# TheoCoombes/ClipCap

Hardware: AMD Instinct MI355X
Metric: train samples/sec (512-d prefix, 40-tok caption) (higher is better)
Workload: dtype bf16; 1 GPU; BASELINE configs[1]: TransformerMapper(8L,P=L=10,H=8)+frozen GPT-2-small; per_gpu_batch=256, global_batch=256, encoder_dim=512, train_language_model=False, parallelism=dp1

## Files before the change

clipcap_amd/_lib.py:

```python
from __future__ import annotations

import ctypes as C
import os
import threading

HERE = os.path.dirname(os.path.abspath(__file__))
_SEL = os.environ.get("CLIPCAP_HIP_LIB", "")
LIB_PATH = os.path.join(HERE, "libclipcap_hip.so") if not _SEL else os.path.join(HERE, "libclipcap_hip_lab.so") if _SEL == "lab" else _SEL
IS_LAB = _SEL == "lab"

ERR = {0: "ok", -1: "invalid argument", -2: "unsupported shape / alignment", -3: "kernel launch failed", -4: "invalid state"}


class HipExtensionMissing(RuntimeError):
    pass


class CCError(RuntimeError):
    pass


OP_BF16, OP_FP16, OP_X3 = 0, 1, 2


# ... 44 lines not shown
    "cc_gpt2_embed": (_I, [_GC, _GS, _P, _P, _P, _P, _P]),
    "cc_gpt2_embed_from": (_I, [_GC, _GS, _P, _P, _P, _P]),
    "cc_gpt2_fwd": (_I, [_GC, _GS, _P, _P, _P, _P]),
    "cc_gpt2_logits": (_I, [_GC, _GS, _P, _P, _P, _P, _L, _P]),
    "cc_gpt2_logits_bwd": (_I, [_GC, _GS, _P, _P, _P, _P, _L, _P, _P, _P]),
    "cc_lmhead_ce_fwd": (_I, [_GC, _GS, _P, _P, _P, _P, _P, _P]),
    "cc_lmhead_score": (_I, [_GC, _GS, _P, _P, _P, _P, _I, _P, _P, _P]),
    "cc_lmhead_ce_bwd": (_I, [_GC, _GS, _P, _P, _P, _P, _P, _P, _P]),
    "cc_lmhead_put_x": (_I, [_GC, _GS, _P, _P, _P]),
    "cc_lmhead_get": (_I, [_GC, _GS, _P, _I, _P, _L, _P]),
    "cc_gpt2_bwd": (_I, [_GC, _GS, _P, _P, _P, _P, _P, _P, _P]),
    "cc_decode_ws_bytes": (_L, [_GC, _I, _I]),
    "cc_decode_fwd": (_I, [_GC, _I, _I, _I, _I, _P, _P, _P, _P, _P, _P, _P, _L, _P]),
    "cc_decode_part_floats": (_L, [_GC, _I]),
    "cc_decode_fwd_p": (_I, [_GC, _I, _I, _I, _I, _P, _P, _P, _P, _P, _P, _P, _L, _P, _P]),
    "cc_decode_fwd_g": (_I, [_GC, _I, _I, _I, _I, _P, _P, _P, _P, _P, _I, _P, _P, _L, _P, _P]),
    "cc_beam_step_p": (_I, [_I, _I, _I, _P, _L, _P, _I, _F, _I, _I, _P, _P, _P, _P, _P, _P, _P]),
    "cc_decode_reorder": (_I, [_GC, _I, _I, _I, _I, _P, _P, _P, _P]),
    "cc_beam_step": (_I, [_I, _I, _I, _P, _L, _F, _I, _I, _P, _P, _P, _P, _P, _P, _P]),
    "cc_beam_ws_bytes": (_L, [_I, _I, _I]),
    "cc_logits_constrain": (_I, [_P, _I, _I, _L, _P, _I, _P, _I, _L, _I, _I, _I, _P, _I, _P, _P]),
    "cc_embed_tokens": (_I, [_GC, _I, _P, _P, _P, _P]),
    "cc_embed_tokens_bwd": (_I, [_GC, _I, _P, _P, _P, _P]),
    "cc_embed_tokens_bwd_ws": (_I, [_GC, _I, _P, _P, _P, _P, _P]),
    "cc_embed_tokens_bwd_ws_bytes": (_L, [_GC, _I]),
    "cc_beam_advance": (_I, [_GC, _I, _I, _P, _P, _P, _I, _I, _P, _P, _I, _I, _P, _P, _P, _P]),
    "cc_adamw_step": (_I, [_P, _P, _P, _P, _L, _F, _F, _F, _F, _F, _I, _F, _P, _P, _P]),
    "cc_adamw_step_cast": (_I, [_I, _P, _P, _P, _P, _L, _F, _F, _F, _F, _F, _I, _F, _P, _P, _P, _P]),
    "cc_cast_op16": (_I, [_I, _P, _P, _L, _P]),
    "cc_grad_wire_pack": (_I, [_P, _P, _L, _P]),
    "cc_grad_wire_unpack": (_I, [_P, _P, _L, _P]),
    "cc_grad_nonfinite": (_I, [_P, _L, _P, _P]),
    "cc_loss_scale_update": (_I, [_P, _P, _F, _F, _I, _P]),
    "cc_grad_norm_scratch_floats": (_L, []),
    "cc_grad_sqnorm": (_I, [_P, _L, _P, _P, _P]),
    "cc_grad_clip_coef": (_I, [_P, _F, _F, _P, _P, _P]),
    "cc_adamw_step_clip": (_I, [_I, _P, _P, _P, _P, _L, _F, _F, _F, _F, _F, _I, _F, _P, _P, _P, _P, _P]),
    "cc_dropout_mask": (_I, [C.c_uint64, _I, _I, _F, _L, _P, _P]),
    "cc_sample_step": (_I, [_P, _I, _I, _I, _F, _I, _F, _I, _P, _I, _I, _F, _P, _P, _P, _P]),
    "cc_sample_step_lp": (_I, [_P, _I, _I, _I, _F, _I, _F, _I, _P, _I, _I, _F, _I, _F, _P, _P, _P, _P]),
    "cc_wgrad_scratch_bytes": (_L, []),
    "cc_gemm_wgrad": (_I, [_I, _P, _I, _P, _I, _I, _I, _I, _P, _I, _P, _P]),
    "cc_x3_image_bytes": (_L, [_L, _L]),
    "cc_x3_split_rows": (_I, [_I, _P, _L, _I, _I, _I, _P, _P]),
    "cc_gemm_act": (_I, [_I, _I, _I, _P, _I, _I, _P, _I, _I, _I, _I, _P, _I, _I, _P, _I, _P, _P, _L, _P]),
    "cc_gemm_resid": (_I, [_I, _I, _I, _P, _I, _I, _P, _I, _I, _I, _I, _P, _P, _I, _P, _F, C.c_uint64, _I, _I, _P, _L, _P]),
    "cc_gemm_dact": (_I, [_I, _I, _I, _P, _I, _I, _P, _I, _I, _I, _I, _P, _I, _I, _P, _I, _P, _L, _P]),
    "cc_gemm_f32": (_I, [_I, _I, _I, _P, _I, _I, _P, _I, _I, _I, _I, _P, _I, _P, _I, _F, _I, _P, _L, _P]),
    "cc_gemm_wgrad_split": (_I, [_I, _P, _I, _I, _P, _I, _I, _I, _I, _P, _I, _P, _P, _L, _P]),
    "cc_gemm_tile_mode": (_I, [_I]),
    "cc_gemm_skinny_mode": (_I, [_I]),
    "cc_decode_mode": (_I, [_I]),
    "cc_decode_attention": (_I, [_GC, _I, _I, _I, _I, _P, _P, _P, _I, _I, _P, _P, C.POINTER(_I), _P]),
    "cc_gemm_op16_f32": (_I, [_I, _I, _I, _P, _I, _P, _I, _I, _I, _I, _P, _I, _P, _I, _P]),
    "cc_layernorm_fwd": (_I, [_I, _P, _P, _P, _P, _P, _P, _I, _I, _P]),
    "cc_attention_fwd": (_I, [_I, _P, _I, _I, _I, _I, _I, _P, _P, _P]),
    "cc_attention_bwd": (_I, [_I, _P, _P, _P, _P, _P, _I, _I, _I, _I, _I, _P, _P]),
    "cc_attention_fwd_x": (_I, [_I, _P, _I, _I, _I, _I, _I, _P, _I, _P, _F, C.c_uint64, _I, _P]),
    "cc_attention_bwd_x": (_I, [_I, _P, _P, _P, _P, _P, _I, _I, _I, _I, _I, _P, _I, _F, C.c_uint64, _I, _P]),
    "cc_red_scratch_floats": (_L, []),
    "cc_layernorm_bwd": (_I, [_I, _P, _P, _I, _P, _P, _P, _P, _P, _P, _P, _P, _P, _P, _I, _I, _P, _P]),
    "cc_colsum_bf16": (_I, [_I, _P, _I, _I, _I, _P, _P, _P]),
    "cc_colsum_multi": (_I, [_I, _P, _P, _I, _I, _I, _I, _P, _P]),
    "cc_batch_sum": (_I, [_P, _L, _P, _I, _I, _P, _P]),
    "cc_comm_unique_id": (_I, [_P]),
    "cc_comm_create": (_I, [C.POINTER(_P), _I, _I, _P]),
    "cc_allreduce_bucket": (_I, [_P, _P, _L, _I, _P]),
    "cc_broadcast_bucket": (_I, [_P, _P, _L, _I, _I, _P]),
    "cc_reduce_bucket": (_I, [_P, _P, _L, _I, _I, _P]),
    "cc_comm_destroy": (_I, [_P]),
    "cc_comm_count": (_I, [_P, C.POINTER(_I)]),
    "cc_prof_start": (_I, [_I, _I]),
    "cc_prof_stop": (_I, [C.POINTER(C.c_float), C.POINTER(C.c_double), C.POINTER(_I)]),
}

LAB_SIGNATURES = {
    "cc_decode_ws_check": (_I, [_GC, _I, _I, _P, _P]),
    "cc_decode_image_bytes": (_L, [_GC]),
    "cc_decode_image": (_I, [_GC, _P, _P, _P]),
    "cc_decode_xt_image_bytes": (_L, [_GC]),
    "cc_decode_xt_image": (_I, [_GC, _P, _P, _P]),
    "cc_decode_fwd_x": (_I, [_GC, _I, _I, _I, _I, _P, _P, _P, _P, _P, _P, _P, _I, _P, _P, _L, _P, _P]),
    "cc_decode_last_path": (_I, []),
}

ABI_VERSION = 3

SITES = {"lmhead_fwd": 1, "lmhead_dgrad": 2, "gpt2_fc_fwd": 3, "gpt2_proj2_fwd": 4, "gpt2_fc_dgrad": 5, "mapper_fc1_fwd": 6,
         "mapper_qkv_fwd": 7, "mapper_wgrad_fc2": 8, "all_gemms": 100}

_lib = None
_lock = threading.Lock()


def lib() -> C.CDLL:
    global _lib
    if _lib is not None:
        return _lib
    with _lock:
        if _lib is None:
            if not os.path.exists(LIB_PATH):
                raise HipExtensionMissing(
                    f"{LIB_PATH} not found: build it with `make -C clipcap_amd/csrc` (hipcc, gfx950). "
                    "clipcap_amd has no CPU fallback.")
            try:
                l = C.CDLL(LIB_PATH)
# ... 18 lines not shown
```

clipcap_amd/csrc/abi_dispatch.cpp:

```cpp
#include "../../include/clipcap_hip.h"
#ifdef CC_EXPERIMENTS
#include "../../include/clipcap_hip_lab.h"
#endif

extern "C" {

int64_t cc_mapper_param_count_bf16(const cc_mapper_cfg* cfg);
int64_t cc_mapper_param_count_f16(const cc_mapper_cfg* cfg);
int64_t cc_mapper_param_count_x3(const cc_mapper_cfg* cfg);
int cc_mapper_param_offsets_bf16(const cc_mapper_cfg* cfg, int64_t* offsets);
int cc_mapper_param_offsets_f16(const cc_mapper_cfg* cfg, int64_t* offsets);
int cc_mapper_param_offsets_x3(const cc_mapper_cfg* cfg, int64_t* offsets);
int64_t cc_mapper_ws_bytes_bf16(const cc_mapper_cfg* cfg, int32_t B, int32_t save);
int64_t cc_mapper_ws_bytes_f16(const cc_mapper_cfg* cfg, int32_t B, int32_t save);
int64_t cc_mapper_ws_bytes_x3(const cc_mapper_cfg* cfg, int32_t B, int32_t save);
int cc_mapper_sync_weights_bf16(const cc_mapper_cfg* cfg, const float* w32, uint16_t* w16, void* stream);
int cc_mapper_sync_weights_f16(const cc_mapper_cfg* cfg, const float* w32, uint16_t* w16, void* stream);
int cc_mapper_sync_weights_x3(const cc_mapper_cfg* cfg, const float* w32, uint16_t* w16, void* stream);
int cc_mapper_transpose_weights_bf16(const cc_mapper_cfg* cfg, uint16_t* w16, void* stream);
int cc_mapper_transpose_weights_f16(const cc_mapper_cfg* cfg, uint16_t* w16, void* stream);
int cc_mapper_transpose_weights_x3(const cc_mapper_cfg* cfg, uint16_t* w16, void* stream);
int cc_mapper_fwd_bf16(const cc_mapper_cfg* cfg, int32_t B, const float* w32, const uint16_t* w16, const float* emb, void* ws, float* out, int32_t save, void* stream);
int cc_mapper_fwd_f16(const cc_mapper_cfg* cfg, int32_t B, const float* w32, const uint16_t* w16, const float* emb, void* ws, float* out, int32_t save, void* stream);
int cc_mapper_fwd_x3(const cc_mapper_cfg* cfg, int32_t B, const float* w32, const uint16_t* w16, const float* emb, void* ws, float* out, int32_t save, void* stream);
// ... 81 lines not shown
int cc_embed_tokens_bwd_x3(const cc_gpt2_cfg* cfg, int32_t R, const float* dout, const int32_t* tokens, float* dwte, void* stream);
int cc_embed_tokens_bwd_ws_bf16(const cc_gpt2_cfg* cfg, int32_t R, const float* dout, const int32_t* tokens, float* dwte, void* ws, void* stream);
int cc_embed_tokens_bwd_ws_f16(const cc_gpt2_cfg* cfg, int32_t R, const float* dout, const int32_t* tokens, float* dwte, void* ws, void* stream);
int cc_embed_tokens_bwd_ws_x3(const cc_gpt2_cfg* cfg, int32_t R, const float* dout, const int32_t* tokens, float* dwte, void* ws, void* stream);
int64_t cc_embed_tokens_bwd_ws_bytes_bf16(const cc_gpt2_cfg* cfg, int32_t R);
int64_t cc_embed_tokens_bwd_ws_bytes_f16(const cc_gpt2_cfg* cfg, int32_t R);
int64_t cc_embed_tokens_bwd_ws_bytes_x3(const cc_gpt2_cfg* cfg, int32_t R);
int cc_beam_advance_bf16(const cc_gpt2_cfg* cfg, int32_t R, int32_t beam, const float* w32, const int32_t* next_tokens, const int32_t* src_rows, int32_t pos, int32_t ctx_max, const int32_t* row_map_in, int32_t* row_map_out, int32_t step, int32_t tok_ld, const int32_t* tokens_in, int32_t* tokens_out, float* x_out, void* stream);
int cc_beam_advance_f16(const cc_gpt2_cfg* cfg, int32_t R, int32_t beam, const float* w32, const int32_t* next_tokens, const int32_t* src_rows, int32_t pos, int32_t ctx_max, const int32_t* row_map_in, int32_t* row_map_out, int32_t step, int32_t tok_ld, const int32_t* tokens_in, int32_t* tokens_out, float* x_out, void* stream);
int cc_beam_advance_x3(const cc_gpt2_cfg* cfg, int32_t R, int32_t beam, const float* w32, const int32_t* next_tokens, const int32_t* src_rows, int32_t pos, int32_t ctx_max, const int32_t* row_map_in, int32_t* row_map_out, int32_t step, int32_t tok_ld, const int32_t* tokens_in, int32_t* tokens_out, float* x_out, void* stream);
int cc_adamw_step_bf16(float* p32, const float* g32, float* m, float* v, int64_t n, float lr, float beta1, float beta2, float eps, float weight_decay, int32_t step, float grad_scale, const float* loss_scale, const float* found_inf, void* stream);
int cc_adamw_step_cast_bf16(float* p32, const float* g32, float* m, float* v, int64_t n, float lr, float beta1, float beta2, float eps, float weight_decay, int32_t step, float grad_scale, const float* loss_scale, const float* found_inf, uint16_t* w16, void* stream);
int cc_adamw_step_cast_f16(float* p32, const float* g32, float* m, float* v, int64_t n, float lr, float beta1, float beta2, float eps, float weight_decay, int32_t step, float grad_scale, const float* loss_scale, const float* found_inf, uint16_t* w16, void* stream);
int cc_adamw_step_cast_x3(float* p32, const float* g32, float* m, float* v, int64_t n, float lr, float beta1, float beta2, float eps, float weight_decay, int32_t step, float grad_scale, const float* loss_scale, const float* found_inf, uint16_t* w16, void* stream);
int cc_cast_op16_bf16(const float* src, uint16_t* dst, int64_t n, void* stream);
int cc_cast_op16_f16(const float* src, uint16_t* dst, int64_t n, void* stream);
int cc_cast_op16_x3(const float* src, uint16_t* dst, int64_t n, void* stream);
int cc_grad_wire_pack_bf16(const float* g32, uint16_t* wire, int64_t n, void* stream);
int cc_grad_wire_unpack_bf16(const uint16_t* wire, float* g32, int64_t n, void* stream);
int cc_grad_nonfinite_bf16(const float* g32, int64_t n, float* found_inf, void* stream);
int cc_loss_scale_update_bf16(float* state, float* found_inf, float growth, float backoff, int32_t interval, void* stream);
int64_t cc_grad_norm_scratch_floats_bf16(void);
int cc_grad_sqnorm_bf16(const float* g32, int64_t n, float* scratch, float* sumsq, void* stream);
int cc_grad_clip_coef_bf16(const float* sumsq, float max_norm, float grad_scale, const float* loss_scale, float* clip, void* stream);
int cc_adamw_step_clip_bf16(float* p32, const float* g32, float* m, float* v, int64_t n, float lr, float beta1, float beta2, float eps, float weight_decay, int32_t step, float grad_scale, const float* loss_scale, const float* found_inf, const float* clip, uint16_t* w16, void* stream);
int cc_adamw_step_clip_f16(float* p32, const float* g32, float* m, float* v, int64_t n, float lr, float beta1, float beta2, float eps, float weight_decay, int32_t step, float grad_scale, const float* loss_scale, const float* found_inf, const float* clip, uint16_t* w16, void* stream);
int cc_adamw_step_clip_x3(float* p32, const float* g32, float* m, float* v, int64_t n, float lr, float beta1, float beta2, float eps, float weight_decay, int32_t step, float grad_scale, const float* loss_scale, const float* found_inf, const float* clip, uint16_t* w16, void* stream);
int cc_dropout_mask_bf16(uint64_t seed, int32_t site, int32_t layer, float p, int64_t n, uint8_t* out, void* stream);
int cc_sample_step_bf16(const float* logits, int32_t R, int32_t V, int32_t ld, float temperature, int32_t top_k, float top_p, int32_t mode, const int64_t* history, int32_t hist_len, int32_t hist_ld, float repetition_penalty, const float* u, int32_t* next_token, float* probs_out, void* stream);
int cc_sample_step_lp_bf16(const float* logits, int32_t R, int32_t V, int32_t ld, float temperature, int32_t top_k, float top_p, int32_t mode, const int64_t* history, int32_t hist_len, int32_t hist_ld, float repetition_penalty, int32_t stop_token, float length_penalty, const float* u, int32_t* next_token, float* probs_out, void* stream);
int cc_gemm_op16_f32_bf16(int32_t al, int32_t bl, const uint16_t* A, int32_t lda, const uint16_t* B, int32_t ldb, int32_t M, int32_t N, int32_t K, float* C, int32_t ldc, const float* bias, int32_t ksplit, void* stream);
int cc_gemm_op16_f32_f16(int32_t al, int32_t bl, const uint16_t* A, int32_t lda, const uint16_t* B, int32_t ldb, int32_t M, int32_t N, int32_t K, float* C, int32_t ldc, const float* bias, int32_t ksplit, void* stream);
int cc_gemm_op16_f32_x3(int32_t al, int32_t bl, const uint16_t* A, int32_t lda, const uint16_t* B, int32_t ldb, int32_t M, int32_t N, int32_t K, float* C, int32_t ldc, const float* bias, int32_t ksplit, void* stream);
int64_t cc_wgrad_scratch_bytes_bf16(void);
int cc_gemm_wgrad_bf16(const uint16_t* X, int32_t ldx, const uint16_t* Y, int32_t ldy, int32_t Mw, int32_t Nw, int32_t K, float* dW, int32_t ldw, float* scratch, void* stream);
int cc_gemm_wgrad_f16(const uint16_t* X, int32_t ldx, const uint16_t* Y, int32_t ldy, int32_t Mw, int32_t Nw, int32_t K, float* dW, int32_t ldw, float* scratch, void* stream);
int cc_gemm_wgrad_x3(const uint16_t* X, int32_t ldx, const uint16_t* Y, int32_t ldy, int32_t Mw, int32_t Nw, int32_t K, float* dW, int32_t ldw, float* scratch, void* stream);
int64_t cc_x3_image_bytes_bf16(int64_t rows, int64_t depth);
int cc_x3_split_rows_bf16(const float* src, int64_t ld, int32_t rows, int32_t width, int32_t form, uint16_t* dst, void* stream);
int cc_x3_split_rows_f16(const float* src, int64_t ld, int32_t rows, int32_t width, int32_t form, uint16_t* dst, void* stream);
int cc_x3_split_rows_x3(const float* src, int64_t ld, int32_t rows, int32_t width, int32_t form, uint16_t* dst, void* stream);
int cc_gemm_act_bf16(int32_t al, int32_t bl, const void* A, int32_t a_img, int32_t lda, const uint16_t* B, int32_t ldb, int32_t M, int32_t N, int32_t K, void* C, int32_t c_img, int32_t ldc, const float* bias, int32_t act, void* pre, void* x3, int64_t x3_bytes, void* stream);
int cc_gemm_act_f16(int32_t al, int32_t bl, const void* A, int32_t a_img, int32_t lda, const uint16_t* B, int32_t ldb, int32_t M, int32_t N, int32_t K, void* C, int32_t c_img, int32_t ldc, const float* bias, int32_t act, void* pre, void* x3, int64_t x3_bytes, void* stream);
int cc_gemm_act_x3(int32_t al, int32_t bl, const void* A, int32_t a_img, int32_t lda, const uint16_t* B, int32_t ldb, int32_t M, int32_t N, int32_t K, void* C, int32_t c_img, int32_t ldc, const float* bias, int32_t act, void* pre, void* x3, int64_t x3_bytes, void* stream);
int cc_gemm_resid_bf16(int32_t al, int32_t bl, const void* A, int32_t a_img, int32_t lda, const uint16_t* B, int32_t ldb, int32_t M, int32_t N, int32_t K, float* out, const float* res, int32_t ld, const float* bias, float p, uint64_t seed, int32_t site, int32_t layer, void* x3, int64_t x3_bytes, void* stream);
int cc_gemm_resid_f16(int32_t al, int32_t bl, const void* A, int32_t a_img, int32_t lda, const uint16_t* B, int32_t ldb, int32_t M, int32_t N, int32_t K, float* out, const float* res, int32_t ld, const float* bias, float p, uint64_t seed, int32_t site, int32_t layer, void* x3, int64_t x3_bytes, void* stream);
int cc_gemm_resid_x3(int32_t al, int32_t bl, const void* A, int32_t a_img, int32_t lda, const uint16_t* B, int32_t ldb, int32_t M, int32_t N, int32_t K, float* out, const float* res, int32_t ld, const float* bias, float p, uint64_t seed, int32_t site, int32_t layer, void* x3, int64_t x3_bytes, void* stream);
int cc_gemm_dact_bf16(int32_t al, int32_t bl, const void* A, int32_t a_img, int32_t lda, const uint16_t* B, int32_t ldb, int32_t M, int32_t N, int32_t K, void* C, int32_t c_img, int32_t ldc, const void* aux, int32_t act, void* x3, int64_t x3_bytes, void* stream);
int cc_gemm_dact_f16(int32_t al, int32_t bl, const void* A, int32_t a_img, int32_t lda, const uint16_t* B, int32_t ldb, int32_t M, int32_t N, int32_t K, void* C, int32_t c_img, int32_t ldc, const void* aux, int32_t act, void* x3, int64_t x3_bytes, void* stream);
int cc_gemm_dact_x3(int32_t al, int32_t bl, const void* A, int32_t a_img, int32_t lda, const uint16_t* B, int32_t ldb, int32_t M, int32_t N, int32_t K, void* C, int32_t c_img, int32_t ldc, const void* aux, int32_t act, void* x3, int64_t x3_bytes, void* stream);
int cc_gemm_f32_bf16(int32_t al, int32_t bl, const void* A, int32_t a_img, int32_t lda, const uint16_t* B, int32_t ldb, int32_t M, int32_t N, int32_t K, float* C, int32_t ldc, const float* bias, int32_t mode, float alpha, int32_t ksplit, void* x3, int64_t x3_bytes, void* stream);
int cc_gemm_f32_f16(int32_t al, int32_t bl, const void* A, int32_t a_img, int32_t lda, const uint16_t* B, int32_t ldb, int32_t M, int32_t N, int32_t K, float* C, int32_t ldc, const float* bias, int32_t mode, float alpha, int32_t ksplit, void* x3, int64_t x3_bytes, void* stream);
int cc_gemm_f32_x3(int32_t al, int32_t bl, const void* A, int32_t a_img, int32_t lda, const uint16_t* B, int32_t ldb, int32_t M, int32_t N, int32_t K, float* C, int32_t ldc, const float* bias, int32_t mode, float alpha, int32_t ksplit, void* x3, int64_t x3_bytes, void* stream);
int cc_gemm_wgrad_split_bf16(const void* X, int32_t x_img, int32_t ldx, const float* Y, int32_t ldy, int32_t Mw, int32_t Nw, int32_t K, float* dW, int32_t ldw, float* scratch, void* x3, int64_t x3_bytes, void* stream);
int cc_gemm_wgrad_split_f16(const void* X, int32_t x_img, int32_t ldx, const float* Y, int32_t ldy, int32_t Mw, int32_t Nw, int32_t K, float* dW, int32_t ldw, float* scratch, void* x3, int64_t x3_bytes, void* stream);
int cc_gemm_wgrad_split_x3(const void* X, int32_t x_img, int32_t ldx, const float* Y, int32_t ldy, int32_t Mw, int32_t Nw, int32_t K, float* dW, int32_t ldw, float* scratch, void* x3, int64_t x3_bytes, void* stream);
int cc_decode_attention_bf16(const cc_gpt2_cfg* cfg, int32_t R, int32_t Tnew, int32_t pos0, int32_t ctx_max, const uint16_t* qkv, uint16_t* kv_layer, const int32_t* row_map, int32_t group, int32_t append, void* ws, uint16_t* out, int32_t* path, void* stream);
int cc_decode_attention_f16(const cc_gpt2_cfg* cfg, int32_t R, int32_t Tnew, int32_t pos0, int32_t ctx_max, const uint16_t* qkv, uint16_t* kv_layer, const int32_t* row_map, int32_t group, int32_t append, void* ws, uint16_t* out, int32_t* path, void* stream);
int cc_decode_attention_x3(const cc_gpt2_cfg* cfg, int32_t R, int32_t Tnew, int32_t pos0, int32_t ctx_max, const uint16_t* qkv, uint16_t* kv_layer, const int32_t* row_map, int32_t group, int32_t append, void* ws, uint16_t* out, int32_t* path, void* stream);
int cc_layernorm_fwd_bf16(const float* x, const float* gamma, const float* beta, uint16_t* y, float* mean, float* rstd, int32_t rows, int32_t D, void* stream);
int cc_layernorm_fwd_f16(const float* x, const float* gamma, const float* beta, uint16_t* y, float* mean, float* rstd, int32_t rows, int32_t D, void* stream);
int cc_layernorm_fwd_x3(const float* x, const float* gamma, const float* beta, uint16_t* y, float* mean, float* rstd, int32_t rows, int32_t D, void* stream);
int cc_attention_fwd_bf16(const uint16_t* qkv, int32_t B, int32_t S, int32_t H, int32_t hd, int32_t causal, uint16_t* out, float* lse, void* stream);
int cc_attention_fwd_f16(const uint16_t* qkv, int32_t B, int32_t S, int32_t H, int32_t hd, int32_t causal, uint16_t* out, float* lse, void* stream);
int cc_attention_fwd_x3(const uint16_t* qkv, int32_t B, int32_t S, int32_t H, int32_t hd, int32_t causal, uint16_t* out, float* lse, void* stream);
int cc_attention_bwd_bf16(const uint16_t* qkv, const uint16_t* dout, const uint16_t* o, const float* lse, float* delta_ws, int32_t B, int32_t S, int32_t H, int32_t hd, int32_t causal, uint16_t* dqkv, void* stream);
int cc_attention_bwd_f16(const uint16_t* qkv, const uint16_t* dout, const uint16_t* o, const float* lse, float* delta_ws, int32_t B, int32_t S, int32_t H, int32_t hd, int32_t causal, uint16_t* dqkv, void* stream);
int cc_attention_bwd_x3(const uint16_t* qkv, const uint16_t* dout, const uint16_t* o, const float* lse, float* delta_ws, int32_t B, int32_t S, int32_t H, int32_t hd, int32_t causal, uint16_t* dqkv, void* stream);
int cc_attention_fwd_x_bf16(const uint16_t* qkv, int32_t B, int32_t S, int32_t H, int32_t hd, int32_t causal, uint16_t* out, int32_t out_img, float* lse, float p, uint64_t seed, int32_t layer, void* stream);
int cc_attention_fwd_x_f16(const uint16_t* qkv, int32_t B, int32_t S, int32_t H, int32_t hd, int32_t causal, uint16_t* out, int32_t out_img, float* lse, float p, uint64_t seed, int32_t layer, void* stream);
int cc_attention_fwd_x_x3(const uint16_t* qkv, int32_t B, int32_t S, int32_t H, int32_t hd, int32_t causal, uint16_t* out, int32_t out_img, float* lse, float p, uint64_t seed, int32_t layer, void* stream);
int cc_attention_bwd_x_bf16(const uint16_t* qkv, const uint16_t* dout, const uint16_t* o, const float* lse, float* delta_ws, int32_t B, int32_t S, int32_t H, int32_t hd, int32_t causal, uint16_t* dqkv, int32_t dqkv_img, float p, uint64_t seed, int32_t layer, void* stream);
int cc_attention_bwd_x_f16(const uint16_t* qkv, const uint16_t* dout, const uint16_t* o, const float* lse, float* delta_ws, int32_t B, int32_t S, int32_t H, int32_t hd, int32_t causal, uint16_t* dqkv, int32_t dqkv_img, float p, uint64_t seed, int32_t layer, void* stream);
int cc_attention_bwd_x_x3(const uint16_t* qkv, const uint16_t* dout, const uint16_t* o, const float* lse, float* delta_ws, int32_t B, int32_t S, int32_t H, int32_t hd, int32_t causal, uint16_t* dqkv, int32_t dqkv_img, float p, uint64_t seed, int32_t layer, void* stream);
int cc_lmhead_put_x_bf16(const cc_gpt2_cfg* cfg, const cc_gpt2_shape* shp, void* ws, const float* x, void* stream);
int cc_lmhead_put_x_f16(const cc_gpt2_cfg* cfg, const cc_gpt2_shape* shp, void* ws, const float* x, void* stream);
int cc_lmhead_put_x_x3(const cc_gpt2_cfg* cfg, const cc_gpt2_shape* shp, void* ws, const float* x, void* stream);
int cc_lmhead_get_bf16(const cc_gpt2_cfg* cfg, const cc_gpt2_shape* shp, void* ws, int32_t field, void* dst, int64_t dst_bytes, void* stream);
int cc_lmhead_get_f16(const cc_gpt2_cfg* cfg, const cc_gpt2_shape* shp, void* ws, int32_t field, void* dst, int64_t dst_bytes, void* stream);
int cc_lmhead_get_x3(const cc_gpt2_cfg* cfg, const cc_gpt2_shape* shp, void* ws, int32_t field, void* dst, int64_t dst_bytes, void* stream);
int64_t cc_red_scratch_floats_bf16(void);
int cc_layernorm_bwd_bf16(const uint16_t* dy, const float* x, int32_t ldx, const int32_t* row_map, const float* mean, const float* rstd, const float* gamma, const float* dres, float* dx32, uint16_t* dx16, float* dgamma, float* dbeta, float* dcol, int32_t rows, int32_t D, float* red_ws, void* stream);
int cc_layernorm_bwd_f16(const uint16_t* dy, const float* x, int32_t ldx, const int32_t* row_map, const float* mean, const float* rstd, const float* gamma, const float* dres, float* dx32, uint16_t* dx16, float* dgamma, float* dbeta, float* dcol, int32_t rows, int32_t D, float* red_ws, void* stream);
int cc_layernorm_bwd_x3(const uint16_t* dy, const float* x, int32_t ldx, const int32_t* row_map, const float* mean, const float* rstd, const float* gamma, const float* dres, float* dx32, uint16_t* dx16, float* dgamma, float* dbeta, float* dcol, int32_t rows, int32_t D, float* red_ws, void* stream);
int cc_colsum_bf16_bf16(const uint16_t* X, int32_t ld, int32_t M, int32_t N, float* out, float* red_ws, void* stream);
int cc_colsum_bf16_f16(const uint16_t* X, int32_t ld, int32_t M, int32_t N, float* out, float* red_ws, void* stream);
int cc_colsum_bf16_x3(const uint16_t* X, int32_t ld, int32_t M, int32_t N, float* out, float* red_ws, void* stream);
int cc_colsum_multi_bf16(const uint16_t* const* X_host, float* const* out_host, int32_t n, int32_t ld, int32_t M, int32_t N, float* red_ws, void* stream);
int cc_colsum_multi_f16(const uint16_t* const* X_host, float* const* out_host, int32_t n, int32_t ld, int32_t M, int32_t N, float* red_ws, void* stream);
int cc_colsum_multi_x3(const uint16_t* const* X_host, float* const* out_host, int32_t n, int32_t ld, int32_t M, int32_t N, float* red_ws, void* stream);
int cc_batch_sum_bf16(const float* src, int64_t src_stride, float* dst, int32_t len, int32_t B, float* red_ws, void* stream);

int64_t cc_mapper_param_count(const cc_mapper_cfg* cfg) { const int op_ = (cfg ? cfg->op_dtype : CC_OP_BF16); return op_ == CC_OP_FP16 ? cc_mapper_param_count_f16(cfg) : op_ == CC_OP_BF16X3 ? cc_mapper_param_count_x3(cfg) : cc_mapper_param_count_bf16(cfg); }
int cc_mapper_param_offsets(const cc_mapper_cfg* cfg, int64_t* offsets) { const int op_ = (cfg ? cfg->op_dtype : CC_OP_BF16); return op_ == CC_OP_FP16 ? cc_mapper_param_offsets_f16(cfg, offsets) : op_ == CC_OP_BF16X3 ? cc_mapper_param_offsets_x3(cfg, offsets) : cc_mapper_param_offsets_bf16(cfg, offsets); }
int64_t cc_mapper_ws_bytes(const cc_mapper_cfg* cfg, int32_t B, int32_t save) { const int op_ = (cfg ? cfg->op_dtype : CC_OP_BF16); return op_ == CC_OP_FP16 ? cc_mapper_ws_bytes_f16(cfg, B, save) : op_ == CC_OP_BF16X3 ? cc_mapper_ws_bytes_x3(cfg, B, save) : cc_mapper_ws_bytes_bf16(cfg, B, save); }
int cc_mapper_sync_weights(const cc_mapper_cfg* cfg, const float* w32, uint16_t* w16, void* stream) { const int op_ = (cfg ? cfg->op_dtype : CC_OP_BF16); return op_ == CC_OP_FP16 ? cc_mapper_sync_weights_f16(cfg, w32, w16, stream) : op_ == CC_OP_BF16X3 ? cc_mapper_sync_weights_x3(cfg, w32, w16, stream) : cc_mapper_sync_weights_bf16(cfg, w32, w16, stream); }
int cc_mapper_transpose_weights(const cc_mapper_cfg* cfg, uint16_t* w16, void* stream) { const int op_ = (cfg ? cfg->op_dtype : CC_OP_BF16); return op_ == CC_OP_FP16 ? cc_mapper_transpose_weights_f16(cfg, w16, stream) : op_ == CC_OP_BF16X3 ? cc_mapper_transpose_weights_x3(cfg, w16, stream) : cc_mapper_transpose_weights_bf16(cfg, w16, stream); }
int cc_mapper_fwd(const cc_mapper_cfg* cfg, int32_t B, const float* w32, const uint16_t* w16, const float* emb, void* ws, float* out, int32_t save, void* stream) { const int op_ = (cfg ? cfg->op_dtype : CC_OP_BF16); return op_ == CC_OP_FP16 ? cc_mapper_fwd_f16(cfg, B, w32, w16, emb, ws, out, save, stream) : op_ == CC_OP_BF16X3 ? cc_mapper_fwd_x3(cfg, B, w32, w16, emb, ws, out, save, stream) : cc_mapper_fwd_bf16(cfg, B, w32, w16, emb, ws, out, save, stream); }
int cc_mapper_attention_probs(const cc_mapper_cfg* cfg, int32_t B, void* ws, int32_t layer, float* out, void* stream) { const int op_ = (cfg ? cfg->op_dtype : CC_OP_BF16); return op_ == CC_OP_FP16 ? cc_mapper_attention_probs_f16(cfg, B, ws, layer, out, stream) : op_ == CC_OP_BF16X3 ? cc_mapper_attention_probs_x3(cfg, B, ws, layer, out, stream) : cc_mapper_attention_probs_bf16(cfg, B, ws, layer, out, stream); }
int cc_mapper_bwd(const cc_mapper_cfg* cfg, int32_t B, const float* w32, const uint16_t* w16, void* ws, const float* dout, float* g32, void* stream) { const int op_ = (cfg ? cfg->op_dtype : CC_OP_BF16); return op_ == CC_OP_FP16 ? cc_mapper_bwd_f16(cfg, B, w32, w16, ws, dout, g32, stream) : op_ == CC_OP_BF16X3 ? cc_mapper_bwd_x3(cfg, B, w32, w16, ws, dout, g32, stream) : cc_mapper_bwd_bf16(cfg, B, w32, w16, ws, dout, g32, stream); }
int cc_mapper_bwd_range(const cc_mapper_cfg* cfg, int32_t B, const float* w32, const uint16_t* w16, void* ws, const float* dout, float* g32, int32_t l_hi, int32_t l_lo, void* stream) { const int op_ = (cfg ? cfg->op_dtype : CC_OP_BF16); return op_ == CC_OP_FP16 ? cc_mapper_bwd_range_f16(cfg, B, w32, w16, ws, dout, g32, l_hi, l_lo, stream) : op_ == CC_OP_BF16X3 ? cc_mapper_bwd_range_x3(cfg, B, w32, w16, ws, dout, g32, l_hi, l_lo, stream) : cc_mapper_bwd_range_bf16(cfg, B, w32, w16, ws, dout, g32, l_hi, l_lo, stream); }
int64_t cc_gpt2_param_count(const cc_gpt2_cfg* cfg) { const int op_ = (cfg ? cfg->op_dtype : CC_OP_BF16); return op_ == CC_OP_FP16 ? cc_gpt2_param_count_f16(cfg) : op_ == CC_OP_BF16X3 ? cc_gpt2_param_count_x3(cfg) : cc_gpt2_param_count_bf16(cfg); }
int cc_gpt2_param_offsets(const cc_gpt2_cfg* cfg, int64_t* offsets) { const int op_ = (cfg ? cfg->op_dtype : CC_OP_BF16); return op_ == CC_OP_FP16 ? cc_gpt2_param_offsets_f16(cfg, offsets) : op_ == CC_OP_BF16X3 ? cc_gpt2_param_offsets_x3(cfg, offsets) : cc_gpt2_param_offsets_bf16(cfg, offsets); }
int64_t cc_gpt2_ws_bytes(const cc_gpt2_cfg* cfg, const cc_gpt2_shape* shp) { const int op_ = (cfg ? cfg->op_dtype : CC_OP_BF16); return op_ == CC_OP_FP16 ? cc_gpt2_ws_bytes_f16(cfg, shp) : op_ == CC_OP_BF16X3 ? cc_gpt2_ws_bytes_x3(cfg, shp) : cc_gpt2_ws_bytes_bf16(cfg, shp); }
int cc_gpt2_sync_weights(const cc_gpt2_cfg* cfg, const float* w32, uint16_t* w16, void* stream) { const int op_ = (cfg ? cfg->op_dtype : CC_OP_BF16); return op_ == CC_OP_FP16 ? cc_gpt2_sync_weights_f16(cfg, w32, w16, stream) : op_ == CC_OP_BF16X3 ? cc_gpt2_sync_weights_x3(cfg, w32, w16, stream) : cc_gpt2_sync_weights_bf16(cfg, w32, w16, stream); }
int cc_gpt2_transpose_weights(const cc_gpt2_cfg* cfg, uint16_t* w16, void* stream) { const int op_ = (cfg ? cfg->op_dtype : CC_OP_BF16); return op_ == CC_OP_FP16 ? cc_gpt2_transpose_weights_f16(cfg, w16, stream) : op_ == CC_OP_BF16X3 ? cc_gpt2_transpose_weights_x3(cfg, w16, stream) : cc_gpt2_transpose_weights_bf16(cfg, w16, stream); }
int cc_gpt2_embed(const cc_gpt2_cfg* cfg, const cc_gpt2_shape* shp, const float* w32, const float* prefix, const int64_t* tokens, void* ws, void* stream) { const int op_ = (cfg ? cfg->op_dtype : CC_OP_BF16); return op_ == CC_OP_FP16 ? cc_gpt2_embed_f16(cfg, shp, w32, prefix, tokens, ws, stream) : op_ == CC_OP_BF16X3 ? cc_gpt2_embed_x3(cfg, shp, w32, prefix, tokens, ws, stream) : cc_gpt2_embed_bf16(cfg, shp, w32, prefix, tokens, ws, stream); }
int cc_gpt2_embed_from(const cc_gpt2_cfg* cfg, const cc_gpt2_shape* shp, const float* w32, const float* inputs_embeds, void* ws, void* stream) { const int op_ = (cfg ? cfg->op_dtype : CC_OP_BF16); return op_ == CC_OP_FP16 ? cc_gpt2_embed_from_f16(cfg, shp, w32, inputs_embeds, ws, stream) : op_ == CC_OP_BF16X3 ? cc_gpt2_embed_from_x3(cfg, shp, w32, inputs_embeds, ws, stream) : cc_gpt2_embed_from_bf16(cfg, shp, w32, inputs_embeds, ws, stream); }
int cc_gpt2_fwd(const cc_gpt2_cfg* cfg, const cc_gpt2_shape* shp, const float* w32, const uint16_t* w16, void* ws, void* stream) { const int op_ = (cfg ? cfg->op_dtype : CC_OP_BF16); return op_ == CC_OP_FP16 ? cc_gpt2_fwd_f16(cfg, shp, w32, w16, ws, stream) : op_ == CC_OP_BF16X3 ? cc_gpt2_fwd_x3(cfg, shp, w32, w16, ws, stream) : cc_gpt2_fwd_bf16(cfg, shp, w32, w16, ws, stream); }
int cc_gpt2_logits(const cc_gpt2_cfg* cfg, const cc_gpt2_shape* shp, const float* w32, const uint16_t* w16, void* ws, float* logits, int64_t ldl, void* stream) { const int op_ = (cfg ? cfg->op_dtype : CC_OP_BF16); return op_ == CC_OP_FP16 ? cc_gpt2_logits_f16(cfg, shp, w32, w16, ws, logits, ldl, stream) : op_ == CC_OP_BF16X3 ? cc_gpt2_logits_x3(cfg, shp, w32, w16, ws, logits, ldl, stream) : cc_gpt2_logits_bf16(cfg, shp, w32, w16, ws, logits, ldl, stream); }
int cc_gpt2_logits_bwd(const cc_gpt2_cfg* cfg, const cc_gpt2_shape* shp, const float* w32, const uint16_t* w16, void* ws, const float* dlogits, int64_t ldl, float* dx0, float* g32, void* stream) { const int op_ = (cfg ? cfg->op_dtype : CC_OP_BF16); return op_ == CC_OP_FP16 ? cc_gpt2_logits_bwd_f16(cfg, shp, w32, w16, ws, dlogits, ldl, dx0, g32, stream) : op_ == CC_OP_BF16X3 ? cc_gpt2_logits_bwd_x3(cfg, shp, w32, w16, ws, dlogits, ldl, dx0, g32, stream) : cc_gpt2_logits_bwd_bf16(cfg, shp, w32, w16, ws, dlogits, ldl, dx0, g32, stream); }
int cc_lmhead_ce_fwd(const cc_gpt2_cfg* cfg, const cc_gpt2_shape* shp, const float* w32, const uint16_t* w16, void* ws, const int64_t* tokens, float* stats, void* stream) { const int op_ = (cfg ? cfg->op_dtype : CC_OP_BF16); return op_ == CC_OP_FP16 ? cc_lmhead_ce_fwd_f16(cfg, shp, w32, w16, ws, tokens, stats, stream) : op_ == CC_OP_BF16X3 ? cc_lmhead_ce_fwd_x3(cfg, shp, w32, w16, ws, tokens, stats, stream) : cc_lmhead_ce_fwd_bf16(cfg, shp, w32, w16, ws, tokens, stats, stream); }
int cc_lmhead_score(const cc_gpt2_cfg* cfg, const cc_gpt2_shape* shp, const float* w32, const uint16_t* w16, void* ws, const int64_t* tokens, int32_t ignore_zero, float* token_logprob, float* sample_stats, void* stream) { const int op_ = (cfg ? cfg->op_dtype : CC_OP_BF16); return op_ == CC_OP_FP16 ? cc_lmhead_score_f16(cfg, shp, w32, w16, ws, tokens, ignore_zero, token_logprob, sample_stats, stream) : op_ == CC_OP_BF16X3 ? cc_lmhead_score_x3(cfg, shp, w32, w16, ws, tokens, ignore_zero, token_logprob, sample_stats, stream) : cc_lmhead_score_bf16(cfg, shp, w32, w16, ws, tokens, ignore_zero, token_logprob, sample_stats, stream); }
int cc_lmhead_ce_bwd(const cc_gpt2_cfg* cfg, const cc_gpt2_shape* shp, const float* w32, const uint16_t* w16, void* ws, const float* denom, const float* loss_scale, float* g32, void* stream) { const int op_ = (cfg ? cfg->op_dtype : CC_OP_BF16); return op_ == CC_OP_FP16 ? cc_lmhead_ce_bwd_f16(cfg, shp, w32, w16, ws, denom, loss_scale, g32, stream) : op_ == CC_OP_BF16X3 ? cc_lmhead_ce_bwd_x3(cfg, shp, w32, w16, ws, denom, loss_scale, g32, stream) : cc_lmhead_ce_bwd_bf16(cfg, shp, w32, w16, ws, denom, loss_scale, g32, stream); }
int cc_gpt2_bwd(const cc_gpt2_cfg* cfg, const cc_gpt2_shape* shp, const float* w32, const uint16_t* w16, void* ws, const int64_t* tokens, float* dprefix, float* g32, void* stream) { const int op_ = (cfg ? cfg->op_dtype : CC_OP_BF16); return op_ == CC_OP_FP16 ? cc_gpt2_bwd_f16(cfg, shp, w32, w16, ws, tokens, dprefix, g32, stream) : op_ == CC_OP_BF16X3 ? cc_gpt2_bwd_x3(cfg, shp, w32, w16, ws, tokens, dprefix, g32, stream) : cc_gpt2_bwd_bf16(cfg, shp, w32, w16, ws, tokens, dprefix, g32, stream); }
int cc_gpt2_bwd_range(const cc_gpt2_cfg* cfg, const cc_gpt2_shape* shp, const float* w32, const uint16_t* w16, void* ws, const int64_t* tokens, float* dprefix, float* g32, int32_t l_hi, int32_t l_lo, void* stream) { const int op_ = (cfg ? cfg->op_dtype : CC_OP_BF16); return op_ == CC_OP_FP16 ? cc_gpt2_bwd_range_f16(cfg, shp, w32, w16, ws, tokens, dprefix, g32, l_hi, l_lo, stream) : op_ == CC_OP_BF16X3 ? cc_gpt2_bwd_range_x3(cfg, shp, w32, w16, ws, tokens, dprefix, g32, l_hi, l_lo, stream) : cc_gpt2_bwd_range_bf16(cfg, shp, w32, w16, ws, tokens, dprefix, g32, l_hi, l_lo, stream); }
int64_t cc_decode_ws_bytes(const cc_gpt2_cfg* cfg, int32_t R, int32_t Tnew) { const int op_ = (cfg ? cfg->op_dtype : CC_OP_BF16); return op_ == CC_OP_FP16 ? cc_decode_ws_bytes_f16(cfg, R, Tnew) : op_ == CC_OP_BF16X3 ? cc_decode_ws_bytes_x3(cfg, R, Tnew) : cc_decode_ws_bytes_bf16(cfg, R, Tnew); }
int cc_decode_fwd(const cc_gpt2_cfg* cfg, int32_t R, int32_t Tnew, int32_t pos0, int32_t ctx_max, const float* w32, const uint16_t* w16, const float* x, uint16_t* kv, const int32_t* row_map, void* ws, float* logits, int64_t ldl, void* stream) { const int op_ = (cfg ? cfg->op_dtype : CC_OP_BF16); return op_ == CC_OP_FP16 ? cc_decode_fwd_f16(cfg, R, Tnew, pos0, ctx_max, w32, w16, x, kv, row_map, ws, logits, ldl, stream) : op_ == CC_OP_BF16X3 ? cc_decode_fwd_x3(cfg, R, Tnew, pos0, ctx_max, w32, w16, x, kv, row_map, ws, logits, ldl, stream) : cc_decode_fwd_bf16(cfg, R, Tnew, pos0, ctx_max, w32, w16, x, kv, row_map, ws, logits, ldl, stream); }
int64_t cc_decode_part_floats(const cc_gpt2_cfg* cfg, int32_t R) { const int op_ = (cfg ? cfg->op_dtype : CC_OP_BF16); return op_ == CC_OP_FP16 ? cc_decode_part_floats_f16(cfg, R) : op_ == CC_OP_BF16X3 ? cc_decode_part_floats_x3(cfg, R) : cc_decode_part_floats_bf16(cfg, R); }
int cc_decode_fwd_p(const cc_gpt2_cfg* cfg, int32_t R, int32_t Tnew, int32_t pos0, int32_t ctx_max, const float* w32, const uint16_t* w16, const float* x, uint16_t* kv, const int32_t* row_map, void* ws, float* logits, int64_t ldl, float* lpart, void* stream) { const int op_ = (cfg ? cfg->op_dtype : CC_OP_BF16); return op_ == CC_OP_FP16 ? cc_decode_fwd_p_f16(cfg, R, Tnew, pos0, ctx_max, w32, w16, x, kv, row_map, ws, logits, ldl, lpart, stream) : op_ == CC_OP_BF16X3 ? cc_decode_fwd_p_x3(cfg, R, Tnew, pos0, ctx_max, w32, w16, x, kv, row_map, ws, logits, ldl, lpart, stream) : cc_decode_fwd_p_bf16(cfg, R, Tnew, pos0, ctx_max, w32, w16, x, kv, row_map, ws, logits, ldl, lpart, stream); }
int cc_decode_fwd_g(const cc_gpt2_cfg* cfg, int32_t R, int32_t Tnew, int32_t pos0, int32_t ctx_max, const float* w32, const uint16_t* w16, const float* x, uint16_t* kv, const int32_t* row_map, int32_t group, void* ws, float* logits, int64_t ldl, float* lpart, void* stream) { const int op_ = (cfg ? cfg->op_dtype : CC_OP_BF16); return op_ == CC_OP_FP16 ? cc_decode_fwd_g_f16(cfg, R, Tnew, pos0, ctx_max, w32, w16, x, kv, row_map, group, ws, logits, ldl, lpart, stream) : op_ == CC_OP_BF16X3 ? cc_decode_fwd_g_x3(cfg, R, Tnew, pos0, ctx_max, w32, w16, x, kv, row_map, group, ws, logits, ldl, lpart, stream) : cc_decode_fwd_g_bf16(cfg, R, Tnew, pos0, ctx_max, w32, w16, x, kv, row_map, group, ws, logits, ldl, lpart, stream); }
int cc_decode_reorder(const cc_gpt2_cfg* cfg, int32_t R_src, int32_t R_dst, int32_t ctx, int32_t ctx_max, const uint16_t* kv_src, uint16_t* kv_dst, const int32_t* src, void* stream) { const int op_ = (cfg ? cfg->op_dtype : CC_OP_BF16); return op_ == CC_OP_FP16 ? cc_decode_reorder_f16(cfg, R_src, R_dst, ctx, ctx_max, kv_src, kv_dst, src, stream) : op_ == CC_OP_BF16X3 ? cc_decode_reorder_x3(cfg, R_src, R_dst, ctx, ctx_max, kv_src, kv_dst, src, stream) : cc_decode_reorder_bf16(cfg, R_src, R_dst, ctx, ctx_max, kv_src, kv_dst, src, stream); }
int cc_beam_step(int32_t S, int32_t beam, int32_t V, const float* logits, int64_t ldl, float temperature, int32_t first, int32_t stop_token, float* scores, float* seq_lengths, uint8_t* has_stopped, int32_t* next_tokens, int32_t* src_rows, void* ws, void* stream) { return cc_beam_step_bf16(S, beam, V, logits, ldl, temperature, first, stop_token, scores, seq_lengths, has_stopped, next_tokens, src_rows, ws, stream); }
int cc_beam_step_p(int32_t S, int32_t beam, int32_t V, const float* logits, int64_t ldl, const float* lpart, int32_t npart, float temperature, int32_t first, int32_t stop_token, float* scores, float* seq_lengths, uint8_t* has_stopped, int32_t* next_tokens, int32_t* src_rows, void* ws, void* stream) { return cc_beam_step_p_bf16(S, beam, V, logits, ldl, lpart, npart, temperature, first, stop_token, scores, seq_lengths, has_stopped, next_tokens, src_rows, ws, stream); }
int64_t cc_beam_ws_bytes(int32_t S, int32_t beam, int32_t V) { return cc_beam_ws_bytes_bf16(S, beam, V); }
int cc_logits_constrain(float* logits, int32_t R, int32_t V, int64_t ldl, float* lpart, int32_t npart, const void* history, int32_t hist_elem_bytes, int64_t hist_stride, int32_t hist_len, int32_t no_repeat_ngram, int32_t ban_token, const int32_t* suppress, int32_t n_suppress, const uint8_t* skip_rows, void* stream) { return cc_logits_constrain_bf16(logits, R, V, ldl, lpart, npart, history, hist_elem_bytes, hist_stride, hist_len, no_repeat_ngram, ban_token, suppress, n_suppress, skip_rows, stream); }
int cc_embed_tokens(const cc_gpt2_cfg* cfg, int32_t R, const float* w32, const int32_t* tokens, float* out, void* stream) { const int op_ = (cfg ? cfg->op_dtype : CC_OP_BF16); return op_ == CC_OP_FP16 ? cc_embed_tokens_f16(cfg, R, w32, tokens, out, stream) : op_ == CC_OP_BF16X3 ? cc_embed_tokens_x3(cfg, R, w32, tokens, out, stream) : cc_embed_tokens_bf16(cfg, R, w32, tokens, out, stream); }
int cc_embed_tokens_bwd(const cc_gpt2_cfg* cfg, int32_t R, const float* dout, const int32_t* tokens, float* dwte, void* stream) { const int op_ = (cfg ? cfg->op_dtype : CC_OP_BF16); return op_ == CC_OP_FP16 ? cc_embed_tokens_bwd_f16(cfg, R, dout, tokens, dwte, stream) : op_ == CC_OP_BF16X3 ? cc_embed_tokens_bwd_x3(cfg, R, dout, tokens, dwte, stream) : cc_embed_tokens_bwd_bf16(cfg, R, dout, tokens, dwte, stream); }
int cc_embed_tokens_bwd_ws(const cc_gpt2_cfg* cfg, int32_t R, const float* dout, const int32_t* tokens, float* dwte, void* ws, void* stream) { const int op_ = (cfg ? cfg->op_dtype : CC_OP_BF16); return op_ == CC_OP_FP16 ? cc_embed_tokens_bwd_ws_f16(cfg, R, dout, tokens, dwte, ws, stream) : op_ == CC_OP_BF16X3 ? cc_embed_tokens_bwd_ws_x3(cfg, R, dout, tokens, dwte, ws, stream) : cc_embed_tokens_bwd_ws_bf16(cfg, R, dout, tokens, dwte, ws, stream); }
int64_t cc_embed_tokens_bwd_ws_bytes(const cc_gpt2_cfg* cfg, int32_t R) { const int op_ = (cfg ? cfg->op_dtype : CC_OP_BF16); return op_ == CC_OP_FP16 ? cc_embed_tokens_bwd_ws_bytes_f16(cfg, R) : op_ == CC_OP_BF16X3 ? cc_embed_tokens_bwd_ws_bytes_x3(cfg, R) : cc_embed_tokens_bwd_ws_bytes_bf16(cfg, R); }
int cc_beam_advance(const cc_gpt2_cfg* cfg, int32_t R, int32_t beam, const float* w32, const int32_t* next_tokens, const int32_t* src_rows, int32_t pos, int32_t ctx_max, const int32_t* row_map_in, int32_t* row_map_out, int32_t step, int32_t tok_ld, const int32_t* tokens_in, int32_t* tokens_out, float* x_out, void* stream) { const int op_ = (cfg ? cfg->op_dtype : CC_OP_BF16); return op_ == CC_OP_FP16 ? cc_beam_advance_f16(cfg, R, beam, w32, next_tokens, src_rows, pos, ctx_max, row_map_in, row_map_out, step, tok_ld, tokens_in, tokens_out, x_out, stream) : op_ == CC_OP_BF16X3 ? cc_beam_advance_x3(cfg, R, beam, w32, next_tokens, src_rows, pos, ctx_max, row_map_in, row_map_out, step, tok_ld, tokens_in, tokens_out, x_out, stream) : cc_beam_advance_bf16(cfg, R, beam, w32, next_tokens, src_rows, pos, ctx_max, row_map_in, row_map_out, step, tok_ld, tokens_in, tokens_out, x_out, stream); }
int cc_adamw_step(float* p32, const float* g32, float* m, float* v, int64_t n, float lr, float beta1, float beta2, float eps, float weight_decay, int32_t step, float grad_scale, const float* loss_scale, const float* found_inf, void* stream) { return cc_adamw_step_bf16(p32, g32, m, v, n, lr, beta1, beta2, eps, weight_decay, step, grad_scale, loss_scale, found_inf, stream); }
int cc_adamw_step_cast(int32_t op_dtype, float* p32, const float* g32, float* m, float* v, int64_t n, float lr, float beta1, float beta2, float eps, float weight_decay, int32_t step, float grad_scale, const float* loss_scale, const float* found_inf, uint16_t* w16, void* stream) { const int op_ = op_dtype; return op_ == CC_OP_FP16 ? cc_adamw_step_cast_f16(p32, g32, m, v, n, lr, beta1, beta2, eps, weight_decay, step, grad_scale, loss_scale, found_inf, w16, stream) : op_ == CC_OP_BF16X3 ? cc_adamw_step_cast_x3(p32, g32, m, v, n, lr, beta1, beta2, eps, weight_decay, step, grad_scale, loss_scale, found_inf, w16, stream) : cc_adamw_step_cast_bf16(p32, g32, m, v, n, lr, beta1, beta2, eps, weight_decay, step, grad_scale, loss_scale, found_inf, w16, stream); }
int cc_cast_op16(int32_t op_dtype, const float* src, uint16_t* dst, int64_t n, void* stream) { const int op_ = op_dtype; return op_ == CC_OP_FP16 ? cc_cast_op16_f16(src, dst, n, stream) : op_ == CC_OP_BF16X3 ? cc_cast_op16_x3(src, dst, n, stream) : cc_cast_op16_bf16(src, dst, n, stream); }
int cc_grad_wire_pack(const float* g32, uint16_t* wire, int64_t n, void* stream) { return cc_grad_wire_pack_bf16(g32, wire, n, stream); }
int cc_grad_wire_unpack(const uint16_t* wire, float* g32, int64_t n, void* stream) { return cc_grad_wire_unpack_bf16(wire, g32, n, stream); }
int cc_grad_nonfinite(const float* g32, int64_t n, float* found_inf, void* stream) { return cc_grad_nonfinite_bf16(g32, n, found_inf, stream); }
int cc_loss_scale_update(float* state, float* found_inf, float growth, float backoff, int32_t interval, void* stream) { return cc_loss_scale_update_bf16(state, found_inf, growth, backoff, interval, stream); }
int64_t cc_grad_norm_scratch_floats(void) { return cc_grad_norm_scratch_floats_bf16(); }
int cc_grad_sqnorm(const float* g32, int64_t n, float* scratch, float* sumsq, void* stream) { return cc_grad_sqnorm_bf16(g32, n, scratch, sumsq, stream); }
int cc_grad_clip_coef(const float* sumsq, float max_norm, float grad_scale, const float* loss_scale, float* clip, void* stream) { return cc_grad_clip_coef_bf16(sumsq, max_norm, grad_scale, loss_scale, clip, stream); }
int cc_adamw_step_clip(int32_t op_dtype, float* p32, const float* g32, float* m, float* v, int64_t n, float lr, float beta1, float beta2, float eps, float weight_decay, int32_t step, float grad_scale, const float* loss_scale, const float* found_inf, const float* clip, uint16_t* w16, void* stream) { const int op_ = op_dtype; return op_ == CC_OP_FP16 ? cc_adamw_step_clip_f16(p32, g32, m, v, n, lr, beta1, beta2, eps, weight_decay, step, grad_scale, loss_scale, found_inf, clip, w16, stream) : op_ == CC_OP_BF16X3 ? cc_adamw_step_clip_x3(p32, g32, m, v, n, lr, beta1, beta2, eps, weight_decay, step, grad_scale, loss_scale, found_inf, clip, w16, stream) : cc_adamw_step_clip_bf16(p32, g32, m, v, n, lr, beta1, beta2, eps, weight_decay, step, grad_scale, loss_scale, found_inf, clip, w16, stream); }
int cc_dropout_mask(uint64_t seed, int32_t site, int32_t layer, float p, int64_t n, uint8_t* out, void* stream) { return cc_dropout_mask_bf16(seed, site, layer, p, n, out, stream); }
int cc_sample_step(const float* logits, int32_t R, int32_t V, int32_t ld, float temperature, int32_t top_k, float top_p, int32_t mode, const int64_t* history, int32_t hist_len, int32_t hist_ld, float repetition_penalty, const float* u, int32_t* next_token, float* probs_out, void* stream) { return cc_sample_step_bf16(logits, R, V, ld, temperature, top_k, top_p, mode, history, hist_len, hist_ld, repetition_penalty, u, next_token, probs_out, stream); }
int cc_sample_step_lp(const float* logits, int32_t R, int32_t V, int32_t ld, float temperature, int32_t top_k, float top_p, int32_t mode, const int64_t* history, int32_t hist_len, int32_t hist_ld, float repetition_penalty, int32_t stop_token, float length_penalty, const float* u, int32_t* next_token, float* probs_out, void* stream) { return cc_sample_step_lp_bf16(logits, R, V, ld, temperature, top_k, top_p, mode, history, hist_len, hist_ld, repetition_penalty, stop_token, length_penalty, u, next_token, probs_out, stream); }
int cc_gemm_op16_f32(int32_t op_dtype, int32_t al, int32_t bl, const uint16_t* A, int32_t lda, const uint16_t* B, int32_t ldb, int32_t M, int32_t N, int32_t K, float* C, int32_t ldc, const float* bias, int32_t ksplit, void* stream) { const int op_ = op_dtype; return op_ == CC_OP_FP16 ? cc_gemm_op16_f32_f16(al, bl, A, lda, B, ldb, M, N, K, C, ldc, bias, ksplit, stream) : op_ == CC_OP_BF16X3 ? cc_gemm_op16_f32_x3(al, bl, A, lda, B, ldb, M, N, K, C, ldc, bias, ksplit, stream) : cc_gemm_op16_f32_bf16(al, bl, A, lda, B, ldb, M, N, K, C, ldc, bias, ksplit, stream); }
int64_t cc_wgrad_scratch_bytes(void) { return cc_wgrad_scratch_bytes_bf16(); }
int cc_gemm_wgrad(int32_t op_dtype, const uint16_t* X, int32_t ldx, const uint16_t* Y, int32_t ldy, int32_t Mw, int32_t Nw, int32_t K, float* dW, int32_t ldw, float* scratch, void* stream) { const int op_ = op_dtype; return op_ == CC_OP_FP16 ? cc_gemm_wgrad_f16(X, ldx, Y, ldy, Mw, Nw, K, dW, ldw, scratch, stream) : op_ == CC_OP_BF16X3 ? cc_gemm_wgrad_x3(X, ldx, Y, ldy, Mw, Nw, K, dW, ldw, scratch, stream) : cc_gemm_wgrad_bf16(X, ldx, Y, ldy, Mw, Nw, K, dW, ldw, scratch, stream); }
int64_t cc_x3_image_bytes(int64_t rows, int64_t depth) { return cc_x3_image_bytes_bf16(rows, depth); }
int cc_x3_split_rows(int32_t op_dtype, const float* src, int64_t ld, int32_t rows, int32_t width, int32_t form, uint16_t* dst, void* stream) { const int op_ = op_dtype; return op_ == CC_OP_FP16 ? cc_x3_split_rows_f16(src, ld, rows, width, form, dst, stream) : op_ == CC_OP_BF16X3 ? cc_x3_split_rows_x3(src, ld, rows, width, form, dst, stream) : cc_x3_split_rows_bf16(src, ld, rows, width, form, dst, stream); }
int cc_gemm_act(int32_t op_dtype, int32_t al, int32_t bl, const void* A, int32_t a_img, int32_t lda, const uint16_t* B, int32_t ldb, int32_t M, int32_t N, int32_t K, void* C, int32_t c_img, int32_t ldc, const float* bias, int32_t act, void* pre, void* x3, int64_t x3_bytes, void* stream) { const int op_ = op_dtype; return op_ == CC_OP_FP16 ? cc_gemm_act_f16(al, bl, A, a_img, lda, B, ldb, M, N, K, C, c_img, ldc, bias, act, pre, x3, x3_bytes, stream) : op_ == CC_OP_BF16X3 ? cc_gemm_act_x3(al, bl, A, a_img, lda, B, ldb, M, N, K, C, c_img, ldc, bias, act, pre, x3, x3_bytes, stream) : cc_gemm_act_bf16(al, bl, A, a_img, lda, B, ldb, M, N, K, C, c_img, ldc, bias, act, pre, x3, x3_bytes, stream); }
int cc_gemm_resid(int32_t op_dtype, int32_t al, int32_t bl, const void* A, int32_t a_img, int32_t lda, const uint16_t* B, int32_t ldb, int32_t M, int32_t N, int32_t K, float* out, const float* res, int32_t ld, const float* bias, float p, uint64_t seed, int32_t site, int32_t layer, void* x3, int64_t x3_bytes, void* stream) { const int op_ = op_dtype; return op_ == CC_OP_FP16 ? cc_gemm_resid_f16(al, bl, A, a_img, lda, B, ldb, M, N, K, out, res, ld, bias, p, seed, site, layer, x3, x3_bytes, stream) : op_ == CC_OP_BF16X3 ? cc_gemm_resid_x3(al, bl, A, a_img, lda, B, ldb, M, N, K, out, res, ld, bias, p, seed, site, layer, x3, x3_bytes, stream) : cc_gemm_resid_bf16(al, bl, A, a_img, lda, B, ldb, M, N, K, out, res, ld, bias, p, seed, site, layer, x3, x3_bytes, stream); }
int cc_gemm_dact(int32_t op_dtype, int32_t al, int32_t bl, const void* A, int32_t a_img, int32_t lda, const uint16_t* B, int32_t ldb, int32_t M, int32_t N, int32_t K, void* C, int32_t c_img, int32_t ldc, const void* aux, int32_t act, void* x3, int64_t x3_bytes, void* stream) { const int op_ = op_dtype; return op_ == CC_OP_FP16 ? cc_gemm_dact_f16(al, bl, A, a_img, lda, B, ldb, M, N, K, C, c_img, ldc, aux, act, x3, x3_bytes, stream) : op_ == CC_OP_BF16X3 ? cc_gemm_dact_x3(al, bl, A, a_img, lda, B, ldb, M, N, K, C, c_img, ldc, aux, act, x3, x3_bytes, stream) : cc_gemm_dact_bf16(al, bl, A, a_img, lda, B, ldb, M, N, K, C, c_img, ldc, aux, act, x3, x3_bytes, stream); }
int cc_gemm_f32(int32_t op_dtype, int32_t al, int32_t bl, const void* A, int32_t a_img, int32_t lda, const uint16_t* B, int32_t ldb, int32_t M, int32_t N, int32_t K, float* C, int32_t ldc, const float* bias, int32_t mode, float alpha, int32_t ksplit, void* x3, int64_t x3_bytes, void* stream) { const int op_ = op_dtype; return op_ == CC_OP_FP16 ? cc_gemm_f32_f16(al, bl, A, a_img, lda, B, ldb, M, N, K, C, ldc, bias, mode, alpha, ksplit, x3, x3_bytes, stream) : op_ == CC_OP_BF16X3 ? cc_gemm_f32_x3(al, bl, A, a_img, lda, B, ldb, M, N, K, C, ldc, bias, mode, alpha, ksplit, x3, x3_bytes, stream) : cc_gemm_f32_bf16(al, bl, A, a_img, lda, B, ldb, M, N, K, C, ldc, bias, mode, alpha, ksplit, x3, x3_bytes, stream); }
int cc_gemm_wgrad_split(int32_t op_dtype, const void* X, int32_t x_img, int32_t ldx, const float* Y, int32_t ldy, int32_t Mw, int32_t Nw, int32_t K, float* dW, int32_t ldw, float* scratch, void* x3, int64_t x3_bytes, void* stream) { const int op_ = op_dtype; return op_ == CC_OP_FP16 ? cc_gemm_wgrad_split_f16(X, x_img, ldx, Y, ldy, Mw, Nw, K, dW, ldw, scratch, x3, x3_bytes, stream) : op_ == CC_OP_BF16X3 ? cc_gemm_wgrad_split_x3(X, x_img, ldx, Y, ldy, Mw, Nw, K, dW, ldw, scratch, x3, x3_bytes, stream) : cc_gemm_wgrad_split_bf16(X, x_img, ldx, Y, ldy, Mw, Nw, K, dW, ldw, scratch, x3, x3_bytes, stream); }
int cc_decode_attention(const cc_gpt2_cfg* cfg, int32_t R, int32_t Tnew, int32_t pos0, int32_t ctx_max, const uint16_t* qkv, uint16_t* kv_layer, const int32_t* row_map, int32_t group, int32_t append, void* ws, uint16_t* out, int32_t* path, void* stream) { const int op_ = (cfg ? cfg->op_dtype : CC_OP_BF16); return op_ == CC_OP_FP16 ? cc_decode_attention_f16(cfg, R, Tnew, pos0, ctx_max, qkv, kv_layer, row_map, group, append, ws, out, path, stream) : op_ == CC_OP_BF16X3 ? cc_decode_attention_x3(cfg, R, Tnew, pos0, ctx_max, qkv, kv_layer, row_map, group, append, ws, out, path, stream) : cc_decode_attention_bf16(cfg, R, Tnew, pos0, ctx_max, qkv, kv_layer, row_map, group, append, ws, out, path, stream); }
int cc_layernorm_fwd(int32_t op_dtype, const float* x, const float* gamma, const float* beta, uint16_t* y, float* mean, float* rstd, int32_t rows, int32_t D, void* stream) { const int op_ = op_dtype; return op_ == CC_OP_FP16 ? cc_layernorm_fwd_f16(x, gamma, beta, y, mean, rstd, rows, D, stream) : op_ == CC_OP_BF16X3 ? cc_layernorm_fwd_x3(x, gamma, beta, y, mean, rstd, rows, D, stream) : cc_layernorm_fwd_bf16(x, gamma, beta, y, mean, rstd, rows, D, stream); }
int cc_attention_fwd(int32_t op_dtype, const uint16_t* qkv, int32_t B, int32_t S, int32_t H, int32_t hd, int32_t causal, uint16_t* out, float* lse, void* stream) { const int op_ = op_dtype; return op_ == CC_OP_FP16 ? cc_attention_fwd_f16(qkv, B, S, H, hd, causal, out, lse, stream) : op_ == CC_OP_BF16X3 ? cc_attention_fwd_x3(qkv, B, S, H, hd, causal, out, lse, stream) : cc_attention_fwd_bf16(qkv, B, S, H, hd, causal, out, lse, stream); }
int cc_attention_bwd(int32_t op_dtype, const uint16_t* qkv, const uint16_t* dout, const uint16_t* o, const float* lse, float* delta_ws, int32_t B, int32_t S, int32_t H, int32_t hd, int32_t causal, uint16_t* dqkv, void* stream) { const int op_ = op_dtype; return op_ == CC_OP_FP16 ? cc_attention_bwd_f16(qkv, dout, o, lse, delta_ws, B, S, H, hd, causal, dqkv, stream) : op_ == CC_OP_BF16X3 ? cc_attention_bwd_x3(qkv, dout, o, lse, delta_ws, B, S, H, hd, causal, dqkv, stream) : cc_attention_bwd_bf16(qkv, dout, o, lse, delta_ws, B, S, H, hd, causal, dqkv, stream); }
int cc_attention_fwd_x(int32_t op_dtype, const uint16_t* qkv, int32_t B, int32_t S, int32_t H, int32_t hd, int32_t causal, uint16_t* out, int32_t out_img, float* lse, float p, uint64_t seed, int32_t layer, void* stream) { const int op_ = op_dtype; return op_ == CC_OP_FP16 ? cc_attention_fwd_x_f16(qkv, B, S, H, hd, causal, out, out_img, lse, p, seed, layer, stream) : op_ == CC_OP_BF16X3 ? cc_attention_fwd_x_x3(qkv, B, S, H, hd, causal, out, out_img, lse, p, seed, layer, stream) : cc_attention_fwd_x_bf16(qkv, B, S, H, hd, causal, out, out_img, lse, p, seed, layer, stream); }
int cc_attention_bwd_x(int32_t op_dtype, const uint16_t* qkv, const uint16_t* dout, const uint16_t* o, const float* lse, float* delta_ws, int32_t B, int32_t S, int32_t H, int32_t hd, int32_t causal, uint16_t* dqkv, int32_t dqkv_img, float p, uint64_t seed, int32_t layer, void* stream) { const int op_ = op_dtype; return op_ == CC_OP_FP16 ? cc_attention_bwd_x_f16(qkv, dout, o, lse, delta_ws, B, S, H, hd, causal, dqkv, dqkv_img, p, seed, layer, stream) : op_ == CC_OP_BF16X3 ? cc_attention_bwd_x_x3(qkv, dout, o, lse, delta_ws, B, S, H, hd, causal, dqkv, dqkv_img, p, seed, layer, stream) : cc_attention_bwd_x_bf16(qkv, dout, o, lse, delta_ws, B, S, H, hd, causal, dqkv, dqkv_img, p, seed, layer, stream); }
int cc_lmhead_put_x(const cc_gpt2_cfg* cfg, const cc_gpt2_shape* shp, void* ws, const float* x, void* stream) { const int op_ = (cfg ? cfg->op_dtype : CC_OP_BF16); return op_ == CC_OP_FP16 ? cc_lmhead_put_x_f16(cfg, shp, ws, x, stream) : op_ == CC_OP_BF16X3 ? cc_lmhead_put_x_x3(cfg, shp, ws, x, stream) : cc_lmhead_put_x_bf16(cfg, shp, ws, x, stream); }
int cc_lmhead_get(const cc_gpt2_cfg* cfg, const cc_gpt2_shape* shp, void* ws, int32_t field, void* dst, int64_t dst_bytes, void* stream) { const int op_ = (cfg ? cfg->op_dtype : CC_OP_BF16); return op_ == CC_OP_FP16 ? cc_lmhead_get_f16(cfg, shp, ws, field, dst, dst_bytes, stream) : op_ == CC_OP_BF16X3 ? cc_lmhead_get_x3(cfg, shp, ws, field, dst, dst_bytes, stream) : cc_lmhead_get_bf16(cfg, shp, ws, field, dst, dst_bytes, stream); }
int64_t cc_red_scratch_floats(void) { return cc_red_scratch_floats_bf16(); }
int cc_layernorm_bwd(int32_t op_dtype, const uint16_t* dy, const float* x, int32_t ldx, const int32_t* row_map, const float* mean, const float* rstd, const float* gamma, const float* dres, float* dx32, uint16_t* dx16, float* dgamma, float* dbeta, float* dcol, int32_t rows, int32_t D, float* red_ws, void* stream) { const int op_ = op_dtype; return op_ == CC_OP_FP16 ? cc_layernorm_bwd_f16(dy, x, ldx, row_map, mean, rstd, gamma, dres, dx32, dx16, dgamma, dbeta, dcol, rows, D, red_ws, stream) : op_ == CC_OP_BF16X3 ? cc_layernorm_bwd_x3(dy, x, ldx, row_map, mean, rstd, gamma, dres, dx32, dx16, dgamma, dbeta, dcol, rows, D, red_ws, stream) : cc_layernorm_bwd_bf16(dy, x, ldx, row_map, mean, rstd, gamma, dres, dx32, dx16, dgamma, dbeta, dcol, rows, D, red_ws, stream); }
int cc_colsum_bf16(int32_t op_dtype, const uint16_t* X, int32_t ld, int32_t M, int32_t N, float* out, float* red_ws, void* stream) { const int op_ = op_dtype; return op_ == CC_OP_FP16 ? cc_colsum_bf16_f16(X, ld, M, N, out, red_ws, stream) : op_ == CC_OP_BF16X3 ? cc_colsum_bf16_x3(X, ld, M, N, out, red_ws, stream) : cc_colsum_bf16_bf16(X, ld, M, N, out, red_ws, stream); }
int cc_colsum_multi(int32_t op_dtype, const uint16_t* const* X_host, float* const* out_host, int32_t n, int32_t ld, int32_t M, int32_t N, float* red_ws, void* stream) { const int op_ = op_dtype; return op_ == CC_OP_FP16 ? cc_colsum_multi_f16(X_host, out_host, n, ld, M, N, red_ws, stream) : op_ == CC_OP_BF16X3 ? cc_colsum_multi_x3(X_host, out_host, n, ld, M, N, red_ws, stream) : cc_colsum_multi_bf16(X_host, out_host, n, ld, M, N, red_ws, stream); }
int cc_batch_sum(const float* src, int64_t src_stride, float* dst, int32_t len, int32_t B, float* red_ws, void* stream) { return cc_batch_sum_bf16(src, src_stride, dst, len, B, red_ws, stream); }

#ifdef CC_EXPERIMENTS
int cc_decode_ws_check_bf16(const cc_gpt2_cfg* cfg, int32_t R, int32_t Tnew, const void* ws, void* stream);
int cc_decode_ws_check_f16(const cc_gpt2_cfg* cfg, int32_t R, int32_t Tnew, const void* ws, void* stream);
int cc_decode_ws_check_x3(const cc_gpt2_cfg* cfg, int32_t R, int32_t Tnew, const void* ws, void* stream);
int64_t cc_decode_image_bytes_bf16(const cc_gpt2_cfg* cfg);
int64_t cc_decode_image_bytes_f16(const cc_gpt2_cfg* cfg);
int64_t cc_decode_image_bytes_x3(const cc_gpt2_cfg* cfg);
int cc_decode_image_bf16(const cc_gpt2_cfg* cfg, const uint16_t* w16, uint16_t* wimg, void* stream);
int cc_decode_image_f16(const cc_gpt2_cfg* cfg, const uint16_t* w16, uint16_t* wimg, void* stream);
int cc_decode_image_x3(const cc_gpt2_cfg* cfg, const uint16_t* w16, uint16_t* wimg, void* stream);
int64_t cc_decode_xt_image_bytes_bf16(const cc_gpt2_cfg* cfg);
int64_t cc_decode_xt_image_bytes_f16(const cc_gpt2_cfg* cfg);
int64_t cc_decode_xt_image_bytes_x3(const cc_gpt2_cfg* cfg);
int cc_decode_xt_image_bf16(const cc_gpt2_cfg* cfg, const uint16_t* w16, uint16_t* wteam, void* stream);
int cc_decode_xt_image_f16(const cc_gpt2_cfg* cfg, const uint16_t* w16, uint16_t* wteam, void* stream);
int cc_decode_xt_image_x3(const cc_gpt2_cfg* cfg, const uint16_t* w16, uint16_t* wteam, void* stream);
int cc_decode_fwd_x_bf16(const cc_gpt2_cfg* cfg, int32_t R, int32_t Tnew, int32_t pos0, int32_t ctx_max, const float* w32, const uint16_t* w16, const uint16_t* wimg, const uint16_t* wteam, const float* x, uint16_t* kv, const int32_t* row_map, int32_t group, void* ws, float* logits, int64_t ldl, float* lpart, void* stream);
int cc_decode_fwd_x_f16(const cc_gpt2_cfg* cfg, int32_t R, int32_t Tnew, int32_t pos0, int32_t ctx_max, const float* w32, const uint16_t* w16, const uint16_t* wimg, const uint16_t* wteam, const float* x, uint16_t* kv, const int32_t* row_map, int32_t group, void* ws, float* logits, int64_t ldl, float* lpart, void* stream);
int cc_decode_fwd_x_x3(const cc_gpt2_cfg* cfg, int32_t R, int32_t Tnew, int32_t pos0, int32_t ctx_max, const float* w32, const uint16_t* w16, const uint16_t* wimg, const uint16_t* wteam, const float* x, uint16_t* kv, const int32_t* row_map, int32_t group, void* ws, float* logits, int64_t ldl, float* lpart, void* stream);

int cc_decode_ws_check(const cc_gpt2_cfg* cfg, int32_t R, int32_t Tnew, const void* ws, void* stream) { const int op_ = (cfg ? cfg->op_dtype : CC_OP_BF16); return op_ == CC_OP_FP16 ? cc_decode_ws_check_f16(cfg, R, Tnew, ws, stream) : op_ == CC_OP_BF16X3 ? cc_decode_ws_check_x3(cfg, R, Tnew, ws, stream) : cc_decode_ws_check_bf16(cfg, R, Tnew, ws, stream); }
int64_t cc_decode_image_bytes(const cc_gpt2_cfg* cfg) { const int op_ = (cfg ? cfg->op_dtype : CC_OP_BF16); return op_ == CC_OP_FP16 ? cc_decode_image_bytes_f16(cfg) : op_ == CC_OP_BF16X3 ? cc_decode_image_bytes_x3(cfg) : cc_decode_image_bytes_bf16(cfg); }
int cc_decode_image(const cc_gpt2_cfg* cfg, const uint16_t* w16, uint16_t* wimg, void* stream) { const int op_ = (cfg ? cfg->op_dtype : CC_OP_BF16); return op_ == CC_OP_FP16 ? cc_decode_image_f16(cfg, w16, wimg, stream) : op_ == CC_OP_BF16X3 ? cc_decode_image_x3(cfg, w16, wimg, stream) : cc_decode_image_bf16(cfg, w16, wimg, stream); }
int64_t cc_decode_xt_image_bytes(const cc_gpt2_cfg* cfg) { const int op_ = (cfg ? cfg->op_dtype : CC_OP_BF16); return op_ == CC_OP_FP16 ? cc_decode_xt_image_bytes_f16(cfg) : op_ == CC_OP_BF16X3 ? cc_decode_xt_image_bytes_x3(cfg) : cc_decode_xt_image_bytes_bf16(cfg); }
int cc_decode_xt_image(const cc_gpt2_cfg* cfg, const uint16_t* w16, uint16_t* wteam, void* stream) { const int op_ = (cfg ? cfg->op_dtype : CC_OP_BF16); return op_ == CC_OP_FP16 ? cc_decode_xt_image_f16(cfg, w16, wteam, stream) : op_ == CC_OP_BF16X3 ? cc_decode_xt_image_x3(cfg, w16, wteam, stream) : cc_decode_xt_image_bf16(cfg, w16, wteam, stream); }
int cc_decode_fwd_x(const cc_gpt2_cfg* cfg, int32_t R, int32_t Tnew, int32_t pos0, int32_t ctx_max, const float* w32, const uint16_t* w16, const uint16_t* wimg, const uint16_t* wteam, const float* x, uint16_t* kv, const int32_t* row_map, int32_t group, void* ws, float* logits, int64_t ldl, float* lpart, void* stream) { const int op_ = (cfg ? cfg->op_dtype : CC_OP_BF16); return op_ == CC_OP_FP16 ? cc_decode_fwd_x_f16(cfg, R, Tnew, pos0, ctx_max, w32, w16, wimg, wteam, x, kv, row_map, group, ws, logits, ldl, lpart, stream) : op_ == CC_OP_BF16X3 ? cc_decode_fwd_x_x3(cfg, R, Tnew, pos0, ctx_max, w32, w16, wimg, wteam, x, kv, row_map, group, ws, logits, ldl, lpart, stream) : cc_decode_fwd_x_bf16(cfg, R, Tnew, pos0, ctx_max, w32, w16, wimg, wteam, x, kv, row_map, group, ws, logits, ldl, lpart, stream); }
#endif

}
```

clipcap_amd/csrc/api.hip:

```cpp
#include "../../include/clipcap_hip.h"
#include "gemm_api.h"
#include "kernels.h"
#include "shared.h"
#include "layout.h"
#include <vector>

using namespace CC_NS;

namespace {

#define CC_TIMED(site, st, expr)                 \
    do {                                         \
        cc_shared::ProfScope _ps(site, st);      \
        int _e = (expr);                         \
        if (_e != CC_OK) return _e;              \
    } while (0)

struct TileScope {
    int old;
    bool on;
    explicit TileScope(int mode) : old(cc_shared::g_gemm_tile_mode), on(mode != -2) { if (on) cc_shared::g_gemm_tile_mode = mode; }
    ~TileScope() { if (on) cc_shared::g_gemm_tile_mode = old; }
};
inline int env_tile(const char* name) {
// ... 85 lines not shown
        if (save) {
            need = std::max(need, x3_img(M, 3 * D));
            need = std::max(need, std::max(x3_img(M, D) + x3_img(M, Hm), x3_img(M, 3 * D) + x3_img(M, D)));
            need = std::max(need, x3_img(Mb, PD) + x3_img(Mb, c->E));
        }
        w.x3_bytes = need;
        w.x3 = cv.take<char>(need);
    }
    w.bytes = cv.bytes();
}

struct MapperPass {
    hipStream_t st;
    MapperOff o;
    MapperWS w;
    Call cx;
    int D, PP, S, M, H, hd, Hm, PD;
    MapperPass(const cc_mapper_cfg* c, int B, int save, void* ws, void* stream)
        : st(S_(stream)), o(c), D(c->D), PP(c->W * c->P), S(PP + c->L), M(B * S), H(c->H), hd(c->D / c->H), Hm(c->Hm), PD(c->P * c->D) {
        mapper_carve(c, B, save, ws, w);
        cx = call_of(st, w);
    }
};

static bool x3_img_on() {
    static const bool on = []() { const char* e = cc_lab_env("CC_X3_IMG"); return !e || atoi(e) != 0; }();
    return on;
}
static bool lm_exp_form(const cc_gpt2_shape* s) {
    static const bool env = []() { const char* e = cc_lab_env("CC_LM_EXPFORM"); return !e || atoi(e) != 0; }();
    if (CC_OP == 0) return env;
    if (CC_OP == 2) return env && x3_img_on() && s->mode == 1;
    return false;
}
static Act lm_logits(const cc_gpt2_cfg* c, const cc_gpt2_shape* s, act_t* logits16) { return Act(logits16, (kX3 && lm_exp_form(s)) ? c->Vp : 0); }

struct Gpt2WS {
    float* x[MAX_LAYERS + 1];
    float* x1[MAX_LAYERS];
    act_t *qkv[MAX_LAYERS], *u[MAX_LAYERS];
    Act xn1[MAX_LAYERS], xn2[MAX_LAYERS], att[MAX_LAYERS], hact[MAX_LAYERS];
    float *lse[MAX_LAYERS], *mean1[MAX_LAYERS], *rstd1[MAX_LAYERS], *mean2[MAX_LAYERS], *rstd2[MAX_LAYERS];
    act_t* hf16;
    float *meanf, *rstdf;
    int *target, *row_map;
    int* keep;
    act_t* logits16;
    float *pmax, *psum, *tgt_logit, *lse_row, *row_loss;
    float *cref, *lmfac;
    act_t* hfs16;
    float* dx32;
    Act dx16, dx16b, du16, dqkv16;
    act_t *dhf16, *dxn16, *datt16;
    float* wg_scratch;
    float* red;
    void* scat;
    float* adelta;
    char* x3;
    size_t x3_bytes;
    size_t bytes;
};

void gpt2_carve(const cc_gpt2_cfg* c, const cc_gpt2_shape* s, int cap, void* ws, Gpt2WS& w) {
    Carver cv(ws);
    const int B = s->B, T = s->T, hd = c->D / c->H;
    const size_t M = (size_t)B * T, D = c->D, Mc = (size_t)B * cap;
    const bool keep = s->mode >= 1, full = s->mode >= 2;
    const auto take_img = [&](size_t n) { return cv.take<act_t>(n * ((kX3 && !full) ? 3 : 2) / 2); };
    const bool img = kX3 && !full && x3_img_on();
    const bool bimg = img && keep && s->p_resid == 0.f && s->p_attn == 0.f && s->p_embd == 0.f;
    const int xw = img ? (int)D : 0, attw = (img && attn_fwd_can_image(T, hd)) ? (int)D : 0, hw = img ? 4 * (int)D : 0;
    const int dxw = bimg ? (int)D : 0, dqw = (bimg && attn_bwd_can_image(T, hd)) ? 3 * (int)D : 0;
    const int nx = keep ? c->NL + 1 : 2;
    float* xb[MAX_LAYERS + 1];
    for (int i = 0; i < nx; i++) xb[i] = cv.take<float>(M * D);
    for (int l = 0; l <= c->NL; l++) w.x[l] = keep ? xb[l] : xb[l & 1];
    for (int l = 0; l < c->NL; l++) {
        const bool k0 = keep || l == 0, f0 = full || l == 0;
        w.x1[l] = k0 ? cv.take<float>(M * D) : w.x1[0];
        w.qkv[l] = k0 ? cv.take<act_t>(M * 3 * D) : w.qkv[0];
        w.u[l] = k0 ? cv.take<act_t>(M * 4 * D) : w.u[0];
        w.lse[l] = k0 ? cv.take<float>((size_t)B * c->H * T) : w.lse[0];
        w.mean1[l] = k0 ? cv.take<float>(M) : w.mean1[0];
        w.rstd1[l] = k0 ? cv.take<float>(M) : w.rstd1[0];
        w.mean2[l] = k0 ? cv.take<float>(M) : w.mean2[0];
        w.rstd2[l] = k0 ? cv.take<float>(M) : w.rstd2[0];
        w.xn1[l] = f0 ? Act(take_img(M * D), xw) : w.xn1[0];
        w.xn2[l] = f0 ? Act(take_img(M * D), xw) : w.xn2[0];
        w.att[l] = k0 ? Act(take_img(M * D), attw) : w.att[0];
        w.hact[l] = f0 ? Act(take_img(M * 4 * D), hw) : w.hact[0];
    }
    const size_t Mh = std::max(M, Mc);
    w.hf16 = cv.take<act_t>(Mh * D);
    w.meanf = cv.take<float>(Mh);
    w.rstdf = cv.take<float>(Mh);
    w.target = cv.take<int>(Mh);
    w.row_map = cv.take<int>(Mh);
    w.keep = nullptr;
    if (keep) {
        const int npart = c->Vp / 64;
        w.logits16 = take_img(Mc * c->Vp);
        w.pmax = cv.take<float>(Mc * npart);
        w.psum = cv.take<float>(Mc * npart);
        w.tgt_logit = cv.take<float>(Mc);
        w.lse_row = cv.take<float>(Mc);
        w.row_loss = cv.take<float>(Mc);
        w.cref = cv.take<float>(Mc);
        w.lmfac = cv.take<float>(2 * Mc);
        w.hfs16 = full ? cv.take<act_t>(Mc * D) : nullptr;
        w.dx32 = cv.take<float>(M * D);
        w.dx16 = Act(take_img(M * D), dxw);
        w.dx16b = full ? Act(cv.take<act_t>(M * D)) : w.dx16;
        w.dhf16 = cv.take<act_t>(Mc * D);
        w.du16 = Act(take_img(M * 4 * D), hw);
        w.dxn16 = cv.take<act_t>(M * D);
        w.datt16 = cv.take<act_t>(M * D);
        w.dqkv16 = Act(take_img(M * 3 * D), dqw);
        w.wg_scratch = full ? cv.take<float>(WGRAD_SCRATCH_BYTES / sizeof(float)) : nullptr;
        w.red = full ? cv.take<float>(RED_SCRATCH_FLOATS) : nullptr;
        w.scat = full ? cv.take<char>(scatter_ws_bytes((int)Mc, (int)D)) : nullptr;
        w.adelta = cv.take<float>((size_t)B * c->H * T);
    } else {
        w.wg_scratch = nullptr; w.adelta = nullptr; w.red = nullptr; w.scat = nullptr;
        w.logits16 = nullptr; w.pmax = w.psum = w.tgt_logit = w.lse_row = w.row_loss = nullptr;
        w.cref = w.lmfac = nullptr; w.hfs16 = nullptr;
        w.dx32 = nullptr; w.dx16 = w.dx16b = w.du16 = w.dqkv16 = Act(); w.dhf16 = w.dxn16 = w.datt16 = nullptr;
        if (Mc > 0) {
            const int npart = c->Vp / 64;
            w.pmax = cv.take<float>(Mc * npart);
            w.psum = cv.take<float>(Mc * npart);
            w.tgt_logit = cv.take<float>(Mc);
            w.lse_row = cv.take<float>(Mc);
            w.keep = cv.take<int>(Mc);
        }
    }
    w.x3 = nullptr; w.x3_bytes = 0;
    if (kX3) {
        size_t need = x3_img(Mh, 4 * D);
        if (keep) need = std::max(need, x3_img(Mc, c->Vp));
        if (full) need = std::max(need, std::max(x3_img(M, D) + x3_img(M, 4 * D), x3_img(Mc, c->Vp) + x3_img(Mc, D)));
        w.x3_bytes = need;
        w.x3 = cv.take<char>(need);
    }
    w.bytes = cv.bytes();
}

struct Gpt2Pass {
    hipStream_t st;
    Gpt2Off o;
    Gpt2WS w;
    Call cx;
    int D, M, H, hd;
    Gpt2Pass(const cc_gpt2_cfg* c, const cc_gpt2_shape* s, int cap, void* ws, void* stream)
        : st(S_(stream)), o(c), D(c->D), M(s->B * s->T), H(c->H), hd(c->D / c->H) {
        gpt2_carve(c, s, cap, ws, w);
        cx = call_of(st, w);
    }
};

}

extern "C" {

int CC_API(cc_mapper_bwd_range)(const cc_mapper_cfg* c, int32_t B, const float* w32, const uint16_t* w16, void* ws, const float* dout, float* g32,
                        int32_t l_hi, int32_t l_lo, void* stream);
int CC_API(cc_gpt2_bwd_range)(const cc_gpt2_cfg* c, const cc_gpt2_shape* s, const float* w32, const uint16_t* w16, void* ws, const int64_t* tokens,
                      float* dprefix, float* g32, int32_t l_hi, int32_t l_lo, void* stream);

int64_t CC_API(cc_mapper_param_count)(const cc_mapper_cfg* cfg) {
    if (!mapper_cfg_ok(cfg)) return CC_ERR_SHAPE;
    return MapperOff(cfg).total;
}

int CC_API(cc_mapper_param_offsets)(const cc_mapper_cfg* cfg, int64_t* offs) {
    if (!mapper_cfg_ok(cfg) || !offs) return CC_ERR_SHAPE;
    const MapperOff o(cfg);
    *offs++ = o.lin_w; *offs++ = o.lin_b; *offs++ = o.prefix; *offs++ = o.pos;
    for (int l = 0; l < cfg->N; l++) offs = put_layer(offs, o.layer(l));
    return CC_OK;
// ... 336 lines not shown
    if (!gpt2_cfg_ok(c) || !shape_ok(c, s) || s->mode < 1 || s->L < 1 || !w32 || !w16 || !ws || !tokens || !stats) return CC_ERR_ARG;
    const int cap = s->T - s->L;
    if (cap != s->cap) return CC_ERR_SHAPE;
    Gpt2Pass ps(c, s, cap, ws, stream);
    auto& [st, o, w, cx, D, M, H, hd] = ps;
    const int Mc = s->B * cap, npart = c->Vp / 64;
    if (hipMemsetAsync(stats, 0, 2 * sizeof(float), st) != hipSuccess) return CC_ERR_LAUNCH;
    CC_TRY(ce_targets(reinterpret_cast<const long long*>(tokens), w.target, w.row_map, s->B, cap, s->L, s->T, st));
    CC_TRY(ln_fwd(w.x[c->NL], D, w.row_map, w32 + o.lnf_w, w32 + o.lnf_b, w.hf16, nullptr, w.meanf, w.rstdf, Mc, D, st));
    const bool ef = lm_exp_form(s);
    const op16_t* wte_rows = kX3 ? reinterpret_cast<const op16_t*>(w32 + o.wte) : W16(w16, o.wte);
    if (ef) CC_TRY(lm_tgt_ref(w.hf16, wte_rows, D, w.target, w.cref, Mc, st));
    CC_TIMED(CC_SITE_LMHEAD_FWD, st, gemm_lmhead(w.hf16, D, W16(w16, o.wte), D, Mc, c->Vp, c->V, D, lm_logits(c, s, w.logits16), c->Vp, w.pmax, w.psum, npart, w.target, w.tgt_logit, cx,
                                                 ef ? w.cref : nullptr));
    CC_TRY(ce_rows(w.pmax, w.psum, npart, w.target, ef ? w.cref : w.tgt_logit, w.lse_row, w.row_loss, stats, Mc, st));
    return CC_OK;
}

int CC_API(cc_lmhead_score)(const cc_gpt2_cfg* c, const cc_gpt2_shape* s, const float* w32, const uint16_t* w16, void* ws, const int64_t* tokens,
                    int32_t ignore_zero, float* token_logprob, float* sample_stats, void* stream) {
    if (!gpt2_cfg_ok(c) || !shape_ok(c, s) || s->mode != 0 || s->L < 1 || !w32 || !w16 || !ws || !tokens || !token_logprob || !sample_stats)
        return CC_ERR_ARG;
    const int cap = s->T - s->L;
    if (cap < 1 || cap != s->cap) return CC_ERR_SHAPE;
    Gpt2Pass ps(c, s, cap, ws, stream);
    auto& [st, o, w, cx, D, M, H, hd] = ps;
    const int Mc = s->B * cap, npart = c->Vp / 64;
    CC_TRY(ce_targets(reinterpret_cast<const long long*>(tokens), w.target, w.row_map, s->B, cap, s->L, s->T, st));
    CC_TRY(score_keep(reinterpret_cast<const long long*>(tokens), w.keep, Mc, ignore_zero, st));
    CC_TRY(ln_fwd(w.x[c->NL], D, w.row_map, w32 + o.lnf_w, w32 + o.lnf_b, w.hf16, nullptr, w.meanf, w.rstdf, Mc, D, st));
    CC_TIMED(CC_SITE_LMHEAD_FWD, st, gemm_lmhead_score(w.hf16, D, W16(w16, o.wte), D, Mc, c->Vp, c->V, D, w.pmax, w.psum, npart, w.target, w.tgt_logit, cx));
    return score_rows(w.pmax, w.psum, npart, w.keep, w.tgt_logit, w.lse_row, token_logprob, sample_stats, s->B, cap, st);
}

int CC_API(cc_lmhead_ce_bwd)(const cc_gpt2_cfg* c, const cc_gpt2_shape* s, const float* w32, const uint16_t* w16, void* ws, const float* denom,
                     const float* loss_scale, float* g32, void* stream) {
    if (!gpt2_cfg_ok(c) || !shape_ok(c, s) || s->mode < 1 || !w32 || !w16 || !ws || !denom || (s->mode == 2 && !g32)) return CC_ERR_ARG;
    const int cap = s->T - s->L;
    Gpt2Pass ps(c, s, cap, ws, stream);
    auto& [st, o, w, cx, D, M, H, hd] = ps;
    const int Mc = s->B * cap;
    const bool full = s->mode == 2;
    const bool ef = lm_exp_form(s);
    const LmFix fix{w.lmfac, w.target, kX3 ? reinterpret_cast<const op16_t*>(w32 + o.wte) : W16(w16, o.wte)};
    if (ef) CC_TRY(lm_rowfac(w.cref, w.lse_row, w.target, denom, loss_scale, w.lmfac, Mc, st));
    const Act lg = lm_logits(c, s, w.logits16);
    ActIn dlog = lg;
    op16_t* dimg = (kX3 && !ef && !full && x3_img_on()) ? x3_scratch_block(cx, x3_img(Mc, c->Vp)) : nullptr;
    if (dimg) dlog = ActIn(reinterpret_cast<const act_t*>(dimg), c->Vp);
    if (!ef) CC_TRY(ce_dlogits(w.logits16, c->Vp, c->V, w.target, w.lse_row, denom, loss_scale, Mc, st, dimg));
    const auto lm_dgrad = [&]() {
        auto& [st, o, w, cx, D, M, H, hd] = ps;
        const int rc = gemm_nt_deepk(dlog, c->Vp, W16(w16, o.total + o.wte), c->Vp, Mc, D, c->Vp, w.dhf16, D, reinterpret_cast<float*>(w.du16.p),
                                     (size_t)M * 4 * D * sizeof(act_t), cx, ef ? &fix : nullptr);
        if (rc != CC_ERR_SHAPE) return rc;
        const int rc2 = gemm_bf16out(0, 0, dlog, c->Vp, W16(w16, o.total + o.wte), c->Vp, Mc, D, c->Vp, w.dhf16, D, nullptr, 0, nullptr, cx);
        return (rc2 != CC_OK || !ef) ? rc2 : lm_dgrad_fix(w.dhf16, w.lmfac, w.target, fix.wte, D, Mc, st);
    };
    CC_TIMED(CC_SITE_LMHEAD_DGRAD, st, lm_dgrad());
    if (full) {
        if (ef) {
            CC_TRY(lm_scale_rows(w.hf16, w.lmfac, w.hfs16, D, Mc, st));
            CC_TRY(gemm_wgrad(lg, c->Vp, w.hfs16, D, c->Vp, D, Mc, g32 + o.wte, D, w.wg_scratch, cx));
            ScatterSrc oh;
            oh.ids32 = w.target; oh.act = w.hf16; oh.fac = w.lmfac;
            CC_TRY(scatter_rows(oh, Mc, D, c->Vp, g32 + o.wte, w.scat, st));
        } else {
            CC_TRY(gemm_wgrad(lg, c->Vp, w.hf16, D, c->Vp, D, Mc, g32 + o.wte, D, w.wg_scratch, cx));
        }
    }
    if (hipMemsetAsync(w.dx32, 0, (size_t)M * D * sizeof(float), st) != hipSuccess) return CC_ERR_LAUNCH;
    const size_t dx16_bytes = (size_t)M * D * (w.dx16.img ? 3 * sizeof(op16_t) : sizeof(act_t));
    if (hipMemsetAsync(w.dx16.p, 0, dx16_bytes, st) != hipSuccess) return CC_ERR_LAUNCH;
    CC_TRY(ln_bwd(w.dhf16, w.x[c->NL], D, w.row_map, w.meanf, w.rstdf, w32 + o.lnf_w, nullptr, w.dx32, w.dx16, full ? g32 + o.lnf_w : nullptr,
                  full ? g32 + o.lnf_b : nullptr, Mc, D, cx));
    return CC_OK;
}

int CC_API(cc_lmhead_put_x)(const cc_gpt2_cfg* c, const cc_gpt2_shape* s, void* ws, const float* x, void* stream) {
    if (!gpt2_cfg_ok(c) || !shape_ok(c, s) || !ws || !x) return CC_ERR_ARG;
    Gpt2Pass ps(c, s, s->T - s->L, ws, stream);
    const size_t bytes = (size_t)s->B * s->T * c->D * sizeof(float);
    return hipMemcpyAsync(ps.w.x[c->NL], x, bytes, hipMemcpyDeviceToDevice, ps.st) == hipSuccess ? CC_OK : CC_ERR_LAUNCH;
}

int CC_API(cc_lmhead_get)(const cc_gpt2_cfg* c, const cc_gpt2_shape* s, void* ws, int32_t field, void* dst, int64_t dst_bytes, void* stream) {
    if (!gpt2_cfg_ok(c) || !shape_ok(c, s) || !ws || !dst || field < CC_LM_LSE || field > CC_LM_DX32) return CC_ERR_ARG;
    if (s->T - s->L < 1) return CC_ERR_SHAPE;
    Gpt2Pass ps(c, s, s->T - s->L, ws, stream);
    const Gpt2WS& w = ps.w;
    const size_t Mc = (size_t)s->B * (s->T - s->L), M = (size_t)s->B * s->T, D = c->D;
    const void* src = nullptr;
    size_t bytes = 0;
    switch (field) {
        case CC_LM_LSE: src = w.lse_row; bytes = Mc * sizeof(float); break;
        case CC_LM_TGT: src = (s->mode >= 1 && lm_exp_form(s)) ? w.cref : w.tgt_logit; bytes = Mc * sizeof(float); break;
        case CC_LM_ROW_LOSS: src = w.row_loss; bytes = Mc * sizeof(float); break;
        case CC_LM_HF: src = w.hf16; bytes = Mc * D * sizeof(act_t); break;
        case CC_LM_DHF: src = w.dhf16; bytes = Mc * D * sizeof(act_t); break;
        default: src = w.dx32; bytes = M * D * sizeof(float); break;
    }
    if (!src) return CC_ERR_STATE;
    if (dst_bytes < 0 || (size_t)dst_bytes != bytes) return CC_ERR_SHAPE;
    return hipMemcpyAsync(dst, src, bytes, hipMemcpyDeviceToDevice, ps.st) == hipSuccess ? CC_OK : CC_ERR_LAUNCH;
}

int CC_API(cc_gpt2_logits_bwd)(const cc_gpt2_cfg* c, const cc_gpt2_shape* s, const float* w32, const uint16_t* w16, void* ws, const float* dlogits,
// ... 217 lines not shown
#if CC_OP == 2
    if (!src || !dst || rows < 0 || width < 0 || ld < width || (form != 0 && form != 1)) return CC_ERR_ARG;
    return x3_split_rows(src, (size_t)ld, dst, rows, width, form, S_(stream));
#else
    (void)src; (void)ld; (void)rows; (void)width; (void)form; (void)dst; (void)stream;
    return CC_ERR_ARG;
#endif
}

int CC_API(cc_gemm_act)(int32_t al, int32_t bl, const void* A, int32_t a_img, int32_t lda, const uint16_t* B, int32_t ldb, int32_t M, int32_t N, int32_t K,
                void* C, int32_t c_img, int32_t ldc, const float* bias, int32_t act, void* pre, void* x3, int64_t x3_bytes, void* stream) {
    if (!hook_operands_ok(al, bl, A, a_img, lda, B, ldb, M, N, K) || !C || !al16(C) || !al16(pre) || !al16(bias) || ldc < N || act < 0 || act > 3 ||
        !hook_c_img_ok(c_img, N))
        return CC_ERR_ARG;
    Call cx{S_(stream)};
    hook_scratch(cx, x3, x3_bytes);
    return gemm_bf16out(al, bl, ActIn(static_cast<const act_t*>(A), a_img), lda, B, ldb, M, N, K, Act(static_cast<act_t*>(C), c_img), ldc, bias, act,
                        static_cast<act_t*>(pre), cx);
}

int CC_API(cc_gemm_resid)(int32_t al, int32_t bl, const void* A, int32_t a_img, int32_t lda, const uint16_t* B, int32_t ldb, int32_t M, int32_t N, int32_t K,
                  float* out, const float* res, int32_t ld, const float* bias, float p, uint64_t seed, int32_t site, int32_t layer, void* x3,
                  int64_t x3_bytes, void* stream) {
    if (!hook_operands_ok(al, bl, A, a_img, lda, B, ldb, M, N, K) || !out || !res || !al16(out) || !al16(res) || !al16(bias) || ld < N || site < 0 ||
        site > 3 || layer < 0 || layer > 255 || p < 0.f || p >= 1.f)
        return CC_ERR_ARG;
    Call cx{S_(stream)};
    hook_scratch(cx, x3, x3_bytes);
    return gemm_resid(al, bl, ActIn(static_cast<const act_t*>(A), a_img), lda, B, ldb, M, N, K, out, res, ld, bias, cx,
                      make_drop(p, seed, (unsigned)site, (unsigned)layer));
}

int CC_API(cc_gemm_dact)(int32_t al, int32_t bl, const void* A, int32_t a_img, int32_t lda, const uint16_t* B, int32_t ldb, int32_t M, int32_t N, int32_t K,
                 void* C, int32_t c_img, int32_t ldc, const void* aux, int32_t act, void* x3, int64_t x3_bytes, void* stream) {
    if (!hook_operands_ok(al, bl, A, a_img, lda, B, ldb, M, N, K) || !C || !aux || !al16(C) || !al16(aux) || ldc < N || act < 1 || act > 3 ||
        !hook_c_img_ok(c_img, N))
        return CC_ERR_ARG;
    Call cx{S_(stream)};
    hook_scratch(cx, x3, x3_bytes);
    return gemm_dact(al, bl, ActIn(static_cast<const act_t*>(A), a_img), lda, B, ldb, M, N, K, Act(static_cast<act_t*>(C), c_img), ldc,
                     static_cast<const act_t*>(aux), act, cx);
}

int CC_API(cc_gemm_f32)(int32_t al, int32_t bl, const void* A, int32_t a_img, int32_t lda, const uint16_t* B, int32_t ldb, int32_t M, int32_t N, int32_t K,
                float* C, int32_t ldc, const float* bias, int32_t mode, float alpha, int32_t ksplit, void* x3, int64_t x3_bytes, void* stream) {
    if (!hook_operands_ok(al, bl, A, a_img, lda, B, ldb, M, N, K) || !C || !al16(C) || !al16(bias) || ldc < N || mode < 0 || mode > 2 || ksplit < 1 ||
        (bias && mode != 0))
        return CC_ERR_ARG;
    Call cx{S_(stream)};
    hook_scratch(cx, x3, x3_bytes);
    return gemm_f32out(al, bl, ActIn(static_cast<const act_t*>(A), a_img), lda, B, ldb, M, N, K, C, ldc, bias, mode, alpha, ksplit, cx);
}

int CC_API(cc_gemm_wgrad_split)(const void* X, int32_t x_img, int32_t ldx, const float* Y, int32_t ldy, int32_t Mw, int32_t Nw, int32_t K, float* dW,
                     int32_t ldw, float* scratch, void* x3, int64_t x3_bytes, void* stream) {
#if CC_OP == 2
    if (!X || !Y || !dW || !al16(X) || !al16(Y) || !al16(dW) || Mw <= 0 || Nw <= 0 || K <= 0 || x_img < 0 || (!x_img && ldx < Mw) || ldy < Nw || ldw < Nw)
        return CC_ERR_ARG;
    Call cx{S_(stream)};
    hook_scratch(cx, x3, x3_bytes);
    return gemm_wgrad(ActIn(static_cast<const act_t*>(X), x_img), ldx, Y, ldy, Mw, Nw, K, dW, ldw, scratch, cx);
#else
    (void)X; (void)x_img; (void)ldx; (void)Y; (void)ldy; (void)Mw; (void)Nw; (void)K; (void)dW; (void)ldw; (void)scratch; (void)x3; (void)x3_bytes; (void)stream;
    return CC_ERR_ARG;
#endif
}

}
```

clipcap_amd/csrc/gemm.hip.h:

```cpp
#pragma once
#include <cstdlib>
#include <type_traits>
#include "common.hip.h"
#include "gemm_api.h"

namespace CC_NS {

constexpr int G_BM = 128, G_BN = 128, G_BK = 64, G_THREADS = 256;
constexpr int G_TILE_BYTES = G_BM * G_BK * 2;
constexpr int G_EPI_LD = 68;

struct GemmShape {
    int M, N, K;
    int lda, ldb;
    int k_chunk;
    int group_m;
    int stagger;
    int flags = 0;
};

__device__ __forceinline__ int g_lds_off(int row, int chunk) {
    return row * 128 + (((chunk ^ (row >> 1) ^ ((row >> 4) & 3)) & 7) << 4);
}

// ... 1231 lines not shown
        for (int t = 0; t < nk; t++) {
            if (t >= 1) H_MFMA(t - 1);
            H_STAMP(4)
            H_SEGEND();
            H_STAMP(6)
#if CC_STAG_READ_FIRST
            H_LOADF(t);
            __builtin_amdgcn_sched_barrier(0);
            if (t + H_NS - 1 < nk) H_ISSUE(t + H_NS - 1, false);
            H_STAMP(1)
#else
            if (t + H_NS - 1 < nk) H_ISSUE(t + H_NS - 1, false);
            H_STAMP(1)
            H_LOADF(t);
#endif
#ifdef CC_STAMP
            asm volatile("s_waitcnt lgkmcnt(0)" ::: "memory");
#endif
            H_STAMP(2)
            H_WAIT(t, NJ);
            H_STAMP(5)
            H_SEGEND();
            H_STAMP(3)
        }
        H_MFMA(nk - 1); H_SEGEND();
    }
    H_STAMP(0)
    if constexpr (epi_acc_init<Epi>::value && !kAccInit) {
        Epi e2 = epi;
        e2.acc_init = false;
        gemm_epilogue_regs<Epi, NI, NJ>(acc, lane, m0 + arow, n0 + bcol, e2);
    } else {
        gemm_epilogue_regs<Epi, NI, NJ>(acc, lane, m0 + arow, n0 + bcol, epi);
    }
    H_STAMP(7)
    H_STAMP_OUT
}
template <class Epi, int NJ, bool TT = false, int NI = 8, bool X3F = false>
__global__ __launch_bounds__(512, 1) void gemm_nt_stag256_kernel(const op16_t* __restrict__ A, const op16_t* __restrict__ B, GemmShape g, Epi epi) {
    extern __shared__ __attribute__((aligned(1024))) char smem[];
    gemm_stag256_body<Epi, NJ, TT, NI, X3F>(A, B, g, epi, xcd_remap(blockIdx.x, gridDim.x), (int)blockIdx.z, smem);
}
#undef H_STAMP_DECL
#undef H_STAMP
#undef H_STAMP_OUT
#undef H_ISSUE
#undef H_LOADF
#undef H_MFMA
#undef H_LOADF_LO
#undef H_MFMA_LO
#undef H_SEGEND
#undef H_WAIT

#include "gemm_q4.hip.h"

__device__ __forceinline__ HTTFrag g_tt_read(const char* tile, int lane_base, int xoff) {
    typedef __attribute__((address_space(3))) const char* lp_t;
    const unsigned a = (unsigned)(size_t)(lp_t)(tile + lane_base + xoff);
    HTTFrag f;
    asm volatile("ds_read_b64_tr_b16 %0, %1" : "=v"(f.lo) : "v"(a) : "memory");
    asm volatile("ds_read_b64_tr_b16 %0, %1 offset:1024" : "=v"(f.hi) : "v"(a) : "memory");
    return f;
}
__device__ __forceinline__ void glds_tile_tt(const op16_t* __restrict__ base, int ld, int cols, int c0, int k0, char* lds, int wave, int lane) {
#pragma unroll
    for (int i = 0; i < 4; i++) {
        const int seg = wave + 4 * i;
        const int kr = seg * 4 + (lane >> 4);
        const int c = (lane & 15) ^ (h_tt_g(kr) << 1);
        const op16_t* src = base + (size_t)(k0 + kr) * ld + min(c0 + c * 8, cols - 8);
        __builtin_amdgcn_global_load_lds((gptr_t)src, (lptr_t)(lds + seg * 1024), 16, 0, 0);
    }
}
template <class Epi>
__device__ __forceinline__ void gemm_tt_glds4_body(const op16_t* __restrict__ A, const op16_t* __restrict__ B, const GemmShape& g, const Epi& epi,
                                                   int tile, int zslice, char* smemt) {
    const int tid = threadIdx.x, lane = tid & 63;
    const int wave = __builtin_amdgcn_readfirstlane(tid >> 6);
    const int wm = wave >> 1, wn = wave & 1;
    const int tiles_n = (g.N + G_BN - 1) / G_BN, tiles_m = (g.M + G_BM - 1) / G_BM;
    int tm, tn;
    tile_coords(tile, tiles_m, tiles_n, g.group_m, tm, tn);
    const int m0 = tm * G_BM, n0 = tn * G_BN;
    const int kbeg = zslice * g.k_chunk;
    const int nk = (min(g.K, kbeg + g.k_chunk) - kbeg) / G_BK;
    f32x4 acc[4][4];
#pragma unroll
    for (int i = 0; i < 4; i++)
#pragma unroll
        for (int j = 0; j < 4; j++) acc[i][j] = f32x4{0.f, 0.f, 0.f, 0.f};
#define GT_ISSUE(T)                                                                                                      \
    {                                                                                                                    \
        char* st_ = smemt + ((T) & 3) * 2 * G_TILE_BYTES;                                                                \
        glds_tile_tt(A, g.lda, g.M, m0, kbeg + (T)*G_BK, st_, wave, lane);                                               \
        glds_tile_tt(B, g.ldb, g.N, n0, kbeg + (T)*G_BK, st_ + G_TILE_BYTES, wave, lane);                                \
    }
    GT_ISSUE(0);
    if (nk > 1) GT_ISSUE(1);
    if (nk > 2) GT_ISSUE(2);
    const int frow = lane & 15, fchunk = lane >> 4;
    const int tt_base = (8 * fchunk + (frow >> 2)) * 256 + ((frow & 3) >> 1) * 16 + (frow & 1) * 8;
    const int tt_gx = h_tt_g(8 * fchunk + (frow >> 2)) << 1;
    HTTFrag fa[2][4], fb[2][4];
#define GT_READ(SET, CUR, KS)                                                                                            \
    {                                                                                                                    \
        _Pragma("unroll") for (int i_ = 0; i_ < 4; i_++) fa[SET][i_] = g_tt_read((CUR) + (KS)*32 * 256, tt_base, ((wm * 8 + 2 * i_) ^ tt_gx) << 4);                 \
// ... 167 lines not shown
                float m0, m1;
                drop_mul_pair(drop, (unsigned)o + e, m0, m1);
                y[e] *= m0; y[e + 1] *= m1;
            }
        }
        const float r[8] = {r0.x, r0.y, r0.z, r0.w, r1.x, r1.y, r1.z, r1.w};
        store_sum(o, r, y);
    }
    bool acc_init = false;
    __device__ __forceinline__ bool init_from_input() const { return acc_init; }
    __device__ __forceinline__ void init4(int row, int col, f32x4& a) const {
        if (row >= M || col >= Ns) return;
        const float4 r = *reinterpret_cast<const float4*>(res + (size_t)row * ld + col);
        a[0] = r.x; a[1] = r.y; a[2] = r.z; a[3] = r.w;
    }
    static constexpr bool kPre = true;
    __device__ __forceinline__ void pre4(int row, int col, f32x4& a) const {
        if (acc_init || row >= M || col >= Ns) return;
        const size_t o = (size_t)row * ld + col;
        const float4 r = *reinterpret_cast<const float4*>(res + o);
        if (drop.thresh) {
            float4 b = make_float4(0, 0, 0, 0);
            if (bias) b = *reinterpret_cast<const float4*>(bias + col);
            float m0, m1, m2, m3;
            drop_mul_pair(drop, (unsigned)o, m0, m1);
            drop_mul_pair(drop, (unsigned)o + 2, m2, m3);
            a[0] = r.x + m0 * (a[0] + b.x);
            a[1] = r.y + m1 * (a[1] + b.y);
            a[2] = r.z + m2 * (a[2] + b.z);
            a[3] = r.w + m3 * (a[3] + b.w);
            return;
        }
        a[0] += r.x; a[1] += r.y; a[2] += r.z; a[3] += r.w;
    }
    __device__ __forceinline__ void bias8(int col, float (&b)[8]) const { load_bias8(drop.thresh ? nullptr : bias, col, Ns, b); }
    __device__ __forceinline__ void fin(int row, int col, float (&v)[8], const float (&b)[8]) const {
        if (row >= M || col >= Ns) return;
        store_sum((size_t)row * ld + col, v, b);
    }
  private:
    __device__ __forceinline__ void store_sum(size_t o, const float (&x)[8], const float (&y)[8]) const {
        *reinterpret_cast<float4*>(out + o) = make_float4(x[0] + y[0], x[1] + y[1], x[2] + y[2], x[3] + y[3]);
        *reinterpret_cast<float4*>(out + o + 4) = make_float4(x[4] + y[4], x[5] + y[5], x[6] + y[6], x[7] + y[7]);
    }
};

struct EpiF32 {
    float* C;
    const float* bias;
    int ldc, M, Ns;
    int mode;
    float alpha;
    size_t zstride = 0;
    __device__ __forceinline__ void operator()(int row, int col, float (&v)[8]) const {
        if (row >= M || col >= Ns) return;
        float* p = C + (size_t)row * ldc + col + (mode == 3 ? blockIdx.z * zstride : 0);
        if (mode == 2) {
#pragma unroll
            for (int e = 0; e < 8; e++) __hip_atomic_fetch_add(p + e, alpha * v[e], __ATOMIC_RELAXED, __HIP_MEMORY_SCOPE_AGENT);
            return;
        }
        float4 o0 = make_float4(alpha * v[0], alpha * v[1], alpha * v[2], alpha * v[3]);
        float4 o1 = make_float4(alpha * v[4], alpha * v[5], alpha * v[6], alpha * v[7]);
        if (mode == 0 && bias) {
            const float4 b0 = *reinterpret_cast<const float4*>(bias + col);
            const float4 b1 = *reinterpret_cast<const float4*>(bias + col + 4);
            o0.x += b0.x; o0.y += b0.y; o0.z += b0.z; o0.w += b0.w; o1.x += b1.x; o1.y += b1.y; o1.z += b1.z; o1.w += b1.w;
        }
        if (mode == 1) {
            const float4 c0 = *reinterpret_cast<const float4*>(p);
            const float4 c1 = *reinterpret_cast<const float4*>(p + 4);
            o0.x += c0.x; o0.y += c0.y; o0.z += c0.z; o0.w += c0.w; o1.x += c1.x; o1.y += c1.y; o1.z += c1.z; o1.w += c1.w;
        }
        *reinterpret_cast<float4*>(p) = o0;
        *reinterpret_cast<float4*>(p + 4) = o1;
    }
    static constexpr bool kPre = true;
    __device__ __forceinline__ void pre4(int row, int col, f32x4& a) const {
        a[0] *= alpha; a[1] *= alpha; a[2] *= alpha; a[3] *= alpha;
        if (mode != 1 || row >= M || col >= Ns) return;
        const float4 c = *reinterpret_cast<const float4*>(C + (size_t)row * ldc + col);
        a[0] += c.x; a[1] += c.y; a[2] += c.z; a[3] += c.w;
    }
    __device__ __forceinline__ void bias8(int col, float (&b)[8]) const { load_bias8(mode == 0 ? bias : nullptr, col, Ns, b); }
    __device__ __forceinline__ void fin(int row, int col, float (&v)[8], const float (&b)[8]) const {
        if (row >= M || col >= Ns) return;
        float* p = C + (size_t)row * ldc + col + (mode == 3 ? blockIdx.z * zstride : 0);
        if (mode == 2) {
#pragma unroll
            for (int e = 0; e < 8; e++) __hip_atomic_fetch_add(p + e, v[e], __ATOMIC_RELAXED, __HIP_MEMORY_SCOPE_AGENT);
            return;
        }
        *reinterpret_cast<float4*>(p) = make_float4(v[0] + b[0], v[1] + b[1], v[2] + b[2], v[3] + b[3]);
        *reinterpret_cast<float4*>(p + 4) = make_float4(v[4] + b[4], v[5] + b[5], v[6] + b[6], v[7] + b[7]);
    }
};

template <int ACT = -1>
struct EpiDActT {
    act_t* C;
    const act_t* aux;
    int ldc, M, Ns;
    int act;
    int img = 0;
    __device__ __forceinline__ int act_() const { return ACT >= 0 ? ACT : act; }
    __device__ __forceinline__ void operator()(int row, int col, float (&v)[8]) const {
        if (row >= M || col >= Ns) return;
        const size_t o = (size_t)row * ldc + col;
        float a[8];
        act_ld8(aux + o, a);
        if (act_() == 1) {
#pragma unroll
            for (int e = 0; e < 8; e++) v[e] = a[e] > 0.f ? v[e] : 0.f;
        } else if (act_() == 3) {
#pragma unroll
            for (int e = 0; e < 8; e++) v[e] *= a[e];
        } else {
#pragma unroll
            for (int e = 0; e < 8; e++) v[e] *= gelu_new_grad(a[e]);
        }
        epi_store8(C, ldc, row, col, v, img);
    }
    typedef act_raw8 StripAux;
    __device__ __forceinline__ act_raw8 load_aux(int row, int col) const {
        return (row < M && col < Ns) ? act_ldraw8(aux + (size_t)row * ldc + col) : act_zero8();
    }
    __device__ __forceinline__ void operator()(int row, int col, float (&v)[8], const act_raw8& ax) const {
        if (row >= M || col >= Ns) return;
        float a[8];
        act_unpack8(ax, a);
        if (act_() == 1) {
#pragma unroll
            for (int e = 0; e < 8; e++) v[e] = a[e] > 0.f ? v[e] : 0.f;
        } else if (act_() == 3) {
#pragma unroll
            for (int e = 0; e < 8; e++) v[e] *= a[e];
        } else {
#pragma unroll
            for (int e = 0; e < 8; e++) v[e] *= gelu_new_grad(a[e]);
        }
        epi_store8(C, ldc, row, col, v, img);
    }
    static constexpr bool kPre = true;
    __device__ __forceinline__ void pre4(int row, int col, f32x4& a) const {
        if (row >= M || col >= Ns) return;
        float x[4];
        act_unpack4(act_ldraw4(aux + (size_t)row * ldc + col), x[0], x[1], x[2], x[3]);
#pragma unroll
        for (int e = 0; e < 4; e++) a[e] = act_() == 1 ? (x[e] > 0.f ? a[e] : 0.f) : (act_() == 3 ? a[e] * x[e] : a[e] * gelu_new_grad(x[e]));
// ... 203 lines not shown
            *reinterpret_cast<float4*>(p + 4) = make_float4(va[4], va[5], va[6], va[7]);
        }
        if (cb < Ns) {
            float* p = C + (size_t)row * ldc + cb;
            *reinterpret_cast<float4*>(p) = make_float4(vb[0], vb[1], vb[2], vb[3]);
            *reinterpret_cast<float4*>(p + 4) = make_float4(vb[4], vb[5], vb[6], vb[7]);
        }
    }
};
struct EpiLMHeadScore {
    float* pmax;
    float* psum;
    const int* target;
    float* tgt_logit;
    int M, N, V, npart;
    __device__ __forceinline__ void operator()(int row, int col, float (&v)[8]) const {
        const bool ok = row < M && col < N;
        float m, s;
        row_stats8(col, V, v, m, s);
        if (!ok) return;
        if ((col & 63) == 0) put_partials(*this, row, col, m, s);
        const int t = target[row] - col;
        if (t >= 0 && t < 8) tgt_logit[row] = v[t];
    }
    typedef int RowAux;
    __device__ __forceinline__ int load_row(int row) const { return row < M ? target[row] : -1; }
    __device__ __forceinline__ void strip(int row, int ca, int cb, float (&va)[8], float (&vb)[8], int t) const {
        float m, s;
        row_stats_strip<false, true>(ca, cb, V, va, vb, m, s);
        if (row >= M) return;
        if ((ca & 63) == 0 && ca < N) put_partials(*this, row, ca, m, s);
        if (t >= ca && t < ca + 8 && ca < N) tgt_logit[row] = va[t - ca];
        if (t >= cb && t < cb + 8 && cb < N) tgt_logit[row] = vb[t - cb];
    }
};
template <> struct epi_row_strip<EpiLogits> { static constexpr bool value = true; };
template <> struct epi_row_strip<EpiLMHead> { static constexpr bool value = true; };
template <> struct epi_row_strip<EpiLMHeadScore> { static constexpr bool value = true; };
template <> struct epi_row_strip<EpiLMHeadExp> { static constexpr bool value = true; };

template <auto Kernel, class... Args>
inline void launch_dyn(dim3 grid, dim3 block, size_t shmem, hipStream_t st, const Args&... args) {
    static bool attr = false;
    if (!attr) { (void)hipFuncSetAttribute((const void*)Kernel, hipFuncAttributeMaxDynamicSharedMemorySize, (int)shmem); attr = true; }
    hipLaunchKernelGGL(Kernel, grid, block, shmem, st, args...);
}
template <class Epi>
inline int launch_gemm_s64(const op16_t* A, int lda, const op16_t* B, int ldb, int M, int N, int K, int ksplit, int nj, const Epi& epi, int* ks_eff,
                           hipStream_t st, const op16_t* Bimg = nullptr);
inline bool x3_fused_on() {
    static const bool on = kX3 && !(cc_lab_env("CC_X3_FUSED") && atoi(cc_lab_env("CC_X3_FUSED")) == 0);
    return on;
}
template <class Epi>
inline int launch_gemm(int al, int bl, const op16_t* A, int lda, const op16_t* B, int ldb, int M, int N, int K,
                       int ksplit, const Epi& epi, hipStream_t st, int tile = -2, int group_m = 0) {
    if (M <= 0 || N <= 0 || K <= 0) return CC_OK;
    if ((lda & 7) || (ldb & 7) || ((uintptr_t)A & 15) || ((uintptr_t)B & 15)) return CC_ERR_SHAPE;
    if (al == 0 && (K & 7)) return CC_ERR_SHAPE;
    if (bl == 0 && (K & 7)) return CC_ERR_SHAPE;
    if (al == 1 && (M & 7)) return CC_ERR_SHAPE;
    if (bl == 1 && (N & 7)) return CC_ERR_SHAPE;
    if constexpr (!epi_row_strip<Epi>::value && !epi_strip_aux<Epi>::value) {
        if (g_gemm_s64 > 0 && al == 0 && bl == 0 && (K % G_BK) == 0 && M <= 1024)
            return launch_gemm_s64(A, lda, B, ldb, M, N, K, ksplit, g_gemm_s64, epi, nullptr, st);
    }
    GemmShape g;
    g.M = M; g.N = N; g.K = K; g.lda = lda; g.ldb = ldb;
    static const int env_group = []() { const char* e = cc_lab_env("CC_GROUP_M"); return e ? atoi(e) : 0; }();
    g.group_m = env_group > 0 ? env_group : (group_m > 0 ? group_m : 8);
    static const int env_stagger = []() { const char* e = cc_lab_env("CC_GEMM_STAGGER"); return e ? atoi(e) : 0; }();
    g.stagger = env_stagger;
    if (ksplit < 1) ksplit = 1;
    int kt = (K + G_BK - 1) / G_BK;
    int per = (kt + ksplit - 1) / ksplit;
    ksplit = (kt + per - 1) / per;
    g.k_chunk = per * G_BK;
    dim3 grid(((M + G_BM - 1) / G_BM) * ((N + G_BN - 1) / G_BN), 1, ksplit);
    const int s256 = tile != -2 ? tile : g_gemm_tile_mode;
    int nj = 0, ni = 8;
    constexpr bool can160 = !kX3 && !epi_row_strip<Epi>::value && !epi_is_dact<Epi>::value;
    constexpr bool zsplit_ok = std::is_same<Epi, EpiF32>::value;
    if (al == 0 && bl == 0 && (K % H_BK) == 0 && (ksplit == 1 || (zsplit_ok && tile > 0)) && s256 != 0) {
        const long tm = (M + H_BM - 1) / H_BM, t128 = (long)grid.x;
        const long t256 = tm * ((N + 255) / 256), t192 = tm * ((N + 191) / 192), t320 = (long)((M + 319) / 320) * ((N + 255) / 256);
        const double c128 = t128 <= 256 ? 16384.0 / 0.75 : (double)((t128 + 511) / 512) * 32768.0;
        const double c256 = (double)((t256 + 255) / 256) * 65536.0 / 1.2, c192 = (double)((t192 + 255) / 256) * 49152.0 / 1.15;
        const double c320 = (double)((t320 + 255) / 256) * 81920.0 / 1.3;
        constexpr bool can192 = !epi_row_strip<Epi>::value;
        constexpr bool can320 = !epi_is_dact<Epi>::value;
        const long t160 = (long)((M + 159) / 160) * ((N + 255) / 256);
        const double c160 = (double)((t160 + 255) / 256) * 40960.0 / 1.1;
        static const bool s160_on = []() { const char* e = cc_lab_env("CC_GEMM_S160"); return !e || atoi(e) != 0; }();
        if (can160 && (s256 == 6 || s256 == 7 || (s256 < 0 && s160_on && ksplit == 1 && c160 < 0.98 * c128 && c160 < 0.98 * c256 && c160 < 0.98 * c320 && (!can192 || c160 < 0.98 * c192)))) { nj = 4; ni = 5; }
        else if (s256 == 5 || (can320 && s256 < 0 && c320 < 0.98 * c128 && c320 < c256 && (!can192 || c320 < c192))) { nj = 4; ni = 10; }
        else if (s256 == 4 || (s256 < 0 && c256 < 0.98 * c128 && (!can192 || c256 <= c192))) nj = 4;
        else if (can192 && (s256 == 3 || (s256 < 0 && c192 < 0.98 * c128))) nj = 3;
    }
    if (nj) {
        const int bm = 32 * ni;
        const size_t sh = (size_t)H_NS * (bm + H_BN) * H_BK * 2;
        const dim3 gr((unsigned)(((M + bm - 1) / bm) * ((N + 64 * nj - 1) / (64 * nj))), 1, (unsigned)ksplit);
        if (nj == 4 && ni == 8) launch_dyn<gemm_nt_stag256_kernel<Epi, 4, false, 8>>(gr, dim3(512), sh, st, A, B, g, epi);
        else if (nj == 4 && ni == 5) {
            if constexpr (can160) {
                static const bool q4_on = []() { const char* e = cc_lab_env("CC_GEMM_Q4"); return !e || atoi(e) != 0; }();
                const bool fits32 = (size_t)M * (size_t)lda * 2 < 0xffff0000ull && (size_t)N * (size_t)ldb * 2 < 0xffff0000ull;
                const int ns = (K % 192 == 0 && K >= 384) ? 3 : ((K % 128 == 0 && K >= 256) ? 2 : 0);
                static const bool q4_last = []() { const char* e = cc_lab_env("CC_Q4_LAST"); return !e || atoi(e) != 0; }();
                g.flags = q4_last ? 0 : 1;
                if (ns && fits32 && ksplit == 1 && s256 != 6 && (q4_on || s256 == 7)) {
                    static const int ncu = []() { int n = 0, dev = 0; (void)hipGetDevice(&dev); (void)hipDeviceGetAttribute(&n, hipDeviceAttributeMultiprocessorCount, dev); return n > 0 ? n : 256; }();
                    const int tiles = ((M + 159) / 160) * ((N + 255) / 256);
                    const dim3 gq((unsigned)(tiles < ncu ? tiles : ncu));
                    if (ns == 3) {
                        launch_dyn<gemm_nt_q4_kernel<Epi, 5, 3>>(gq, dim3(256), (size_t)3 * (160 + 256) * 128, st, A, B, g, epi);
                    } else {
                        launch_dyn<gemm_nt_q4_kernel<Epi, 5, 2>>(gq, dim3(256), (size_t)2 * (160 + 256) * 128, st, A, B, g, epi);
                    }
                } else launch_dyn<gemm_nt_stag256_kernel<Epi, 4, false, 5>>(gr, dim3(512), sh, st, A, B, g, epi);
            }
        }
        else if (nj == 4) launch_dyn<gemm_nt_stag256_kernel<Epi, 4, false, 10>>(gr, dim3(512), sh, st, A, B, g, epi);
        else if constexpr (!epi_row_strip<Epi>::value) {
            bool fused = false;
            if constexpr (kX3) {
                const bool x3f_on = x3_fused_on();
                if (x3f_on && (K % (3 * H_BK)) == 0 && ksplit <= K / (3 * H_BK)) {
                    launch_dyn<gemm_nt_stag256_kernel<Epi, 3, false, 8, true>>(gr, dim3(512), sh, st, A, B, g, epi);
                    fused = true;
                }
            }
            if (!fused) launch_dyn<gemm_nt_stag256_kernel<Epi, 3, false, 8>>(gr, dim3(512), sh, st, A, B, g, epi);
        }
    } else
#ifdef CC_GEMM_ABLATION
    static const int abl = []() { const char* e = cc_lab_env("CC_GEMM_ABL"); return e ? atoi(e) : 0; }();
    if (al == 0 && bl == 0 && (K % G_BK) == 0 && abl == 1) { hipLaunchKernelGGL((gemm_nt_glds_kernel<Epi, 1>), grid, dim3(G_THREADS), 0, st, A, B, g, epi); }
    else if (al == 0 && bl == 0 && (K % G_BK) == 0 && abl == 2) { hipLaunchKernelGGL((gemm_nt_glds_kernel<Epi, 2>), grid, dim3(G_THREADS), 0, st, A, B, g, epi); }
    else if (al == 0 && bl == 0 && (K % G_BK) == 0 && abl == 4) { hipLaunchKernelGGL((gemm_nt_glds_kernel<Epi, 4>), grid, dim3(G_THREADS), 0, st, A, B, g, epi); }
    else if (al == 0 && bl == 0 && (K % G_BK) == 0 && abl == 5) { hipLaunchKernelGGL((gemm_nt_glds_kernel<Epi, 5>), grid, dim3(G_THREADS), 0, st, A, B, g, epi); }
    else if (al == 0 && bl == 0 && (K % G_BK) == 0 && abl == 6) { hipLaunchKernelGGL((gemm_nt_glds_kernel<Epi, 6>), grid, dim3(G_THREADS), 0, st, A, B, g, epi); }
    else
#endif
    if (al == 0 && bl == 0 && (K % G_BK) == 0 && (long)grid.x * grid.z <= 256 && g_gemm_tile_mode != 0 && K / (int)grid.z >= 4 * G_BK) {
        constexpr size_t sh4 = (size_t)8 * G_TILE_BYTES;
        bool fused = false;
        if constexpr (kX3) {
            const bool x3f_on = x3_fused_on();
            if (g_gemm_small_x2 && x3f_on && ksplit == 1 && (K % (3 * G_BK)) == 0) {
                launch_dyn<gemm_nt_glds4x2_x3f_kernel<Epi>>(grid, dim3(2 * G_THREADS), sh4, st, A, B, g, epi);
                fused = true;
            }
        }
        if (fused) {}
        else if (g_gemm_small_x2) launch_dyn<gemm_nt_glds4x2_kernel<Epi>>(grid, dim3(2 * G_THREADS), sh4, st, A, B, g, epi);
        else launch_dyn<gemm_nt_glds4_kernel<Epi>>(grid, dim3(G_THREADS), sh4, st, A, B, g, epi);
    } else if (al == 0 && bl == 0 && (K % G_BK) == 0) {
        bool fused = false;
        if constexpr (kX3) {
            const bool x3f_on = x3_fused_on();
            if (x3f_on && ksplit == 1 && (K % (3 * G_BK)) == 0) {
                hipLaunchKernelGGL((gemm_nt_glds_x3f_kernel<Epi>), grid, dim3(G_THREADS), 0, st, A, B, g, epi);
                fused = true;
            }
        }
        if (!fused) hipLaunchKernelGGL((gemm_nt_glds_kernel<Epi>), grid, dim3(G_THREADS), 0, st, A, B, g, epi);
// ... 196 lines not shown
```

clipcap_amd/csrc/gemm_api.h:

```cpp
#pragma once
#include "common.hip.h"
#include "shared.h"

namespace CC_NS {
int gemm_bf16out(int al, int bl, ActIn A, int lda, const op16_t* B, int ldb, int M, int N, int K, Act C, int ldc,
                 const float* bias, int act, act_t* pre, Call& cx);
int gemm_resid(int al, int bl, ActIn A, int lda, const op16_t* B, int ldb, int M, int N, int K, float* out, const float* res,
               int ld, const float* bias, Call& cx, Drop drop = Drop());
int gemm_f32out(int al, int bl, ActIn A, int lda, const op16_t* B, int ldb, int M, int N, int K, float* C, int ldc,
                const float* bias, int mode, float alpha, int ksplit, Call& cx);
int gemm_dact(int al, int bl, ActIn A, int lda, const op16_t* B, int ldb, int M, int N, int K, Act C, int ldc,
              const act_t* aux, int act, Call& cx);
int gemm_lmhead(ActIn A, int lda, const op16_t* B, int ldb, int M, int Vp, int V, int K, Act C, int ldc, float* pmax,
                float* psum, int npart, const int* target, float* tgt_logit, Call& cx, const float* cref = nullptr);
int gemm_lmhead_score(ActIn A, int lda, const op16_t* B, int ldb, int M, int Vp, int V, int K, float* pmax, float* psum, int npart,
                      const int* target, float* tgt_logit, Call& cx);

int gemm_logits_part(ActIn A, int lda, const op16_t* B, int ldb, int M, int Ns, int V, int K, float* C, int ldc, float* pmax, float* psum,
                     int npart, Call& cx);

#if CC_OP == 2
const op16_t* x3_operand(Call& cx, const float* src, size_t ld, int rows, int width, int form, bool first, int* rc);
#endif
inline op16_t* x3_scratch_block(const Call& cx, size_t bytes) { return (cx.x3 && bytes <= cx.x3_bytes) ? reinterpret_cast<op16_t*>(cx.x3) : nullptr; }
inline int nt_operand(Call& cx, ActIn A, int al, int bl, int M, int& lda, int& ldb, int& K, const op16_t*& A16) {
#if CC_OP == 2
    if (al || bl || (A.img && A.img != K)) return CC_ERR_ARG;
    if (A.img) {
        A16 = reinterpret_cast<const op16_t*>(A.p);
    } else {
        int rc = CC_OK;
        A16 = x3_operand(cx, A.p, (size_t)lda, M, K, 0, true, &rc);
        if (!A16) return rc;
    }
    lda = 3 * K; ldb = 3 * ldb; K = 3 * K;
#else
    if (A.img) return CC_ERR_ARG;
    A16 = A.p;
#endif
    return CC_OK;
}
constexpr size_t WGRAD_SCRATCH_BYTES = size_t(96) << 20;
struct WgradBatch {
    struct Item { const float* slabs; size_t slab; int ks, Nw; float* dW; int ldw; size_t n4; };
    Item it[8];
    int n = 0;
    size_t used = 0;
    bool defer = false;
    struct Deferred { const op16_t* X; const op16_t* Y; int ldx, ldy, Mw, Nw, K; float* dW; int ldw; };
    Deferred d[32];
    int nd = 0;
    int cap = 4;
    bool direct = false;
    float* scratch = nullptr;
};
int wgrad_flush(WgradBatch& b, hipStream_t st);
int gemm_wgrad(ActIn X, int ldx, const act_t* Y, int ldy, int Mw, int Nw, int K, float* dW, int ldw, float* scratch,
               Call& cx, WgradBatch* batch = nullptr);
struct SkinnyFuse {
    const float* ln_gamma = nullptr;
    const float* ln_beta = nullptr;
    act_t* ln_out16 = nullptr;
    act_t* kcache = nullptr;
    act_t* vcache = nullptr;
    int Tn = 1, pos0 = 0, ctx_max = 0;
    const op16_t* bimg = nullptr;
};
int skinny_image(const op16_t* W, op16_t* img, int N, int K, hipStream_t st);
int gemm_nt_skinny(ActIn A, int lda, const op16_t* B, int ldb, int M, int N, int K, const float* bias, int act, const float* res,
                   float* out32, act_t* out16, int ldo, float* scratch, size_t scratch_bytes, Call& cx,
                   const SkinnyFuse* fuse = nullptr);
struct LmFix { const float* fac; const int* target; const op16_t* wte; };
int gemm_nt_deepk(ActIn A, int lda, const op16_t* B, int ldb, int M, int N, int K, act_t* out16, int ldo, float* scratch,
                  size_t scratch_bytes, Call& cx, const LmFix* fix = nullptr);
int skinny_single_min_tiles();
bool gemm_nt_skinny_can_fuse(int M, int N, int K, size_t scratch_bytes);
}
```

clipcap_amd/csrc/gemm_inst_f32.hip:

```cpp
#include "gemm.hip.h"
#include <algorithm>
#include "gemm_api.h"
namespace CC_NS {
static int gemm_f32out_op(int al, int bl, const op16_t* A, int lda, const op16_t* B, int ldb, int M, int N, int K, float* C, int ldc,
                          const float* bias, int mode, float alpha, int ksplit, hipStream_t st) {
    if ((ldc & 3) || (N & 7)) return CC_ERR_SHAPE;
    if (ksplit > 1 && mode != 2) return CC_ERR_ARG;
    EpiF32 e{C, bias, ldc, M, N, mode, alpha};
    return launch_gemm(al, bl, A, lda, B, ldb, M, N, K, ksplit, e, st);
}
int gemm_f32out(int al, int bl, ActIn A, int lda, const op16_t* B, int ldb, int M, int N, int K, float* C, int ldc,
                const float* bias, int mode, float alpha, int ksplit, Call& cx) {
    const hipStream_t st = cx.st;
    cc_shared::ProfScope _all(cc_shared::SITE_ALL_GEMMS, st, 2.0 * M * N * (double)K);
    const op16_t* A16;
    const int rca = nt_operand(cx, A, al, bl, M, lda, ldb, K, A16);
    if (rca != CC_OK) return rca;
    return gemm_f32out_op(al, bl, A16, lda, B, ldb, M, N, K, C, ldc, bias, mode, alpha, ksplit, st);
}
__global__ __launch_bounds__(256) void k_slab_reduce(const float* __restrict__ slabs, size_t slab_elems, int ks, int Nw, float* __restrict__ dW,
                                                     int ldw, size_t n4) {
    for (size_t i = (size_t)blockIdx.x * blockDim.x + threadIdx.x; i < n4; i += (size_t)gridDim.x * blockDim.x) {
        float4 a = reinterpret_cast<const float4*>(slabs)[i];
        for (int s = 1; s < ks; s++) {
// ... 333 lines not shown
    if (!f.ln_out16) return;
    const float mu = block_sum256(s1, red) / N;
    float q = 0.f;
#pragma unroll
    for (int it = 0; it < MAXV; it++) {
        const int c = threadIdx.x * 4 + it * 1024;
        if (c < N) { const float a = v[it].x - mu, b = v[it].y - mu, c2 = v[it].z - mu, d = v[it].w - mu; q += a * a + b * b + c2 * c2 + d * d; }
    }
    const float rs = rsqrtf(block_sum256(q, red) / N + 1e-5f);
#pragma unroll
    for (int it = 0; it < MAXV; it++) {
        const int c = threadIdx.x * 4 + it * 1024;
        if (c < N) {
            const float4 g = lg_[it], b = lb_[it];
            act_st4(f.ln_out16 + (size_t)row * N + c, (v[it].x - mu) * rs * g.x + b.x, (v[it].y - mu) * rs * g.y + b.y,
                    (v[it].z - mu) * rs * g.z + b.z, (v[it].w - mu) * rs * g.w + b.w);
        }
    }
}

int skinny_single_min_tiles() {
    static const int v = []() { const char* e = cc_lab_env("CC_SKINNY_SINGLE"); return e ? atoi(e) : 60; }();
    return v;
}
bool gemm_nt_skinny_can_fuse(int M, int N, int K, size_t scratch_bytes) {
    return M > 0 && N > 0 && (N & 7) == 0 && N <= 3072 && (K % G_BK) == 0 && scratch_bytes >= (size_t)M * N * sizeof(float);
}

__global__ __launch_bounds__(256) void k_deepk_finish_lm(const float* __restrict__ slabs, size_t slab_elems, int ks, int M, int N, LmFix f,
                                                         act_t* __restrict__ out16, int ldo) {
    const size_t n8 = (size_t)M * (N >> 3);
    for (size_t i = (size_t)blockIdx.x * blockDim.x + threadIdx.x; i < n8; i += (size_t)gridDim.x * blockDim.x) {
        const int row = (int)(i / (N >> 3)), col = (int)(i % (N >> 3)) * 8;
        const size_t e = (size_t)row * N + col;
        float v[8] = {0, 0, 0, 0, 0, 0, 0, 0}, b[8];
        for (int s = 0; s < ks; s++) {
            const float4 a = *reinterpret_cast<const float4*>(slabs + s * slab_elems + e);
            const float4 c = *reinterpret_cast<const float4*>(slabs + s * slab_elems + e + 4);
            v[0] += a.x; v[1] += a.y; v[2] += a.z; v[3] += a.w; v[4] += c.x; v[5] += c.y; v[6] += c.z; v[7] += c.w;
        }
        const float r = f.fac[2 * row], w = f.fac[2 * row + 1];
#if CC_OP == 2
        act_ld8(reinterpret_cast<const float*>(f.wte) + (size_t)f.target[row] * N + col, b);
#else
        unpack8(*reinterpret_cast<const uint4*>(f.wte + (size_t)f.target[row] * N + col), b);
#endif
#pragma unroll
        for (int k = 0; k < 8; k++) v[k] = r * v[k] - w * b[k];
        act_st8(out16 + (size_t)row * ldo + col, v);
    }
}

int gemm_nt_deepk(ActIn Aa, int lda, const op16_t* B, int ldb, int M, int N, int K, act_t* out16, int ldo, float* scratch,
                  size_t scratch_bytes, Call& cx, const LmFix* fix) {
    const hipStream_t st = cx.st;
    static const int knob = []() { const char* e = cc_lab_env("CC_DEEPK"); return e ? atoi(e) : -1; }();
    if (knob == 0 || g_gemm_tile_mode == 0 || !scratch || (N & 7) || (ldo & 7) || (K % 64) || (lda & 7) || (ldb & 7)) return CC_ERR_SHAPE;
    const long tiles = (long)((M + H_BM - 1) / H_BM) * ((N + H_BN - 1) / H_BN);
    const size_t slab = (size_t)M * N;
    int ks = knob > 0 ? knob : (int)(256 / (tiles > 0 ? tiles : 1));
    const size_t fit = scratch_bytes / (slab * sizeof(float));
    if ((size_t)ks > fit) ks = (int)fit;
    if (ks > K / 2048) ks = K / 2048;
    if (ks < 2 || tiles > 128) return CC_ERR_SHAPE;
    cc_shared::ProfScope _all(cc_shared::SITE_ALL_GEMMS, st, 2.0 * M * N * (double)K);
    const op16_t* A;
    const int rca = nt_operand(cx, Aa, 0, 0, M, lda, ldb, K, A);
    if (rca != CC_OK) return rca;
    EpiF32 e{scratch, nullptr, N, M, N, 3, 1.0f};
    e.zstride = slab;
    int tile = 4, tiles_n = (N + H_BN - 1) / H_BN;
    long tl = tiles;
    if (kX3 && x3_fused_on() && (K % (3 * H_BK)) == 0) {
        tile = 3;
        tiles_n = (N + 191) / 192;
        tl = (long)((M + H_BM - 1) / H_BM) * tiles_n;
        const int nc = K / (3 * H_BK);
        long best = -1;
        int best_ks = ks;
        for (int k2 = 1; k2 <= 8 && (size_t)k2 <= fit && k2 <= nc / 32; k2++) {
            const long cost = ((tl * k2 + 255) / 256) * ((nc + k2 - 1) / k2);
            if (best < 0 || cost < best) { best = cost; best_ks = k2; }
        }
        ks = best_ks;
        if (ks < 2) return CC_ERR_SHAPE;
    }
    const int gm = std::max(1, (int)((tl + 7) / 8) / tiles_n);
    const int rc = launch_gemm(0, 0, A, lda, B, ldb, M, N, K, ks, e, st, tile, gm);
    if (rc != CC_OK) return rc;
    const int kt = K / G_BK, per = (kt + ks - 1) / ks, ks_eff = (kt + per - 1) / per;
    const size_t n8 = (size_t)M * (N >> 3);
    if (fix)
        hipLaunchKernelGGL(k_deepk_finish_lm, dim3((int)std::min<size_t>((n8 + 255) / 256, 2048)), dim3(256), 0, st, scratch, slab, ks_eff, M, N, *fix,
                           out16, ldo);
    else
        hipLaunchKernelGGL(k_splitk_finish, dim3((int)std::min<size_t>((n8 + 255) / 256, 2048)), dim3(256), 0, st, scratch, slab, ks_eff, M, N, nullptr, 0,
                           nullptr, nullptr, out16, ldo);
    return hipGetLastError() == hipSuccess ? CC_OK : CC_ERR_LAUNCH;
}

#ifdef CC_EXPERIMENTS
int skinny_image(const op16_t* W, op16_t* img, int N, int K, hipStream_t st) {
    if ((N % 64) || (K % 64) || !W || !img) return CC_ERR_SHAPE;
    hipLaunchKernelGGL(k_skinny_image, dim3(1024), dim3(256), 0, st, W, img, N, K);
    return hipGetLastError() == hipSuccess ? CC_OK : CC_ERR_LAUNCH;
}
#endif

int gemm_nt_skinny(ActIn Aa, int lda, const op16_t* B, int ldb, int M, int N, int K, const float* bias, int act, const float* res,
                   float* out32, act_t* out16, int ldo, float* scratch, size_t scratch_bytes, Call& cx, const SkinnyFuse* fuse) {
    const hipStream_t st = cx.st;
    cc_shared::ProfScope _all(cc_shared::SITE_ALL_GEMMS, st, 2.0 * M * N * (double)K);
    if ((N & 7) || (ldo & 7)) return CC_ERR_SHAPE;
    const op16_t* A;
    const int rca = nt_operand(cx, Aa, 0, 0, M, lda, ldb, K, A);
    if (rca != CC_OK) return rca;
    const int tiles = ((M + G_BM - 1) / G_BM) * ((N + G_BN - 1) / G_BN);
    const size_t slab = (size_t)M * N;
    const bool can_slab = scratch && slab && (K % G_BK) == 0 && scratch_bytes >= slab * sizeof(float);
    const bool fused = fuse && (fuse->ln_out16 || fuse->kcache);
    const op16_t* bimg = (fuse && !kX3) ? fuse->bimg : nullptr;
    const bool s64 = g_gemm_s64 != 0 && (K % G_BK) == 0 && M <= 640 && tiles <= 256 && (lda & 7) == 0 && (ldb & 7) == 0;
    int ks;
    if (s64) {
        const int t64 = ((M + 63) / 64) * ((N + 63) / 64);
        ks = t64 >= 160 ? 1 : 256 / t64;
        const int kmax = K / (4 * G_BK);
        if (ks > kmax) ks = kmax;
    } else {
        ks = 384 / (tiles > 0 ? tiles : 1);
        const int kmax = K / (2 * G_BK);
        if (ks > kmax) ks = kmax;
        if (!fused && tiles >= skinny_single_min_tiles()) ks = 1;
    }
    if (ks < 1) ks = 1;
    if (can_slab) { const size_t fit = scratch_bytes / (slab * sizeof(float)); if ((size_t)ks > fit) ks = (int)fit; }
    static const bool s80_on = []() { const char* e = cc_lab_env("CC_SKINNY_80"); return !e || atoi(e) != 0; }();
    auto s64_form = [&](int slices) {
        const int t64 = ((M + 63) / 64) * ((N + 63) / 64), t80 = ((M + 79) / 80) * ((N + 63) / 64);
        if (g_gemm_s64 == 1 || K / G_BK / (slices > 0 ? slices : 1) < 14) return 1;
        if ((long)t64 * slices <= 256) return 3;
        return (s80_on && slices <= 1 && t80 <= 256) ? 4 : 1;
    };
    if (!can_slab || (ks <= 1 && !fused)) {
        if (fused) return CC_ERR_SHAPE;
        if (s64) {
            const int form = s64_form(1);
            if (res) { EpiResid e{out32, res, bias, ldo, M, N}; return launch_gemm_s64(A, lda, B, ldb, M, N, K, 1, form, e, nullptr, st, bimg); }
            if (out16) {
                static const bool spec_on = []() { const char* v = cc_lab_env("CC_EPI_SPEC"); return !v || atoi(v) != 0; }();
                if (spec_on && act == 0) { EpiBF16Plain e{out16, bias, ldo, M, N}; return launch_gemm_s64(A, lda, B, ldb, M, N, K, 1, form, e, nullptr, st, bimg); }
                if (spec_on && act == 2) { EpiBF16T<2, 0> e{out16, nullptr, bias, ldo, M, N, 2}; return launch_gemm_s64(A, lda, B, ldb, M, N, K, 1, form, e, nullptr, st, bimg); }
                EpiBF16 e{out16, nullptr, bias, ldo, M, N, act};
                return launch_gemm_s64(A, lda, B, ldb, M, N, K, 1, form, e, nullptr, st, bimg);
            }
            EpiF32 e{out32, bias, ldo, M, N, 0, 1.0f};
            return launch_gemm_s64(A, lda, B, ldb, M, N, K, 1, form, e, nullptr, st, bimg);
        }
        if (res) { EpiResid e{out32, res, bias, ldo, M, N}; return launch_gemm(0, 0, A, lda, B, ldb, M, N, K, 1, e, st); }
        if (out16) { EpiBF16 e{out16, nullptr, bias, ldo, M, N, act}; return launch_gemm(0, 0, A, lda, B, ldb, M, N, K, 1, e, st); }
        EpiF32 e{out32, bias, ldo, M, N, 0, 1.0f};
        return launch_gemm(0, 0, A, lda, B, ldb, M, N, K, 1, e, st);
    }
    EpiF32 e{scratch, nullptr, N, M, N, 3, 1.0f};
    e.zstride = slab;
    int rc = s64 ? launch_gemm_s64(A, lda, B, ldb, M, N, K, ks, s64_form(ks), e, nullptr, st, bimg) : launch_gemm(0, 0, A, lda, B, ldb, M, N, K, ks, e, st);
    if (rc != CC_OK) return rc;
    const int kt = K / G_BK, per = (kt + ks - 1) / ks, ks_eff = (kt + per - 1) / per;
    if (N <= 3072 && (N & 3) == 0) {
        SkinnyFuse f = fuse ? *fuse : SkinnyFuse{};
        hipLaunchKernelGGL(k_splitk_finish_row, dim3(M), dim3(256), 0, st, scratch, slab, ks_eff, M, N, bias, act, res, out32, out16, ldo, f);
    } else {
        if (fused) return CC_ERR_SHAPE;
        const size_t n8 = (size_t)M * (N >> 3);
        hipLaunchKernelGGL(k_splitk_finish, dim3((int)std::min<size_t>((n8 + 255) / 256, 2048)), dim3(256), 0, st, scratch, slab, ks_eff, M, N, bias,
                           act, res, out32, out16, ldo);
    }
    return hipGetLastError() == hipSuccess ? CC_OK : CC_ERR_LAUNCH;
}
}
```

clipcap_amd/csrc/gemm_q4.hip.h:

```cpp

#include "gemm_q4_asm.inc"
#if CC_OP == 1
#define Q4_MFMA "v_mfma_f32_16x16x32_f16"
#else
#define Q4_MFMA "v_mfma_f32_16x16x32_bf16"
#endif

template <int N> __device__ __forceinline__ void q4_wait_vm() {
    static_assert(N == 13 || N == 16 || N == 26, "(NS - 1) x per-stage DMA count of the generated forms");
    if constexpr (N == 13) asm volatile("s_waitcnt vmcnt(13)" ::: "memory");
    else if constexpr (N == 16) asm volatile("s_waitcnt vmcnt(16)" ::: "memory");
    else asm volatile("s_waitcnt vmcnt(26)" ::: "memory");
}

template <class Epi, int NI, int NS, int VAR = 0>
__global__ __launch_bounds__(256, 1) void gemm_nt_q4_kernel(const op16_t* __restrict__ A, const op16_t* __restrict__ B, GemmShape g, Epi epi) {
    static_assert((NI == 8 && NS == 2) || (NI == 5 && (NS == 2 || NS == 3)), "forms generated by tools/gen_q4_asm.py");
    extern __shared__ __attribute__((aligned(1024))) char smem[];
    constexpr int SBM = 32 * NI, SA = SBM * 128, SSTAGE = (SBM + 256) * 128;
    constexpr int NA = NI, NB = 8, ND = NA + NB;
    const int tid = threadIdx.x, lane = tid & 63;
    const int wave = __builtin_amdgcn_readfirstlane(tid >> 6);
    const int wm = wave >> 1, wn = wave & 1;
    const int tiles_n = (g.N + 255) / 256, tiles_m = (g.M + SBM - 1) / SBM, ntiles = tiles_m * tiles_n;
    const int nbig = g.K / 64;
    const unsigned lds0 = (unsigned)(size_t)(lptr_t)smem;
    const int frow = lane & 15;
    unsigned q4_la[NS][2], q4_lb[NS][2];
#pragma unroll
    for (int b = 0; b < NS; b++)
#pragma unroll
        for (int kk = 0; kk < 2; kk++) {
            const unsigned ch = (unsigned)(((kk * 4 + (lane >> 4)) ^ ((frow >> 1) & 7)) << 4);
            q4_la[b][kk] = lds0 + (unsigned)(b * SSTAGE + (wm * 16 * NI + frow) * 128) + ch;
            q4_lb[b][kk] = lds0 + (unsigned)(b * SSTAGE + SA + (wn * 128 + frow) * 128) + ch;
        }
    const unsigned q4_slds = (unsigned)__builtin_amdgcn_readfirstlane((int)(lds0 + wave * 1024));
    const unsigned q4_nmain = (unsigned)(nbig / NS - 2);
    const op16_t* q4_pa = A;
    const op16_t* q4_pb = B;
    const int drow = lane >> 3;
    const unsigned dchunk = (unsigned)(((lane & 7) ^ (4 * (wave & 1) + (lane >> 4))) << 4);
    unsigned offA[NA], offB[NB], noffA[NA], noffB[NB];
    unsigned toA[NA], toB[NB], q4_cnt;
#define Q4_OFFSETS(TILE, OA, OB, M0, N0)                                                                                 \
    {                                                                                                                    \
        int tm_, tn_;                                                                                                    \
        tile_coords(xcd_remap((TILE), ntiles), tiles_m, tiles_n, g.group_m, tm_, tn_);                                   \
        M0 = tm_ * SBM; N0 = tn_ * 256;                                                                                  \
        _Pragma("unroll") for (int i_ = 0; i_ < NA; i_++)                                                                \
            OA[i_] = (unsigned)min(M0 + (wave + 4 * i_) * 8 + drow, g.M - 1) * (unsigned)(g.lda * 2) + dchunk;            \
        _Pragma("unroll") for (int j_ = 0; j_ < NB; j_++)                                                                \
            OB[j_] = (unsigned)min(N0 + (wave + 4 * j_) * 8 + drow, g.N - 1) * (unsigned)(g.ldb * 2) + dchunk;            \
    }
#define Q4_ACC_INIT(M0, N0)                                                                                              \
    {                                                                                                                    \
        _Pragma("unroll") for (int h_ = 0; h_ < 2; h_++) _Pragma("unroll") for (int i_ = 0; i_ < NI; i_++)               \
            _Pragma("unroll") for (int j_ = 0; j_ < 4; j_++) acc[h_][i_][j_] = f32x4{0.f, 0.f, 0.f, 0.f};                \
        if constexpr (epi_acc_init<Epi>::value) {                                                                        \
            if (epi.init_from_input()) {                                                                                 \
                const int q_ = lane >> 4, rl_ = lane & 15;                                                               \
                _Pragma("unroll") for (int h_ = 0; h_ < 2; h_++) _Pragma("unroll") for (int i_ = 0; i_ < NI; i_++)       \
                    _Pragma("unroll") for (int j_ = 0; j_ < 4; j_++)                                                     \
                        epi.init4((M0) + wm * 16 * NI + i_ * 16 + rl_, (N0) + wn * 128 + h_ * 64 + j_ * 16 + q_ * 4, acc[h_][i_][j_]); \
            }                                                                                                            \
        }                                                                                                                \
    }
    f32x4 acc[2][NI][4];
    op16x8 af0[NI], bf0[8], af1[NI], bf1[8];
    int my = (int)blockIdx.x, cm0, cn0, nm0 = 0, nn0 = 0;
    Q4_OFFSETS(my, offA, offB, cm0, cn0);
#pragma unroll
    for (int st = 0; st < NS; st++) {
        const char* ga = reinterpret_cast<const char*>(A) + st * 128;
        const char* gb = reinterpret_cast<const char*>(B) + st * 128;
        char* sp = smem + st * SSTAGE;
#pragma unroll
        for (int i = 0; i < NA; i++) __builtin_amdgcn_global_load_lds((gptr_t)(ga + offA[i]), (lptr_t)(sp + (wave + 4 * i) * 1024), 16, 0, 0);
#pragma unroll
        for (int j = 0; j < NB; j++) __builtin_amdgcn_global_load_lds((gptr_t)(gb + offB[j]), (lptr_t)(sp + SA + (wave + 4 * j) * 1024), 16, 0, 0);
    }
    __builtin_amdgcn_sched_barrier(0);
    Q4_ACC_INIT(cm0, cn0);
    __builtin_amdgcn_sched_barrier(0);
    q4_wait_vm<(NS - 1) * ND>();
    __builtin_amdgcn_s_barrier();
    __builtin_amdgcn_sched_barrier(0);
    {
        const unsigned ch = (unsigned)(((lane >> 4) ^ ((frow >> 1) & 7)) << 4);
#pragma unroll
        for (int j = 0; j < 8; j++) bf0[j] = *reinterpret_cast<const op16x8*>(smem + SA + (wn * 128 + frow) * 128 + ch + j * 2048);
#pragma unroll
        for (int i = 0; i < NI; i++) af0[i] = *reinterpret_cast<const op16x8*>(smem + (wm * 16 * NI + frow) * 128 + ch + i * 2048);
    }
    for (;;) {
        const int next = my + (int)gridDim.x;
        const bool more = next < ntiles;
        Q4_OFFSETS(more ? next : my, noffA, noffB, nm0, nn0);
        const unsigned q4_more = (unsigned)__builtin_amdgcn_readfirstlane((more || (g.flags & 1)) ? 1 : 0);
#define Q4_RUN(NI_, NS_, V_) asm volatile(Q4_TILE_ASM_##NI_##_##NS_##_##V_ : Q4_TILE_##NI_##_##NS_##_OUTS : Q4_TILE_##NI_##_##NS_##_INS : "memory", "scc")
#ifdef CC_Q4_VARIANTS
        if constexpr (NI == 8 && VAR == 1) { Q4_RUN(8, 2, 1); } else if constexpr (NI == 8 && VAR == 2) { Q4_RUN(8, 2, 2); }
        else if constexpr (NI == 5 && NS == 3 && VAR == 1) { Q4_RUN(5, 3, 1); } else if constexpr (NI == 5 && NS == 3 && VAR == 2) { Q4_RUN(5, 3, 2); }
        else if constexpr (NI == 5 && NS == 3 && VAR == 3) { Q4_RUN(5, 3, 3); } else if constexpr (NI == 8 && VAR == 3) { Q4_RUN(8, 2, 3); }
        else if constexpr (NI == 5 && NS == 2 && VAR == 1) { Q4_RUN(5, 2, 1); } else if constexpr (NI == 5 && NS == 2 && VAR == 2) { Q4_RUN(5, 2, 2); }
        else
#endif
        {
            if constexpr (NI == 8) { Q4_RUN(8, 2, 0); } else if constexpr (NS == 3) { Q4_RUN(5, 3, 0); } else { Q4_RUN(5, 2, 0); }
        }
#undef Q4_RUN
#pragma unroll
        for (int h = 0; h < 2; h++) gemm_epilogue_regs<Epi, NI, 4>(acc[h], lane, cm0 + wm * 16 * NI, cn0 + wn * 128 + h * 64, epi);
        if (!more) break;
        my = next; cm0 = nm0; cn0 = nn0;
        Q4_ACC_INIT(cm0, cn0);
#pragma unroll
        for (int i = 0; i < NA; i++) offA[i] = noffA[i];
#pragma unroll
        for (int j = 0; j < NB; j++) offB[j] = noffB[j];
    }
    asm volatile("s_waitcnt vmcnt(0)" ::: "memory");
#undef Q4_OFFSETS
#undef Q4_ACC_INIT
}
#undef Q4_MFMA
```

include/clipcap_hip.h:

```cpp
#ifndef CLIPCAP_HIP_H
#define CLIPCAP_HIP_H

#include <stdint.h>

#ifdef __cplusplus
extern "C" {
#endif

#define CC_OK 0
#define CC_ERR_ARG (-1)
#define CC_ERR_SHAPE (-2)
#define CC_ERR_LAUNCH (-3)
#define CC_ERR_STATE (-4)

#define CC_ABI_VERSION 3
int cc_abi_version(void);

#define CC_OP_BF16 0
#define CC_OP_FP16 1
#define CC_OP_BF16X3 2

typedef struct {
    int32_t E;
    int32_t D;
// ... 117 lines not shown
int cc_cast_op16(int32_t op_dtype, const float* src, uint16_t* dst, int64_t n, void* stream);
int cc_grad_wire_pack(const float* g32, uint16_t* wire, int64_t n, void* stream);
int cc_grad_wire_unpack(const uint16_t* wire, float* g32, int64_t n, void* stream);
int cc_grad_nonfinite(const float* g32, int64_t n, float* found_inf, void* stream);
int cc_loss_scale_update(float* state, float* found_inf, float growth, float backoff, int32_t interval, void* stream);
#define CC_GRAD_NORM_BLOCKS 1024
#define CC_GRAD_NORM_THREADS 256
#define CC_GRAD_NORM_ACC 4
int64_t cc_grad_norm_scratch_floats(void);
int cc_grad_sqnorm(const float* g32, int64_t n, float* scratch, float* sumsq, void* stream);
int cc_grad_clip_coef(const float* sumsq, float max_norm, float grad_scale, const float* loss_scale, float* clip, void* stream);
int cc_adamw_step_clip(int32_t op_dtype, float* p32, const float* g32, float* m, float* v, int64_t n, float lr, float beta1, float beta2,
                       float eps, float weight_decay, int32_t step, float grad_scale, const float* loss_scale, const float* found_inf,
                       const float* clip, uint16_t* w16 , void* stream);

int cc_dropout_mask(uint64_t seed, int32_t site, int32_t layer, float p, int64_t n, uint8_t* out, void* stream);

#define CC_COMM_UID_BYTES 128
#define CC_RED_F32 0
#define CC_RED_BF16 1
#define CC_RED_F16 2
int cc_comm_unique_id(uint8_t* uid_host);
int cc_comm_create(void** comm, int32_t nranks, int32_t rank, const uint8_t* uid_host);
int cc_allreduce_bucket(void* comm, void* buf, int64_t count, int32_t dtype, void* stream);
int cc_broadcast_bucket(void* comm, void* buf, int64_t count, int32_t dtype, int32_t root, void* stream);
int cc_reduce_bucket(void* comm, void* buf, int64_t count, int32_t dtype, int32_t root, void* stream);
int cc_comm_count(void* comm, int32_t* nranks);
int cc_comm_destroy(void* comm);

int cc_sample_step(const float* logits, int32_t R, int32_t V, int32_t ld, float temperature, int32_t top_k, float top_p, int32_t mode,
                   const int64_t* history, int32_t hist_len, int32_t hist_ld, float repetition_penalty, const float* u, int32_t* next_token,
                   float* probs_out, void* stream);
int cc_sample_step_lp(const float* logits, int32_t R, int32_t V, int32_t ld, float temperature, int32_t top_k, float top_p, int32_t mode,
                      const int64_t* history, int32_t hist_len, int32_t hist_ld, float repetition_penalty, int32_t stop_token,
                      float length_penalty, const float* u, int32_t* next_token, float* probs_out, void* stream);

int cc_gemm_op16_f32(int32_t op_dtype, int32_t al, int32_t bl, const uint16_t* A, int32_t lda, const uint16_t* B, int32_t ldb, int32_t M, int32_t N,
                     int32_t K, float* C, int32_t ldc, const float* bias, int32_t ksplit, void* stream);
int64_t cc_wgrad_scratch_bytes(void);
int cc_gemm_wgrad(int32_t op_dtype, const uint16_t* X, int32_t ldx, const uint16_t* Y, int32_t ldy, int32_t Mw, int32_t Nw, int32_t K, float* dW, int32_t ldw,
                  float* scratch, void* stream);
int64_t cc_x3_image_bytes(int64_t rows, int64_t depth);
int cc_x3_split_rows(int32_t op_dtype, const float* src, int64_t ld, int32_t rows, int32_t width, int32_t form, uint16_t* dst, void* stream);
int cc_gemm_act(int32_t op_dtype, int32_t al, int32_t bl, const void* A, int32_t a_img, int32_t lda, const uint16_t* B, int32_t ldb, int32_t M, int32_t N,
                int32_t K, void* C, int32_t c_img, int32_t ldc, const float* bias, int32_t act, void* pre, void* x3, int64_t x3_bytes, void* stream);
int cc_gemm_resid(int32_t op_dtype, int32_t al, int32_t bl, const void* A, int32_t a_img, int32_t lda, const uint16_t* B, int32_t ldb, int32_t M, int32_t N,
                  int32_t K, float* out, const float* res, int32_t ld, const float* bias, float p, uint64_t seed, int32_t site, int32_t layer,
                  void* x3, int64_t x3_bytes, void* stream);
int cc_gemm_dact(int32_t op_dtype, int32_t al, int32_t bl, const void* A, int32_t a_img, int32_t lda, const uint16_t* B, int32_t ldb, int32_t M, int32_t N,
                 int32_t K, void* C, int32_t c_img, int32_t ldc, const void* aux, int32_t act, void* x3, int64_t x3_bytes, void* stream);
int cc_gemm_f32(int32_t op_dtype, int32_t al, int32_t bl, const void* A, int32_t a_img, int32_t lda, const uint16_t* B, int32_t ldb, int32_t M, int32_t N,
                int32_t K, float* C, int32_t ldc, const float* bias, int32_t mode, float alpha, int32_t ksplit, void* x3, int64_t x3_bytes,
                void* stream);
int cc_gemm_wgrad_split(int32_t op_dtype, const void* X, int32_t x_img, int32_t ldx, const float* Y, int32_t ldy, int32_t Mw, int32_t Nw, int32_t K,
                     float* dW, int32_t ldw, float* scratch, void* x3, int64_t x3_bytes, void* stream);
int cc_gemm_tile_mode(int32_t mode);
int cc_gemm_skinny_mode(int32_t mode);
int cc_decode_mode(int32_t mode);
int cc_decode_attention(const cc_gpt2_cfg* cfg, int32_t R, int32_t Tnew, int32_t pos0, int32_t ctx_max, const uint16_t* qkv, uint16_t* kv_layer,
                        const int32_t* row_map, int32_t group, int32_t append, void* ws, uint16_t* out, int32_t* path, void* stream);
int cc_layernorm_fwd(int32_t op_dtype, const float* x, const float* gamma, const float* beta, uint16_t* y, float* mean, float* rstd, int32_t rows,
                     int32_t D, void* stream);
int cc_attention_fwd(int32_t op_dtype, const uint16_t* qkv, int32_t B, int32_t S, int32_t H, int32_t hd, int32_t causal, uint16_t* out, float* lse,
                     void* stream);
int cc_attention_bwd(int32_t op_dtype, const uint16_t* qkv, const uint16_t* dout, const uint16_t* o, const float* lse, float* delta_ws, int32_t B, int32_t S,
                     int32_t H, int32_t hd, int32_t causal, uint16_t* dqkv, void* stream);
int cc_attention_fwd_x(int32_t op_dtype, const uint16_t* qkv, int32_t B, int32_t S, int32_t H, int32_t hd, int32_t causal, uint16_t* out, int32_t out_img,
                       float* lse, float p, uint64_t seed, int32_t layer, void* stream);
int cc_attention_bwd_x(int32_t op_dtype, const uint16_t* qkv, const uint16_t* dout, const uint16_t* o, const float* lse, float* delta_ws, int32_t B, int32_t S,
                       int32_t H, int32_t hd, int32_t causal, uint16_t* dqkv, int32_t dqkv_img, float p, uint64_t seed, int32_t layer, void* stream);
#define CC_LM_LSE 0
#define CC_LM_TGT 1
#define CC_LM_ROW_LOSS 2
#define CC_LM_HF 3
#define CC_LM_DHF 4
#define CC_LM_DX32 5
int cc_lmhead_put_x(const cc_gpt2_cfg* cfg, const cc_gpt2_shape* shp, void* ws, const float* x, void* stream);
int cc_lmhead_get(const cc_gpt2_cfg* cfg, const cc_gpt2_shape* shp, void* ws, int32_t field, void* dst, int64_t dst_bytes, void* stream);
int64_t cc_red_scratch_floats(void);
int cc_layernorm_bwd(int32_t op_dtype, const uint16_t* dy, const float* x, int32_t ldx, const int32_t* row_map, const float* mean,
                     const float* rstd, const float* gamma, const float* dres, float* dx32, uint16_t* dx16, float* dgamma, float* dbeta,
                     float* dcol, int32_t rows, int32_t D, float* red_ws, void* stream);
int cc_colsum_bf16(int32_t op_dtype, const uint16_t* X, int32_t ld, int32_t M, int32_t N, float* out, float* red_ws, void* stream);
int cc_colsum_multi(int32_t op_dtype, const uint16_t* const* X_host, float* const* out_host, int32_t n, int32_t ld, int32_t M, int32_t N,
                    float* red_ws, void* stream);
int cc_batch_sum(const float* src, int64_t src_stride, float* dst, int32_t len, int32_t B, float* red_ws, void* stream);

#define CC_SITE_LMHEAD_FWD 1
#define CC_SITE_LMHEAD_DGRAD 2
#define CC_SITE_GPT2_FC_FWD 3
#define CC_SITE_GPT2_PROJ2_FWD 4
#define CC_SITE_GPT2_FC_DGRAD 5
#define CC_SITE_MAPPER_FC1_FWD 6
#define CC_SITE_MAPPER_QKV_FWD 7
#define CC_SITE_MAPPER_WGRAD_FC2 8
#define CC_SITE_ALL_GEMMS 100
int cc_prof_start(int32_t site, int32_t max_samples);
int cc_prof_stop(float* ms_host, double* flops_host, int32_t* n_host);

#ifdef __cplusplus
}
#endif
#endif
```

Before: 22040 samples/s.

## Add split-K slicing to the persistent Q4 GEMM for deep-K LM dgrad

Extends the persistent Q4 GEMM kernel so that, with an FP32 slab epilogue, it can split the K dimension into slices. Each work item becomes a (tile, k-slice) pair that writes its partial into a per-slice scratch slab, and a finish kernel sums the slabs. The LM-head dgrad path, a small-M/N, very large-K (vocab) GEMM, now passes a larger scratch span, reusing the backward workspace region, so more split slices fit. The aim is to fill all CUs on this skinny deep-K GEMM. The cost is extra scratch traffic, a reduction kernel, and more complex offset and slice bookkeeping in the hand-written asm kernel loop.

```diff
diff --git a/clipcap_amd/_lib.py b/clipcap_amd/_lib.py
--- a/clipcap_amd/_lib.py
+++ b/clipcap_amd/_lib.py
@@ -120,6 +120,7 @@
     "cc_gemm_skinny_mode": (_I, [_I]),
     "cc_decode_mode": (_I, [_I]),
     "cc_decode_attention": (_I, [_GC, _I, _I, _I, _I, _P, _P, _P, _I, _I, _P, _P, C.POINTER(_I), _P]),
+    "cc_gemm_f32_slabs": (_I, [_I, _P, _I, _I, _P, _I, _I, _I, _I, _P, _I, _I, _P, _L, _P, _P, _L, _P]),
     "cc_gemm_op16_f32": (_I, [_I, _I, _I, _P, _I, _P, _I, _I, _I, _I, _P, _I, _P, _I, _P]),
     "cc_layernorm_fwd": (_I, [_I, _P, _P, _P, _P, _P, _P, _I, _I, _P]),
     "cc_attention_fwd": (_I, [_I, _P, _I, _I, _I, _I, _I, _P, _P, _P]),
diff --git a/clipcap_amd/csrc/abi_dispatch.cpp b/clipcap_amd/csrc/abi_dispatch.cpp
--- a/clipcap_amd/csrc/abi_dispatch.cpp
+++ b/clipcap_amd/csrc/abi_dispatch.cpp
@@ -157,6 +157,9 @@
 int cc_gemm_f32_bf16(int32_t al, int32_t bl, const void* A, int32_t a_img, int32_t lda, const uint16_t* B, int32_t ldb, int32_t M, int32_t N, int32_t K, float* C, int32_t ldc, const float* bias, int32_t mode, float alpha, int32_t ksplit, void* x3, int64_t x3_bytes, void* stream);
 int cc_gemm_f32_f16(int32_t al, int32_t bl, const void* A, int32_t a_img, int32_t lda, const uint16_t* B, int32_t ldb, int32_t M, int32_t N, int32_t K, float* C, int32_t ldc, const float* bias, int32_t mode, float alpha, int32_t ksplit, void* x3, int64_t x3_bytes, void* stream);
 int cc_gemm_f32_x3(int32_t al, int32_t bl, const void* A, int32_t a_img, int32_t lda, const uint16_t* B, int32_t ldb, int32_t M, int32_t N, int32_t K, float* C, int32_t ldc, const float* bias, int32_t mode, float alpha, int32_t ksplit, void* x3, int64_t x3_bytes, void* stream);
+int cc_gemm_f32_slabs_bf16(const void* A, int32_t a_img, int32_t lda, const uint16_t* B, int32_t ldb, int32_t M, int32_t N, int32_t K, float* C, int32_t ldc, int32_t ksplit, float* scratch, int64_t scratch_bytes, int32_t* slices, void* x3, int64_t x3_bytes, void* stream);
+int cc_gemm_f32_slabs_f16(const void* A, int32_t a_img, int32_t lda, const uint16_t* B, int32_t ldb, int32_t M, int32_t N, int32_t K, float* C, int32_t ldc, int32_t ksplit, float* scratch, int64_t scratch_bytes, int32_t* slices, void* x3, int64_t x3_bytes, void* stream);
+int cc_gemm_f32_slabs_x3(const void* A, int32_t a_img, int32_t lda, const uint16_t* B, int32_t ldb, int32_t M, int32_t N, int32_t K, float* C, int32_t ldc, int32_t ksplit, float* scratch, int64_t scratch_bytes, int32_t* slices, void* x3, int64_t x3_bytes, void* stream);
 int cc_gemm_wgrad_split_bf16(const void* X, int32_t x_img, int32_t ldx, const float* Y, int32_t ldy, int32_t Mw, int32_t Nw, int32_t K, float* dW, int32_t ldw, float* scratch, void* x3, int64_t x3_bytes, void* stream);
 int cc_gemm_wgrad_split_f16(const void* X, int32_t x_img, int32_t ldx, const float* Y, int32_t ldy, int32_t Mw, int32_t Nw, int32_t K, float* dW, int32_t ldw, float* scratch, void* x3, int64_t x3_bytes, void* stream);
 int cc_gemm_wgrad_split_x3(const void* X, int32_t x_img, int32_t ldx, const float* Y, int32_t ldy, int32_t Mw, int32_t Nw, int32_t K, float* dW, int32_t ldw, float* scratch, void* x3, int64_t x3_bytes, void* stream);
@@ -258,6 +261,7 @@
 int cc_gemm_resid(int32_t op_dtype, int32_t al, int32_t bl, const void* A, int32_t a_img, int32_t lda, const uint16_t* B, int32_t ldb, int32_t M, int32_t N, int32_t K, float* out, const float* res, int32_t ld, const float* bias, float p, uint64_t seed, int32_t site, int32_t layer, void* x3, int64_t x3_bytes, void* stream) { const int op_ = op_dtype; return op_ == CC_OP_FP16 ? cc_gemm_resid_f16(al, bl, A, a_img, lda, B, ldb, M, N, K, out, res, ld, bias, p, seed, site, layer, x3, x3_bytes, stream) : op_ == CC_OP_BF16X3 ? cc_gemm_resid_x3(al, bl, A, a_img, lda, B, ldb, M, N, K, out, res, ld, bias, p, seed, site, layer, x3, x3_bytes, stream) : cc_gemm_resid_bf16(al, bl, A, a_img, lda, B, ldb, M, N, K, out, res, ld, bias, p, seed, site, layer, x3, x3_bytes, stream); }
 int cc_gemm_dact(int32_t op_dtype, int32_t al, int32_t bl, const void* A, int32_t a_img, int32_t lda, const uint16_t* B, int32_t ldb, int32_t M, int32_t N, int32_t K, void* C, int32_t c_img, int32_t ldc, const void* aux, int32_t act, void* x3, int64_t x3_bytes, void* stream) { const int op_ = op_dtype; return op_ == CC_OP_FP16 ? cc_gemm_dact_f16(al, bl, A, a_img, lda, B, ldb, M, N, K, C, c_img, ldc, aux, act, x3, x3_bytes, stream) : op_ == CC_OP_BF16X3 ? cc_gemm_dact_x3(al, bl, A, a_img, lda, B, ldb, M, N, K, C, c_img, ldc, aux, act, x3, x3_bytes, stream) : cc_gemm_dact_bf16(al, bl, A, a_img, lda, B, ldb, M, N, K, C, c_img, ldc, aux, act, x3, x3_bytes, stream); }
 int cc_gemm_f32(int32_t op_dtype, int32_t al, int32_t bl, const void* A, int32_t a_img, int32_t lda, const uint16_t* B, int32_t ldb, int32_t M, int32_t N, int32_t K, float* C, int32_t ldc, const float* bias, int32_t mode, float alpha, int32_t ksplit, void* x3, int64_t x3_bytes, void* stream) { const int op_ = op_dtype; return op_ == CC_OP_FP16 ? cc_gemm_f32_f16(al, bl, A, a_img, lda, B, ldb, M, N, K, C, ldc, bias, mode, alpha, ksplit, x3, x3_bytes, stream) : op_ == CC_OP_BF16X3 ? cc_gemm_f32_x3(al, bl, A, a_img, lda, B, ldb, M, N, K, C, ldc, bias, mode, alpha, ksplit, x3, x3_bytes, stream) : cc_gemm_f32_bf16(al, bl, A, a_img, lda, B, ldb, M, N, K, C, ldc, bias, mode, alpha, ksplit, x3, x3_bytes, stream); }
+int cc_gemm_f32_slabs(int32_t op_dtype, const void* A, int32_t a_img, int32_t lda, const uint16_t* B, int32_t ldb, int32_t M, int32_t N, int32_t K, float* C, int32_t ldc, int32_t ksplit, float* scratch, int64_t scratch_bytes, int32_t* slices, void* x3, int64_t x3_bytes, void* stream) { const int op_ = op_dtype; return op_ == CC_OP_FP16 ? cc_gemm_f32_slabs_f16(A, a_img, lda, B, ldb, M, N, K, C, ldc, ksplit, scratch, scratch_bytes, slices, x3, x3_bytes, stream) : op_ == CC_OP_BF16X3 ? cc_gemm_f32_slabs_x3(A, a_img, lda, B, ldb, M, N, K, C, ldc, ksplit, scratch, scratch_bytes, slices, x3, x3_bytes, stream) : cc_gemm_f32_slabs_bf16(A, a_img, lda, B, ldb, M, N, K, C, ldc, ksplit, scratch, scratch_bytes, slices, x3, x3_bytes, stream); }
 int cc_gemm_wgrad_split(int32_t op_dtype, const void* X, int32_t x_img, int32_t ldx, const float* Y, int32_t ldy, int32_t Mw, int32_t Nw, int32_t K, float* dW, int32_t ldw, float* scratch, void* x3, int64_t x3_bytes, void* stream) { const int op_ = op_dtype; return op_ == CC_OP_FP16 ? cc_gemm_wgrad_split_f16(X, x_img, ldx, Y, ldy, Mw, Nw, K, dW, ldw, scratch, x3, x3_bytes, stream) : op_ == CC_OP_BF16X3 ? cc_gemm_wgrad_split_x3(X, x_img, ldx, Y, ldy, Mw, Nw, K, dW, ldw, scratch, x3, x3_bytes, stream) : cc_gemm_wgrad_split_bf16(X, x_img, ldx, Y, ldy, Mw, Nw, K, dW, ldw, scratch, x3, x3_bytes, stream); }
 int cc_decode_attention(const cc_gpt2_cfg* cfg, int32_t R, int32_t Tnew, int32_t pos0, int32_t ctx_max, const uint16_t* qkv, uint16_t* kv_layer, const int32_t* row_map, int32_t group, int32_t append, void* ws, uint16_t* out, int32_t* path, void* stream) { const int op_ = (cfg ? cfg->op_dtype : CC_OP_BF16); return op_ == CC_OP_FP16 ? cc_decode_attention_f16(cfg, R, Tnew, pos0, ctx_max, qkv, kv_layer, row_map, group, append, ws, out, path, stream) : op_ == CC_OP_BF16X3 ? cc_decode_attention_x3(cfg, R, Tnew, pos0, ctx_max, qkv, kv_layer, row_map, group, append, ws, out, path, stream) : cc_decode_attention_bf16(cfg, R, Tnew, pos0, ctx_max, qkv, kv_layer, row_map, group, append, ws, out, path, stream); }
 int cc_layernorm_fwd(int32_t op_dtype, const float* x, const float* gamma, const float* beta, uint16_t* y, float* mean, float* rstd, int32_t rows, int32_t D, void* stream) { const int op_ = op_dtype; return op_ == CC_OP_FP16 ? cc_layernorm_fwd_f16(x, gamma, beta, y, mean, rstd, rows, D, stream) : op_ == CC_OP_BF16X3 ? cc_layernorm_fwd_x3(x, gamma, beta, y, mean, rstd, rows, D, stream) : cc_layernorm_fwd_bf16(x, gamma, beta, y, mean, rstd, rows, D, stream); }
diff --git a/clipcap_amd/csrc/api.hip b/clipcap_amd/csrc/api.hip
--- a/clipcap_amd/csrc/api.hip
+++ b/clipcap_amd/csrc/api.hip
@@ -161,6 +161,8 @@
     float* dx32;
     Act dx16, dx16b, du16, dqkv16;
     act_t *dhf16, *dxn16, *datt16;
+    char* bwd_span;
+    size_t bwd_span_bytes;
     float* wg_scratch;
     float* red;
     void* scat;
@@ -225,6 +227,8 @@
         w.dxn16 = cv.take<act_t>(M * D);
         w.datt16 = cv.take<act_t>(M * D);
         w.dqkv16 = Act(take_img(M * 3 * D), dqw);
+        w.bwd_span = reinterpret_cast<char*>(w.du16.p);
+        w.bwd_span_bytes = w.bwd_span ? (size_t)((cv.base + cv.off) - w.bwd_span) : 0;
         w.wg_scratch = full ? cv.take<float>(WGRAD_SCRATCH_BYTES / sizeof(float)) : nullptr;
         w.red = full ? cv.take<float>(RED_SCRATCH_FLOATS) : nullptr;
         w.scat = full ? cv.take<char>(scatter_ws_bytes((int)Mc, (int)D)) : nullptr;
@@ -234,6 +238,7 @@
         w.logits16 = nullptr; w.pmax = w.psum = w.tgt_logit = w.lse_row = w.row_loss = nullptr;
         w.cref = w.lmfac = nullptr; w.hfs16 = nullptr;
         w.dx32 = nullptr; w.dx16 = w.dx16b = w.du16 = w.dqkv16 = Act(); w.dhf16 = w.dxn16 = w.datt16 = nullptr;
+        w.bwd_span = nullptr; w.bwd_span_bytes = 0;
         if (Mc > 0) {
             const int npart = c->Vp / 64;
             w.pmax = cv.take<float>(Mc * npart);
@@ -676,7 +681,7 @@
     const auto lm_dgrad = [&]() {
         auto& [st, o, w, cx, D, M, H, hd] = ps;
         const int rc = gemm_nt_deepk(dlog, c->Vp, W16(w16, o.total + o.wte), c->Vp, Mc, D, c->Vp, w.dhf16, D, reinterpret_cast<float*>(w.du16.p),
-                                     (size_t)M * 4 * D * sizeof(act_t), cx, ef ? &fix : nullptr);
+                                     (size_t)M * 4 * D * sizeof(act_t), cx, ef ? &fix : nullptr, w.bwd_span_bytes);
         if (rc != CC_ERR_SHAPE) return rc;
         const int rc2 = gemm_bf16out(0, 0, dlog, c->Vp, W16(w16, o.total + o.wte), c->Vp, Mc, D, c->Vp, w.dhf16, D, nullptr, 0, nullptr, cx);
         return (rc2 != CC_OK || !ef) ? rc2 : lm_dgrad_fix(w.dhf16, w.lmfac, w.target, fix.wte, D, Mc, st);
@@ -1000,6 +1005,19 @@
     return gemm_f32out(al, bl, ActIn(static_cast<const act_t*>(A), a_img), lda, B, ldb, M, N, K, C, ldc, bias, mode, alpha, ksplit, cx);
 }
 
+int CC_API(cc_gemm_f32_slabs)(const void* A, int32_t a_img, int32_t lda, const uint16_t* B, int32_t ldb, int32_t M, int32_t N, int32_t K, float* C, int32_t ldc,
+                      int32_t ksplit, float* scratch, int64_t scratch_bytes, int32_t* slices, void* x3, int64_t x3_bytes, void* stream) {
+    if (!hook_operands_ok(0, 0, A, a_img, lda, B, ldb, M, N, K) || !C || !al16(C) || ldc < N || ksplit < 1 || !scratch || !al16(scratch) || !slices ||
+        scratch_bytes < (int64_t)ksplit * M * N * (int64_t)sizeof(float))
+        return CC_ERR_ARG;
+    Call cx{S_(stream)};
+    hook_scratch(cx, x3, x3_bytes);
+    int n = 0;
+    const int rc = gemm_f32_slabs(ActIn(static_cast<const act_t*>(A), a_img), lda, B, ldb, M, N, K, C, ldc, ksplit, scratch, &n, cx);
+    *slices = n;
+    return rc;
+}
+
 int CC_API(cc_gemm_wgrad_split)(const void* X, int32_t x_img, int32_t ldx, const float* Y, int32_t ldy, int32_t Mw, int32_t Nw, int32_t K, float* dW,
                      int32_t ldw, float* scratch, void* x3, int64_t x3_bytes, void* stream) {
 #if CC_OP == 2
diff --git a/clipcap_amd/csrc/gemm.hip.h b/clipcap_amd/csrc/gemm.hip.h
--- a/clipcap_amd/csrc/gemm.hip.h
+++ b/clipcap_amd/csrc/gemm.hip.h
@@ -1307,6 +1307,7 @@
 #undef H_SEGEND
 #undef H_WAIT
 
+template <class Epi> struct epi_k_slices { static constexpr bool value = false; };
 #include "gemm_q4.hip.h"
 
 __device__ __forceinline__ HTTFrag g_tt_read(const char* tile, int lane_base, int xoff) {
@@ -1580,6 +1581,11 @@
     int mode;
     float alpha;
     size_t zstride = 0;
+    __device__ __forceinline__ EpiF32 at_slice(int z) const {
+        EpiF32 e = *this;
+        if (mode == 3) e.C += (size_t)z * zstride;
+        return e;
+    }
     __device__ __forceinline__ void operator()(int row, int col, float (&v)[8]) const {
         if (row >= M || col >= Ns) return;
         float* p = C + (size_t)row * ldc + col + (mode == 3 ? blockIdx.z * zstride : 0);
@@ -1623,6 +1629,8 @@
         *reinterpret_cast<float4*>(p + 4) = make_float4(v[4] + b[4], v[5] + b[5], v[6] + b[6], v[7] + b[7]);
     }
 };
+
+template <> struct epi_k_slices<EpiF32> { static constexpr bool value = true; };
 
 template <int ACT = -1>
 struct EpiDActT {
@@ -1932,9 +1940,23 @@
     static const bool on = kX3 && !(cc_lab_env("CC_X3_FUSED") && atoi(cc_lab_env("CC_X3_FUSED")) == 0);
     return on;
 }
+inline int gemm_cu_count() {
+    static const int ncu = []() { int n = 0, dev = 0; (void)hipGetDevice(&dev); (void)hipDeviceGetAttribute(&n, hipDeviceAttributeMultiprocessorCount, dev); return n > 0 ? n : 256; }();
+    return ncu;
+}
+inline int q4_ring(int K) { return (K % 192 == 0 && K >= 384) ? 3 : ((K % 128 == 0 && K >= 256) ? 2 : 0); }
+inline int q4_slices(int K, int ns, int ksplit, int* k_chunk) {
+    const int nchunk = K / (64 * ns);
+    for (int k = ksplit < 1 ? 1 : ksplit; k > 1; k--) {
+        const int per = (nchunk + k - 1) / k, eff = (nchunk + per - 1) / per;
+        if (per >= 2 && nchunk - (eff - 1) * per >= 2) { *k_chunk = per * 64 * ns; return eff; }
+    }
+    *k_chunk = K;
+    return 1;
+}
 template <class Epi>
 inline int launch_gemm(int al, int bl, const op16_t* A, int lda, const op16_t* B, int ldb, int M, int N, int K,
-                       int ksplit, const Epi& epi, hipStream_t st, int tile = -2, int group_m = 0) {
+                       int ksplit, const Epi& epi, hipStream_t st, int tile = -2, int group_m = 0, int* ks_eff = nullptr) {
     if (M <= 0 || N <= 0 || K <= 0) return CC_OK;
     if ((lda & 7) || (ldb & 7) || ((uintptr_t)A & 15) || ((uintptr_t)B & 15)) return CC_ERR_SHAPE;
     if (al == 0 && (K & 7)) return CC_ERR_SHAPE;
@@ -1943,7 +1965,7 @@
     if (bl == 1 && (N & 7)) return CC_ERR_SHAPE;
     if constexpr (!epi_row_strip<Epi>::value && !epi_strip_aux<Epi>::value) {
         if (g_gemm_s64 > 0 && al == 0 && bl == 0 && (K % G_BK) == 0 && M <= 1024)
-            return launch_gemm_s64(A, lda, B, ldb, M, N, K, ksplit, g_gemm_s64, epi, nullptr, st);
+            return launch_gemm_s64(A, lda, B, ldb, M, N, K, ksplit, g_gemm_s64, epi, ks_eff, st);
     }
     GemmShape g;
     g.M = M; g.N = N; g.K = K; g.lda = lda; g.ldb = ldb;
@@ -1956,12 +1978,13 @@
     int per = (kt + ksplit - 1) / ksplit;
     ksplit = (kt + per - 1) / per;
     g.k_chunk = per * G_BK;
+    if (ks_eff) *ks_eff = ksplit;
     dim3 grid(((M + G_BM - 1) / G_BM) * ((N + G_BN - 1) / G_BN), 1, ksplit);
     const int s256 = tile != -2 ? tile : g_gemm_tile_mode;
     int nj = 0, ni = 8;
     constexpr bool can160 = !kX3 && !epi_row_strip<Epi>::value && !epi_is_dact<Epi>::value;
     constexpr bool zsplit_ok = std::is_same<Epi, EpiF32>::value;
-    if (al == 0 && bl == 0 && (K % H_BK) == 0 && (ksplit == 1 || (zsplit_ok && tile > 0)) && s256 != 0) {
+    if (al == 0 && bl == 0 && (K % H_BK) == 0 && (ksplit == 1 || (zsplit_ok && (tile > 0 || s256 == 6 || s256 == 7))) && s256 != 0) {
         const long tm = (M + H_BM - 1) / H_BM, t128 = (long)grid.x;
         const long t256 = tm * ((N + 255) / 256), t192 = tm * ((N + 191) / 192), t320 = (long)((M + 319) / 320) * ((N + 255) / 256);
         const double c128 = t128 <= 256 ? 16384.0 / 0.75 : (double)((t128 + 511) / 512) * 32768.0;
@@ -1986,13 +2009,15 @@
             if constexpr (can160) {
                 static const bool q4_on = []() { const char* e = cc_lab_env("CC_GEMM_Q4"); return !e || atoi(e) != 0; }();
                 const bool fits32 = (size_t)M * (size_t)lda * 2 < 0xffff0000ull && (size_t)N * (size_t)ldb * 2 < 0xffff0000ull;
-                const int ns = (K % 192 == 0 && K >= 384) ? 3 : ((K % 128 == 0 && K >= 256) ? 2 : 0);
+                const int ns = q4_ring(K);
                 static const bool q4_last = []() { const char* e = cc_lab_env("CC_Q4_LAST"); return !e || atoi(e) != 0; }();
                 g.flags = q4_last ? 0 : 1;
-                if (ns && fits32 && ksplit == 1 && s256 != 6 && (q4_on || s256 == 7)) {
-                    static const int ncu = []() { int n = 0, dev = 0; (void)hipGetDevice(&dev); (void)hipDeviceGetAttribute(&n, hipDeviceAttributeMultiprocessorCount, dev); return n > 0 ? n : 256; }();
-                    const int tiles = ((M + 159) / 160) * ((N + 255) / 256);
-                    const dim3 gq((unsigned)(tiles < ncu ? tiles : ncu));
+                if (ns && fits32 && (ksplit == 1 || zsplit_ok) && s256 != 6 && (q4_on || s256 == 7)) {
+                    const int ncu = gemm_cu_count();
+                    const int nsl = q4_slices(K, ns, ksplit, &g.k_chunk);
+                    if (ks_eff) *ks_eff = nsl;
+                    const long items = (long)((M + 159) / 160) * ((N + 255) / 256) * nsl;
+                    const dim3 gq((unsigned)(items < ncu ? items : ncu));
                     if (ns == 3) {
                         launch_dyn<gemm_nt_q4_kernel<Epi, 5, 3>>(gq, dim3(256), (size_t)3 * (160 + 256) * 128, st, A, B, g, epi);
                     } else {
diff --git a/clipcap_amd/csrc/gemm_api.h b/clipcap_amd/csrc/gemm_api.h
--- a/clipcap_amd/csrc/gemm_api.h
+++ b/clipcap_amd/csrc/gemm_api.h
@@ -72,7 +72,8 @@
                    const SkinnyFuse* fuse = nullptr);
 struct LmFix { const float* fac; const int* target; const op16_t* wte; };
 int gemm_nt_deepk(ActIn A, int lda, const op16_t* B, int ldb, int M, int N, int K, act_t* out16, int ldo, float* scratch,
-                  size_t scratch_bytes, Call& cx, const LmFix* fix = nullptr);
+                  size_t scratch_bytes, Call& cx, const LmFix* fix = nullptr, size_t wide_bytes = 0);
+int gemm_f32_slabs(ActIn A, int lda, const op16_t* B, int ldb, int M, int N, int K, float* C, int ldc, int ksplit, float* scratch, int* slices, Call& cx);
 int skinny_single_min_tiles();
 bool gemm_nt_skinny_can_fuse(int M, int N, int K, size_t scratch_bytes);
 }
diff --git a/clipcap_amd/csrc/gemm_inst_f32.hip b/clipcap_amd/csrc/gemm_inst_f32.hip
--- a/clipcap_amd/csrc/gemm_inst_f32.hip
+++ b/clipcap_amd/csrc/gemm_inst_f32.hip
@@ -409,7 +409,7 @@
 }
 
 int gemm_nt_deepk(ActIn Aa, int lda, const op16_t* B, int ldb, int M, int N, int K, act_t* out16, int ldo, float* scratch,
-                  size_t scratch_bytes, Call& cx, const LmFix* fix) {
+                  size_t scratch_bytes, Call& cx, const LmFix* fix, size_t wide_bytes) {
     const hipStream_t st = cx.st;
     static const int knob = []() { const char* e = cc_lab_env("CC_DEEPK"); return e ? atoi(e) : -1; }();
     if (knob == 0 || g_gemm_tile_mode == 0 || !scratch || (N & 7) || (ldo & 7) || (K % 64) || (lda & 7) || (ldb & 7)) return CC_ERR_SHAPE;
@@ -442,10 +442,35 @@
         ks = best_ks;
         if (ks < 2) return CC_ERR_SHAPE;
     }
-    const int gm = std::max(1, (int)((tl + 7) / 8) / tiles_n);
-    const int rc = launch_gemm(0, 0, A, lda, B, ldb, M, N, K, ks, e, st, tile, gm);
+    int gm = std::max(1, (int)((tl + 7) / 8) / tiles_n);
+    if (!kX3) {
+        static const int q4c = []() { const char* v = cc_lab_env("CC_DEEPK_Q4"); return v ? atoi(v) : 1; }();
+        const bool q4c_on = q4c != 0;
+        const long t160 = (long)((M + 159) / 160) * ((N + 255) / 256);
+        const int ns = q4_ring(K), ncu = gemm_cu_count();
+        const bool fits32 = (size_t)M * (size_t)lda * 2 < 0xffff0000ull && (size_t)N * (size_t)ldb * 2 < 0xffff0000ull;
+        if (q4c_on && knob < 0 && t160 >= 64 && ns && fits32 && (g_gemm_tile_mode < 0 || g_gemm_tile_mode == 7)) {
+            const double slab_cost = (double)slab * 8.0 / 4.5e6;
+            const size_t fitw = std::max(wide_bytes, scratch_bytes) / (slab * sizeof(float));
+            double best = -1.0;
+            int best_ks = 0;
+            for (int k2 = 2; k2 <= 8 && (size_t)k2 <= fitw && k2 <= K / 2048; k2++) {
+                int chunk = 0;
+                if (q4_slices(K, ns, k2, &chunk) != k2) continue;
+                const double cost = (double)((t160 * k2 + ncu - 1) / ncu) * (chunk / 64) + k2 * slab_cost;
+                if (best < 0 || cost < best) { best = cost; best_ks = k2; }
+            }
+            const int per256 = (K / G_BK + ks - 1) / ks;
+            const double cost256 = (double)((tiles * ks + ncu - 1) / ncu) * per256 * 1.44 + ks * slab_cost;
+            if (best_ks && (best < cost256 || q4c == 2)) {
+                ks = best_ks; tile = 7;
+                gm = std::max(1, (int)(std::min<long>(t160, ncu) / 8) / ((N + 255) / 256));
+            }
+        }
+    }
+    int ks_eff = ks;
+    const int rc = launch_gemm(0, 0, A, lda, B, ldb, M, N, K, ks, e, st, tile, gm, &ks_eff);
     if (rc != CC_OK) return rc;
-    const int kt = K / G_BK, per = (kt + ks - 1) / ks, ks_eff = (kt + per - 1) / per;
     const size_t n8 = (size_t)M * (N >> 3);
     if (fix)
         hipLaunchKernelGGL(k_deepk_finish_lm, dim3((int)std::min<size_t>((n8 + 255) / 256, 2048)), dim3(256), 0, st, scratch, slab, ks_eff, M, N, *fix,
@@ -453,6 +478,25 @@
     else
         hipLaunchKernelGGL(k_splitk_finish, dim3((int)std::min<size_t>((n8 + 255) / 256, 2048)), dim3(256), 0, st, scratch, slab, ks_eff, M, N, nullptr, 0,
                            nullptr, nullptr, out16, ldo);
+    return hipGetLastError() == hipSuccess ? CC_OK : CC_ERR_LAUNCH;
+}
+
+int gemm_f32_slabs(ActIn Aa, int lda, const op16_t* B, int ldb, int M, int N, int K, float* C, int ldc, int ksplit, float* scratch, int* slices, Call& cx) {
+    const hipStream_t st = cx.st;
+    if ((N & 7) || (ldc & 3)) return CC_ERR_SHAPE;
+    const op16_t* A;
+    const int rca = nt_operand(cx, Aa, 0, 0, M, lda, ldb, K, A);
+    if (rca != CC_OK) return rca;
+    const size_t slab = (size_t)M * N;
+    EpiF32 e{scratch, nullptr, N, M, N, 3, 1.0f};
+    e.zstride = slab;
+    int ks_eff = 0;
+    const int rc = launch_gemm(0, 0, A, lda, B, ldb, M, N, K, ksplit, e, st, -2, 0, &ks_eff);
+    *slices = ks_eff;
+    if (rc != CC_OK) return rc;
+    const size_t n8 = (size_t)M * (N >> 3);
+    hipLaunchKernelGGL(k_splitk_finish, dim3((int)std::min<size_t>((n8 + 255) / 256, 2048)), dim3(256), 0, st, scratch, slab, ks_eff, M, N, nullptr, 0,
+                       nullptr, C, nullptr, ldc);
     return hipGetLastError() == hipSuccess ? CC_OK : CC_ERR_LAUNCH;
 }
 
@@ -521,9 +565,9 @@
     }
     EpiF32 e{scratch, nullptr, N, M, N, 3, 1.0f};
     e.zstride = slab;
-    int rc = s64 ? launch_gemm_s64(A, lda, B, ldb, M, N, K, ks, s64_form(ks), e, nullptr, st, bimg) : launch_gemm(0, 0, A, lda, B, ldb, M, N, K, ks, e, st);
+    int ks_eff = ks;
+    int rc = s64 ? launch_gemm_s64(A, lda, B, ldb, M, N, K, ks, s64_form(ks), e, &ks_eff, st, bimg) : launch_gemm(0, 0, A, lda, B, ldb, M, N, K, ks, e, st, -2, 0, &ks_eff);
     if (rc != CC_OK) return rc;
-    const int kt = K / G_BK, per = (kt + ks - 1) / ks, ks_eff = (kt + per - 1) / per;
     if (N <= 3072 && (N & 3) == 0) {
         SkinnyFuse f = fuse ? *fuse : SkinnyFuse{};
         hipLaunchKernelGGL(k_splitk_finish_row, dim3(M), dim3(256), 0, st, scratch, slab, ks_eff, M, N, bias, act, res, out32, out16, ldo, f);
diff --git a/clipcap_amd/csrc/gemm_q4.hip.h b/clipcap_amd/csrc/gemm_q4.hip.h
--- a/clipcap_amd/csrc/gemm_q4.hip.h
+++ b/clipcap_amd/csrc/gemm_q4.hip.h
@@ -23,7 +23,8 @@
     const int wave = __builtin_amdgcn_readfirstlane(tid >> 6);
     const int wm = wave >> 1, wn = wave & 1;
     const int tiles_n = (g.N + 255) / 256, tiles_m = (g.M + SBM - 1) / SBM, ntiles = tiles_m * tiles_n;
-    const int nbig = g.K / 64;
+    constexpr bool kSl = epi_k_slices<Epi>::value;
+    const int nsl = kSl ? (g.K + g.k_chunk - 1) / g.k_chunk : 1, nitems = ntiles * nsl;
     const unsigned lds0 = (unsigned)(size_t)(lptr_t)smem;
     const int frow = lane & 15;
     unsigned q4_la[NS][2], q4_lb[NS][2];
@@ -36,22 +37,24 @@
             q4_lb[b][kk] = lds0 + (unsigned)(b * SSTAGE + SA + (wn * 128 + frow) * 128) + ch;
         }
     const unsigned q4_slds = (unsigned)__builtin_amdgcn_readfirstlane((int)(lds0 + wave * 1024));
-    const unsigned q4_nmain = (unsigned)(nbig / NS - 2);
     const op16_t* q4_pa = A;
     const op16_t* q4_pb = B;
     const int drow = lane >> 3;
     const unsigned dchunk = (unsigned)(((lane & 7) ^ (4 * (wave & 1) + (lane >> 4))) << 4);
     unsigned offA[NA], offB[NB], noffA[NA], noffB[NB];
     unsigned toA[NA], toB[NB], q4_cnt;
-#define Q4_OFFSETS(TILE, OA, OB, M0, N0)                                                                                 \
+#define Q4_OFFSETS(ITEM, OA, OB, M0, N0, SL)                                                                             \
     {                                                                                                                    \
         int tm_, tn_;                                                                                                    \
-        tile_coords(xcd_remap((TILE), ntiles), tiles_m, tiles_n, g.group_m, tm_, tn_);                                   \
+        const int it_ = xcd_remap((ITEM), nitems);                                                                       \
+        SL = kSl ? it_ / ntiles : 0;                                                                                     \
+        tile_coords(it_ - SL * ntiles, tiles_m, tiles_n, g.group_m, tm_, tn_);                                           \
         M0 = tm_ * SBM; N0 = tn_ * 256;                                                                                  \
+        const unsigned kb_ = (unsigned)(SL * g.k_chunk * 2) + dchunk;                                                    \
         _Pragma("unroll") for (int i_ = 0; i_ < NA; i_++)                                                                \
-            OA[i_] = (unsigned)min(M0 + (wave + 4 * i_) * 8 + drow, g.M - 1) * (unsigned)(g.lda * 2) + dchunk;            \
+            OA[i_] = (unsigned)min(M0 + (wave + 4 * i_) * 8 + drow, g.M - 1) * (unsigned)(g.lda * 2) + kb_;               \
         _Pragma("unroll") for (int j_ = 0; j_ < NB; j_++)                                                                \
-            OB[j_] = (unsigned)min(N0 + (wave + 4 * j_) * 8 + drow, g.N - 1) * (unsigned)(g.ldb * 2) + dchunk;            \
+            OB[j_] = (unsigned)min(N0 + (wave + 4 * j_) * 8 + drow, g.N - 1) * (unsigned)(g.ldb * 2) + kb_;               \
     }
 #define Q4_ACC_INIT(M0, N0)                                                                                              \
     {                                                                                                                    \
@@ -68,8 +71,8 @@
     }
     f32x4 acc[2][NI][4];
     op16x8 af0[NI], bf0[8], af1[NI], bf1[8];
-    int my = (int)blockIdx.x, cm0, cn0, nm0 = 0, nn0 = 0;
-    Q4_OFFSETS(my, offA, offB, cm0, cn0);
+    int my = (int)blockIdx.x, cm0, cn0, csl, nm0 = 0, nn0 = 0, nsl0 = 0;
+    Q4_OFFSETS(my, offA, offB, cm0, cn0, csl);
 #pragma unroll
     for (int st = 0; st < NS; st++) {
         const char* ga = reinterpret_cast<const char*>(A) + st * 128;
@@ -95,10 +98,12 @@
     }
     for (;;) {
         const int next = my + (int)gridDim.x;
-        const bool more = next < ntiles;
-        Q4_OFFSETS(more ? next : my, noffA, noffB, nm0, nn0);
+        const bool more = next < nitems;
+        Q4_OFFSETS(more ? next : my, noffA, noffB, nm0, nn0, nsl0);
+        const unsigned q4_nmain = kSl ? (unsigned)__builtin_amdgcn_readfirstlane((min(g.k_chunk, g.K - csl * g.k_chunk) / 64) / NS - 2)
+                                      : (unsigned)(g.K / 64 / NS - 2);
         const unsigned q4_more = (unsigned)__builtin_amdgcn_readfirstlane((more || (g.flags & 1)) ? 1 : 0);
-#define Q4_RUN(NI_, NS_, V_) asm volatile(Q4_TILE_ASM_##NI_##_##NS_##_##V_ : Q4_TILE_##NI_##_##NS_##_OUTS : Q4_TILE_##NI_##_##NS_##_INS : "memory", "scc")
+#define Q4_RUN(NI_, NS_, V_) asm volatile(Q4_TILE_ASM_##NI_##_##NS_##_##V_ : Q4_TILE_##NI_##_##NS_##_OUTS : Q4_TILE_##NI_##_##NS_##_INS : "memory", "scc", "m0")
 #ifdef CC_Q4_VARIANTS
         if constexpr (NI == 8 && VAR == 1) { Q4_RUN(8, 2, 1); } else if constexpr (NI == 8 && VAR == 2) { Q4_RUN(8, 2, 2); }
         else if constexpr (NI == 5 && NS == 3 && VAR == 1) { Q4_RUN(5, 3, 1); } else if constexpr (NI == 5 && NS == 3 && VAR == 2) { Q4_RUN(5, 3, 2); }
@@ -111,9 +116,12 @@
         }
 #undef Q4_RUN
 #pragma unroll
-        for (int h = 0; h < 2; h++) gemm_epilogue_regs<Epi, NI, 4>(acc[h], lane, cm0 + wm * 16 * NI, cn0 + wn * 128 + h * 64, epi);
+        for (int h = 0; h < 2; h++) {
+            if constexpr (kSl) gemm_epilogue_regs<Epi, NI, 4>(acc[h], lane, cm0 + wm * 16 * NI, cn0 + wn * 128 + h * 64, epi.at_slice(csl));
+            else gemm_epilogue_regs<Epi, NI, 4>(acc[h], lane, cm0 + wm * 16 * NI, cn0 + wn * 128 + h * 64, epi);
+        }
         if (!more) break;
-        my = next; cm0 = nm0; cn0 = nn0;
+        my = next; cm0 = nm0; cn0 = nn0; csl = nsl0;
         Q4_ACC_INIT(cm0, cn0);
 #pragma unroll
         for (int i = 0; i < NA; i++) offA[i] = noffA[i];
diff --git a/include/clipcap_hip.h b/include/clipcap_hip.h
--- a/include/clipcap_hip.h
+++ b/include/clipcap_hip.h
@@ -193,6 +193,8 @@
 int cc_gemm_f32(int32_t op_dtype, int32_t al, int32_t bl, const void* A, int32_t a_img, int32_t lda, const uint16_t* B, int32_t ldb, int32_t M, int32_t N,
                 int32_t K, float* C, int32_t ldc, const float* bias, int32_t mode, float alpha, int32_t ksplit, void* x3, int64_t x3_bytes,
                 void* stream);
+int cc_gemm_f32_slabs(int32_t op_dtype, const void* A, int32_t a_img, int32_t lda, const uint16_t* B, int32_t ldb, int32_t M, int32_t N, int32_t K, float* C,
+                      int32_t ldc, int32_t ksplit, float* scratch, int64_t scratch_bytes, int32_t* slices, void* x3, int64_t x3_bytes, void* stream);
 int cc_gemm_wgrad_split(int32_t op_dtype, const void* X, int32_t x_img, int32_t ldx, const float* Y, int32_t ldy, int32_t Mw, int32_t Nw, int32_t K,
                      float* dW, int32_t ldw, float* scratch, void* x3, int64_t x3_bytes, void* stream);
 int cc_gemm_tile_mode(int32_t mode);
```

Result: no change. 22000 samples/s (-0.2%).
